# pierrebarbera/epa-ng

Hardware: AMD Instinct MI355X
Metric: query placements/sec (whole node), 512-tip GTR+G4 DNA ref, preplace+thorough (higher is better)
Workload: dtype f64; 1 GPU; cfg2: 512-tip DNA GTR+G4 ref, W=1500, 150 bp reads, dyn-heur 0.99999, preplace+thorough; branches=1021, parallelism=query-shard x1 (weak)

## Files before the change

epa_ng_amd/build.py:

```python
import os
import subprocess
import sys

HERE = os.path.dirname(os.path.abspath(__file__))
ROOT = os.path.dirname(HERE)
CSRC = os.path.join(HERE, "csrc")
HIPCC = os.environ.get("HIPCC", "/opt/rocm/bin/hipcc")

DEV_SOURCES = ["epa_dev.hip", "preplace.hip", "thorough_dna.hip", "thorough_aa.hip", "thorough_aa_mfma.hip", "thorough_generic.hip", "score_at.hip", "marginal.hip", "rell.hip", "comm.hip"]
EXTRA_FLAGS = {"thorough_dna.hip": ["-mllvm", "-amdgpu-sched-strategy=iterative-ilp"],
               "thorough_aa_mfma.hip": ["-mllvm", "-amdgpu-sched-strategy=iterative-ilp"]}
DEV_FLAGS = ["--offload-arch=gfx950", "-O3", "-std=c++17", "-fPIC", "-I", os.path.join(ROOT, "include"),
             "-I", CSRC, "-Wall", "-Wno-unused-function", "-Wno-unused-result"]


def _newer(target, deps):
    if not os.path.exists(target):
        return True
    t = os.path.getmtime(target)
    return any(os.path.getmtime(d) > t for d in deps)


def build_dev(force=False, verbose=False):
    out = os.path.join(HERE, "libepa_dev.so")
    objdir = os.path.join(HERE, "build")
    os.makedirs(objdir, exist_ok=True)
    hdrs = [os.path.join(CSRC, "epa_dev_internal.hpp"), os.path.join(CSRC, "wave_util.hpp"), os.path.join(CSRC, "rccl_abi.hpp"),
            os.path.join(ROOT, "include", "epa_dev.h")]
    objs, procs = [], []
    for src in DEV_SOURCES:
        sp = os.path.join(CSRC, src)
        op = os.path.join(objdir, src.replace(".hip", ".o"))
        objs.append(op)
        if force or _newer(op, [sp] + hdrs):
            cmd = [HIPCC] + DEV_FLAGS + EXTRA_FLAGS.get(src, []) + ["-c", sp, "-o", op]
            if verbose:
                print(" ".join(cmd), file=sys.stderr)
            procs.append((src, subprocess.Popen(cmd), [HIPCC] + DEV_FLAGS + ["-c", sp, "-o", op]))
    for src, p, plain in procs:
        if p.wait() != 0:
            if not EXTRA_FLAGS.get(src) or subprocess.call(plain) != 0:
                raise RuntimeError("hipcc failed on " + src)
    if force or procs or _newer(out, objs):
        cmd = [HIPCC, "--offload-arch=gfx950", "-shared", "-fPIC", "-o", out + ".tmp"] + objs
        subprocess.check_call(cmd)
        os.replace(out + ".tmp", out)
    return out


HOST_SOURCES = ["model.cpp", "aa_models.cpp", "parse_model.cpp", "tree.cpp", "place.cpp", "place_ranks.cpp", "rescore.cpp", "io.cpp", "capi.cpp"]
HOST_FLAGS = ["-O2", "-std=c++17", "-fPIC", "-fopenmp", "-Wall", "-Wextra", "-Wno-unused-parameter",
              "-I", os.path.join(ROOT, "include")]


def build_host(force=False, verbose=False):
    hdir = os.path.join(CSRC, "host")
    out = os.path.join(HERE, "libepa_host.so")
    exe = os.path.join(HERE, "epa-ng-amd")
    srcs = [os.path.join(hdir, s) for s in HOST_SOURCES]
    deps = srcs + [os.path.join(hdir, "epa_host.hpp"), os.path.join(ROOT, "include", "epa_dev.h")]
    link = ["-L", HERE, "-lepa_dev", "-Wl,-rpath,$ORIGIN"]
    if force or _newer(out, deps):
        cmd = ["g++"] + HOST_FLAGS + ["-shared", "-o", out + ".tmp"] + srcs + link
        if verbose:
            print(" ".join(cmd), file=sys.stderr)
        subprocess.check_call(cmd)
        os.replace(out + ".tmp", out)
    main = os.path.join(hdir, "main.cpp")
    if force or _newer(exe, deps + [main, out]):
        cmd = ["g++"] + HOST_FLAGS + ["-o", exe + ".tmp", main, "-L", HERE, "-lepa_host", "-lepa_dev",
                                      "-Wl,-rpath,$ORIGIN"]
        subprocess.check_call(cmd)
        os.replace(exe + ".tmp", exe)
    return out


if __name__ == "__main__":
    print(build_dev(force="--force" in sys.argv, verbose=True))
    print(build_host(force="--force" in sys.argv, verbose=True))
```

epa_ng_amd/csrc/epa_dev.hip:

```cpp
#include "epa_dev_internal.hpp"

#include <math.h>
#include <string.h>

#include <algorithm>
#include <numeric>
#include <atomic>
#include <thread>

static thread_local std::string g_create_err;

int epa_fail(epa_ctx* ctx, int code, const std::string& msg) {
  if (ctx) ctx->err = msg; else g_create_err = msg;
  return code;
}

namespace {
__global__ void __launch_bounds__(256) k_zero(uint4* __restrict__ a, size_t na, uint4* __restrict__ b, size_t nb) {
  const size_t stride = (size_t)gridDim.x * 256, i0 = (size_t)blockIdx.x * 256 + threadIdx.x;
  const uint4 z = make_uint4(0u, 0u, 0u, 0u);
  for (size_t i = i0; i < na; i += stride) a[i] = z;
  for (size_t i = i0; i < nb; i += stride) b[i] = z;
}
}
// ... 473 lines not shown
double log_sum_exp(const double* v, uint32_t K) {
  double mx = v[0], sum = 0.0;
  for (uint32_t j = 1; j < K; ++j) mx = std::max(mx, v[j]);
  for (uint32_t j = 0; j < K; ++j) sum += std::exp(v[j] - mx);
  return mx + std::log(sum);
}
}

extern "C" int epa_quadrature_legendre01(uint32_t K, double* nodes, double* log_weights) {
  if (K < 1 || K > 64 || !nodes || !log_weights) return EPA_ERR_INVALID_ARG;
  std::vector<double> d(K, 0.0), o(K > 1 ? K - 1 : 0), x;
  for (uint32_t i = 1; i < K; ++i) o[i - 1] = (double)i / std::sqrt(4.0 * i * i - 1.0);
  tridiag_eigenvalues(d, o, x);
  for (uint32_t j = 0; j < K; ++j) {
    double t = x[j], dp = 1.0;
    for (int it = 0; it < 3; ++it) {
      double p0 = 1.0, p1 = t;
      for (uint32_t n = 1; n < K; ++n) { const double p2 = ((2.0 * n + 1.0) * t * p1 - n * p0) / (n + 1.0); p0 = p1; p1 = p2; }
      dp = K * (t * p1 - p0) / (t * t - 1.0);
      if (it < 2) t -= p1 / dp;
    }
    nodes[j] = 0.5 * (1.0 + t);
    log_weights[j] = -std::log((1.0 - t) * (1.0 + t)) - 2.0 * std::log(std::fabs(dp));
  }
  const double norm = log_sum_exp(log_weights, K);
  for (uint32_t j = 0; j < K; ++j) log_weights[j] -= norm;
  return EPA_OK;
}

extern "C" int epa_quadrature_laguerre(uint32_t K, double* nodes, double* log_weights) {
  if (K < 1 || K > 64 || !nodes || !log_weights) return EPA_ERR_INVALID_ARG;
  std::vector<double> d(K), o(K > 1 ? K - 1 : 0), x;
  for (uint32_t i = 0; i < K; ++i) d[i] = 2.0 * i + 1.0;
  for (uint32_t i = 1; i < K; ++i) o[i - 1] = (double)i;
  tridiag_eigenvalues(d, o, x);
  for (uint32_t j = 0; j < K; ++j) {
    double t = x[j], lm = 1.0;
    for (int it = 0; it < 3; ++it) {
      double l0 = 1.0, l1 = 1.0 - t;
      for (uint32_t n = 1; n < K; ++n) { const double l2 = ((2.0 * n + 1.0 - t) * l1 - n * l0) / (n + 1.0); l0 = l1; l1 = l2; }
      lm = l0;
      if (it < 2) t -= l1 * t / (K * (l1 - l0));
    }
    nodes[j] = t;
    log_weights[j] = std::log(t) - 2.0 * std::log((double)K) - 2.0 * std::log(std::fabs(lm));
  }
  const double norm = log_sum_exp(log_weights, K);
  for (uint32_t j = 0; j < K; ++j) log_weights[j] -= norm;
  return EPA_OK;
}

extern "C" int epa_dev_device_count(void) {
  int n = 0;
  if (hipGetDeviceCount(&n) != hipSuccess) { (void)hipGetLastError(); return 0; }
  return n;
}

extern "C" const char* epa_dev_last_error(const epa_ctx* ctx) {
  return ctx ? ctx->err.c_str() : g_create_err.c_str();
}

extern "C" int epa_dev_set_query_layout(epa_ctx* ctx, uint32_t code_stride) {
  if (!ctx) return EPA_ERR_INVALID_ARG;
  ctx->code_stride = code_stride;
  return EPA_OK;
}

extern "C" int epa_dev_set_option(epa_ctx* ctx, const char* key, int value) {
  if (!ctx || !key) return EPA_ERR_INVALID_ARG;
  if (strcmp(key, "lookup_block") == 0) {
    if (!ctx->lookup_blocks) return epa_fail(ctx, EPA_ERR_INVALID_ARG, "set_option: lookup_block needs a context in the blocked lookup layout");
    if (value <= 0 || (value & 63)) return epa_fail(ctx, EPA_ERR_INVALID_ARG, "set_option: lookup_block must be a positive multiple of 64");
    for (void* p : ctx->blk_buf)
      if (p) return epa_fail(ctx, EPA_ERR_INVALID_ARG, "set_option: lookup_block must be set before the first preplacement");
    ctx->lookup_block = (uint32_t)value;
    return EPA_OK;
  }
  struct Entry { const char* name; int EpaOptions::*field; };
  static const Entry table[] = {
      {"thorough_generic", &EpaOptions::thorough_generic}, {"preplace_generic", &EpaOptions::preplace_generic},
      {"select_full_rows", &EpaOptions::select_full_rows}, {"select_sort", &EpaOptions::select_sort},
      {"queued_thorough", &EpaOptions::queued_thorough},   {"xcd_balance", &EpaOptions::xcd_balance},
      {"aa_valu", &EpaOptions::aa_valu},                   {"timers", &EpaOptions::timers},
      {"newton_lds", &EpaOptions::newton_lds}};
  for (const Entry& e : table)
    if (strcmp(key, e.name) == 0) {
      ctx->opt.*e.field = value;
      ctx->generic_thorough = ctx->generic_native || ctx->opt.thorough_generic != 0;
      return EPA_OK;
    }
  return epa_fail(ctx, EPA_ERR_INVALID_ARG, std::string("set_option: unknown key '") + key + "'");
}

extern "C" int epa_dev_set_heuristic(epa_ctx* ctx, int mode, double param) {
  if (!ctx) return EPA_ERR_INVALID_ARG;
  if (mode < EPA_HEUR_DYNAMIC || mode > EPA_HEUR_BASEBALL)
    return epa_fail(ctx, EPA_ERR_INVALID_ARG, "set_heuristic: unknown mode");
  if (mode == EPA_HEUR_FIXED && !(param >= 0.0 && param <= 1.0))
    return epa_fail(ctx, EPA_ERR_INVALID_ARG, "set_heuristic: the fraction must lie in [0, 1]");
  ctx->heur_mode = mode;
  ctx->heur_param = param;
  return EPA_OK;
}

extern "C" int epa_dev_set_query_packing(epa_ctx* ctx, int bits) {
  if (!ctx) return EPA_ERR_INVALID_ARG;
  if (bits != 8 && bits != 4) return epa_fail(ctx, EPA_ERR_INVALID_ARG, "set_query_packing: 8 or 4 bits per code");
  if (bits == 4 && ctx->s != 4)
    return epa_fail(ctx, EPA_ERR_UNSUPPORTED, "set_query_packing: the 4-bit format holds nucleotide codes only");
  ctx->code_packed4 = bits == 4;
  return EPA_OK;
}

extern "C" int epa_pack_codes_4bit(const uint8_t* codes, uint32_t Q, uint32_t stride, uint8_t* packed) {
  if (!codes || !packed) return EPA_ERR_INVALID_ARG;
  const size_t ps = ((size_t)stride + 1) / 2;
  const unsigned cap = g_encode_threads.load(std::memory_order_relaxed);
  const unsigned hw = cap ? cap : std::max(1u, std::thread::hardware_concurrency());
  const unsigned nt = (unsigned)std::min<uint64_t>(std::min(hw, 32u), std::max<uint64_t>(1, (uint64_t)Q * stride >> 20));
  std::vector<int> bad(nt, 0);
  auto work = [&](unsigned t) {
    const uint32_t q0 = (uint32_t)((uint64_t)Q * t / nt), q1 = (uint32_t)((uint64_t)Q * (t + 1) / nt);
    unsigned over = 0;
    for (uint32_t q = q0; q < q1; ++q) {
      const uint8_t* r = codes + (size_t)q * stride;
      uint8_t* o = packed + (size_t)q * ps;
      for (uint32_t p = 0; p < stride / 2; ++p) {
        const uint8_t hi = r[2 * p], lo = r[2 * p + 1];
        over |= hi | lo;
        o[p] = (uint8_t)((hi << 4) | lo);
      }
      if (stride & 1) { const uint8_t hi = r[stride - 1]; over |= hi; o[ps - 1] = (uint8_t)(hi << 4); }
    }
    bad[t] = over > 15;
  };
  if (nt == 1) work(0);
  else {
    std::vector<std::thread> th;
    for (unsigned t = 0; t < nt; ++t) th.emplace_back(work, t);
    for (auto& x : th) x.join();
  }
  for (unsigned t = 0; t < nt; ++t) if (bad[t]) return EPA_ERR_INVALID_ARG;
  return EPA_OK;
}

extern "C" int epa_unpack_codes_4bit(const uint8_t* packed, uint32_t Q, uint32_t stride, uint8_t* codes) {
  if (!codes || !packed) return EPA_ERR_INVALID_ARG;
  const size_t ps = ((size_t)stride + 1) / 2;
  for (uint32_t q = 0; q < Q; ++q)
    for (uint32_t i = 0; i < stride; ++i) {
      const uint8_t b = packed[(size_t)q * ps + i / 2];
      codes[(size_t)q * stride + i] = (i & 1) ? (b & 15u) : (b >> 4);
    }
  return EPA_OK;
}

extern "C" int epa_dev_set_stream(epa_ctx* ctx, void* s) {
  if (!ctx) return EPA_ERR_INVALID_ARG;
  ctx->stream = (hipStream_t)s;
  return EPA_OK;
}

extern "C" void epa_dev_destroy(epa_ctx* ctx) {
  if (!ctx) return;
  (void)hipSetDevice(ctx->device);
  (void)hipDeviceSynchronize();
  for (int i = 0; i < epa_ctx::N_BANKS * epa_ctx::N_SCRATCH; ++i) if (ctx->scratch[i]) (void)hipFree(ctx->scratch[i]);
  if (ctx->refT) (void)hipFree(ctx->refT);
  if (ctx->scSum) (void)hipFree(ctx->scSum);
  if (ctx->blen) (void)hipFree(ctx->blen);
  if (ctx->lookup) (void)hipFree(ctx->lookup);
  if (ctx->lookup2) (void)hipFree(ctx->lookup2);
  for (void* p : ctx->blk_buf) if (p) (void)hipFree(p);
  for (auto& v : ctx->blk_ev) for (hipEvent_t e : v) if (e) (void)hipEventDestroy(e);
  if (ctx->th_ctr) (void)hipFree(ctx->th_ctr);
  for (hipEvent_t e : ctx->ev_rb) if (e) (void)hipEventDestroy(e);
  if (ctx->refI) (void)hipFree(ctx->refI);
  if (ctx->cinv) (void)hipFree(ctx->cinv);
  if (ctx->resc0) (void)hipFree(ctx->resc0);
  if (ctx->dmodel) (void)hipFree(ctx->dmodel);
  for (ChunkSlot& sl : ctx->slots) {
    if (sl.h_in) (void)hipHostFree(sl.h_in);
    if (sl.h_out) (void)hipHostFree(sl.h_out);
    if (sl.h_stats) (void)hipHostFree(sl.h_stats);
    if (sl.h_sel) (void)hipHostFree(sl.h_sel);
    if (sl.d_in) (void)hipFree(sl.d_in);
    if (sl.d_unpacked) (void)hipFree(sl.d_unpacked);
    if (sl.d_pairs) (void)hipFree(sl.d_pairs);
    if (sl.d_res) (void)hipFree(sl.d_res);
    if (sl.d_stats) (void)hipFree(sl.d_stats);
    if (sl.d_merge) (void)hipFree(sl.d_merge);
    if (sl.d_gpairs) (void)hipFree(sl.d_gpairs);
    if (sl.d_gres) (void)hipFree(sl.d_gres);
    if (sl.d_goff) (void)hipFree(sl.d_goff);
    if (sl.h_goff) (void)hipHostFree(sl.h_goff);
    for (hipEvent_t e : {sl.ev_up, sl.ev_done, sl.ev_down, sl.ev_base}) if (e) (void)hipEventDestroy(e);
    if (sl.stream) (void)hipStreamDestroy(sl.stream);
  }
  if (ctx->copy_stream) (void)hipStreamDestroy(ctx->copy_stream);
  if (ctx->down_stream) (void)hipStreamDestroy(ctx->down_stream);
  std::vector<EvTimer*> ts = {&ctx->t_lookup};
  for (auto& bk : ctx->t_bank) for (auto& t : bk) ts.push_back(&t);
  for (auto* t : ts) { if (t->a) (void)hipEventDestroy(t->a); if (t->b) (void)hipEventDestroy(t->b); }
  delete ctx;
}

static int precompute_from_tree(epa_ctx* ctx, const epa_tree_desc* t, const uint32_t* d_tipmap);

static int padded_cats(int s, int c_in, uint32_t flags, bool from_tree) {
  int c = (c_in == 1 || c_in == 2) ? 4 : c_in;
  if (s == 4 && c_in >= 3 && (c_in & 3)) c = (c_in + 3) & ~3;
  if (s == 20 && (c_in == 3 || (c_in >= 5 && c_in <= 7))) c = (c_in + 3) & ~3;
  if (c_in >= 3 && c != c_in && (flags & EPA_FLAG_RATE_SCALERS) && !from_tree) c = c_in;
  return c;
}

static bool tuned_thorough_shape(int s, int c, uint32_t flags, bool zero0) {
  const bool sliding = !(flags & EPA_FLAG_RAXML_BLO);
  const bool dna_groups = s == 4 && (c & 3) == 0 && c <= 16;
  const bool tuned_local = (s == 4 && zero0) || s == 20;
  const bool tuned_cats = c == 4 || (dna_groups && sliding && zero0) || (s == 20 && c == 8);
  return tuned_cats && (sliding || tuned_local) &&
         !(flags & (EPA_FLAG_NEWTON_SLOW_BISECT | EPA_FLAG_NEWTON_STRICT_DF | EPA_FLAG_KEEP_EIGENVALUES));
}

static std::atomic<uint64_t> g_mem_cap{0};
extern "C" void epa_dev_set_mem_cap(uint64_t bytes) { g_mem_cap.store(bytes, std::memory_order_relaxed); }

constexpr uint32_t EPA_BLOCK_DEFAULT = 1024;
constexpr int EPA_PLAN_BANKS = 4;

extern "C" int epa_dev_footprint(uint32_t states, uint32_t rate_cats, uint64_t sites, uint64_t branches, int flags,
                                 int from_tree, uint32_t block_branches, int banks, epa_footprint* out) {
  if (!out || !(states == 4 || states == 20) || rate_cats < 1 || rate_cats > EPA_MAX_CATS || !sites || !branches ||
      sites > 0xffffffffull || branches > 0xffffffffull || banks < 0 || (block_branches & 63u))
    return epa_fail(nullptr, EPA_ERR_INVALID_ARG, "footprint: bad shape");
  const uint64_t s = states, W = sites, B = branches;
  const uint64_t c = (uint64_t)padded_cats((int)states, (int)rate_cats, (uint32_t)flags, from_tree != 0);
  const bool blocks = (flags & EPA_FLAG_LOOKUP_BLOCKS) != 0;
  const bool tuned = tuned_thorough_shape((int)s, (int)c, (uint32_t)flags, !(flags & EPA_FLAG_KEEP_EIGENVALUES));
  epa_footprint f;
  memset(&f, 0, sizeof(f));
  f.reft = 8 * 2 * B * c * s * W;
  f.scsum = 4 * B * W;
  if (!blocks) {
    f.lookup = 8 * B * W * (s == 4 ? 16 : 24);
    f.lookup2 = s == 4 ? 8 * B * 2 * ((W + 1) / 2) * 36 : 0;
    f.refi = tuned ? 8 * B * c * s * W + B * W : 0;
  } else {
    const uint64_t blk = std::min<uint64_t>(block_branches ? block_branches : EPA_BLOCK_DEFAULT, (B + 63) & ~(uint64_t)63);
    f.bank = 8 * blk * W * (s == 4 ? 16 : 24) + (s == 4 ? 8 * blk * 2 * ((W + 1) / 2) * 36 : 0);
  }
  f.misc = 8 * B + sizeof(ModelDev) + 256 * (uint64_t)epa_ctx::N_BANKS;
  if (from_tree) {
    const uint64_t n = (B + 3) / 2, cdim = (flags & EPA_FLAG_RATE_SCALERS) ? c : 1;
    f.create_temp = n * W + 32 * 3 * (n - 2) + 4 * 2 * B * cdim * W + 4 * B;
  }
  f.reference = f.reft + f.scsum + f.lookup + f.lookup2 + f.refi + f.misc;
  f.steady = f.reference + (uint64_t)banks * f.bank;
  f.peak = std::max(f.steady, f.reference + f.create_temp);
  *out = f;
  return EPA_OK;
// ... 308 lines not shown
      for (int i = 0; i < S; ++i) if ((mask >> i) & 1u) acc += Ui[x * S + i];
      ta[x] = acc;
    }
  }
  if (tip_b) {
    const uint32_t mask = tipmap[tipchars[(size_t)(r.cb & ~EPA_TIP) * W + site]];
    for (int x = 0; x < S; ++x) {
      double acc = 0.0;
      for (int i = 0; i < S; ++i) if ((mask >> i) & 1u) acc += Ui[x * S + i];
      tb[x] = acc;
    }
  }
  double I[EPA_MAX_CATS][S];
  bool ksmall[EPA_MAX_CATS];
  double mx = 0.0;
  for (int k = 0; k < c; ++k) {
    double av[S], bv[S];
#pragma unroll
    for (int x = 0; x < S; ++x) {
      av[x] = (tip_a ? ta[x] : A[(size_t)(k * S + x) * W]) * Ea[k * S + x];
      bv[x] = (tip_b ? tb[x] : Bv[(size_t)(k * S + x) * W]) * Eb[k * S + x];
    }
    double mxk = 0.0;
#pragma unroll
    for (int i = 0; i < S; ++i) {
      double a = 0.0, b = 0.0;
#pragma unroll
      for (int x = 0; x < S; ++x) {
        a = fma(U[i * S + x], av[x], a);
        b = fma(U[i * S + x], bv[x], b);
      }
      const double v = a * b;
      I[k][i] = v;
      mxk = fmax(mxk, v);
    }
    ksmall[k] = mxk < 0x1p-256;
    mx = fmax(mx, mxk);
  }
  const bool resc = mx < 0x1p-256;
  double* out = refT + (size_t)r.side * cs * W + site;
  for (int k = 0; k < c; ++k) {
    const double mult = (rate_scalers ? ksmall[k] : resc) ? 0x1p+256 : 1.0;
#pragma unroll
    for (int x = 0; x < S; ++x) {
      double acc = 0.0;
#pragma unroll
      for (int i = 0; i < S; ++i) acc = fma(Ui[x * S + i], I[k][i] * mult, acc);
      out[(size_t)(k * S + x) * W] = acc;
    }
  }
  if (rate_scalers) {
    for (int k = 0; k < c; ++k) {
      const uint32_t sa = tip_a ? 0u : sc_side[((size_t)r.ca * c + k) * W + site];
      const uint32_t sb = tip_b ? 0u : sc_side[((size_t)r.cb * c + k) * W + site];
      sc_side[((size_t)r.side * c + k) * W + site] = sa + sb + (ksmall[k] ? 1u : 0u);
    }
    return;
  }
  const uint32_t sa = tip_a ? 0u : sc_side[(size_t)r.ca * W + site];
  const uint32_t sb = tip_b ? 0u : sc_side[(size_t)r.cb * W + site];
  sc_side[(size_t)r.side * W + site] = sa + sb + (resc ? 1u : 0u);
}

__global__ void __launch_bounds__(256) k_tip_sides(const ModelDev* __restrict__ m,
                                                   const uint32_t* __restrict__ tip_of_branch,
                                                   const uint8_t* __restrict__ tipchars,
                                                   const uint32_t* __restrict__ tipmap, uint32_t W,
                                                   double* __restrict__ refT, uint32_t b0) {
  const uint32_t b = b0 + blockIdx.y;
  const uint32_t t = tip_of_branch[b];
  if (t == 0xffffffffu) return;
  const uint32_t site = blockIdx.x * blockDim.x + threadIdx.x;
  if (site >= W) return;
  const int s = m->s, c = m->c;
  const uint32_t mask = tipmap[tipchars[(size_t)t * W + site]];
  double* out = refT + (size_t)(2 * b + 1) * c * s * W + site;
  for (int x = 0; x < s; ++x) {
    double acc = 0.0;
    for (int i = 0; i < s; ++i) if ((mask >> i) & 1u) acc += m->Ui[x * s + i];
    for (int k = 0; k < c; ++k) out[(size_t)(k * s + x) * W] = acc;
  }
}

__global__ void k_scaler_sum(const uint32_t* __restrict__ sc_side, uint32_t* __restrict__ scSum, size_t n,
                             uint32_t W) {
  const size_t i = (size_t)blockIdx.x * blockDim.x + threadIdx.x;
  if (i >= n) return;
  const size_t b = i / W, w = i % W;
  scSum[i] = sc_side[(2 * b) * W + w] + sc_side[(2 * b + 1) * W + w];
}

__global__ void __launch_bounds__(256) k_align_rates(const ModelDev* __restrict__ m, double* __restrict__ refT,
                                                     const uint32_t* __restrict__ sc_side,
                                                     uint32_t* __restrict__ scSum, uint32_t W, uint32_t b0) {
  const uint32_t b = b0 + blockIdx.y;
  const uint32_t site = blockIdx.x * blockDim.x + threadIdx.x;
  if (site >= W) return;
  const int c = m->c, s = m->s;
  const uint32_t* sp = sc_side + (size_t)(2 * b) * c * W + site;
  const uint32_t* sd = sc_side + (size_t)(2 * b + 1) * c * W + site;
  uint32_t mn = 0xffffffffu;
  for (int k = 0; k < c; ++k) mn = min(mn, sp[(size_t)k * W] + sd[(size_t)k * W]);
  double* X = refT + (size_t)(2 * b) * c * s * W + site;
  for (int k = 0; k < c; ++k) {
    const uint32_t d = min(sp[(size_t)k * W] + sd[(size_t)k * W] - mn, 4u);
    if (!d) continue;
    const double f = d == 1 ? 0x1p-256 : d == 2 ? 0x1p-512 : d == 3 ? 0x1p-768 : 0x1p-1024;
    for (int x = 0; x < s; ++x) X[(size_t)(k * s + x) * W] *= f;
  }
  scSum[(size_t)b * W + site] = mn;
}

static int precompute_from_tree(epa_ctx* ctx, const epa_tree_desc* t, const uint32_t* d_tipmap) {
  const uint32_t n = t->tips, R = t->inner_records, B = ctx->B, W = ctx->W;
  if (!t->tipchars || !t->rec_child_a || !t->rec_child_b || !t->rec_length_a || !t->rec_length_b ||
      !t->branch_prox || !t->branch_dist || !d_tipmap)
    return epa_fail(ctx, EPA_ERR_INVALID_ARG, "null pointer in tree descriptor");
  if (n < 3 || R != 3 * (n - 2) || B != 2 * n - 3)
    return epa_fail(ctx, EPA_ERR_INVALID_ARG, "tree descriptor: sizes are not those of an unrooted binary tree");
  std::vector<uint32_t> side_of(R, 0xffffffffu), tip_of_branch(B, 0xffffffffu);
  for (uint32_t b = 0; b < B; ++b) {
    const uint32_t p = t->branch_prox[b], d = t->branch_dist[b];
    if ((p & EPA_TIP) || p >= R || side_of[p] != 0xffffffffu)
      return epa_fail(ctx, EPA_ERR_INVALID_ARG, "tree descriptor: bad proximal record");
    side_of[p] = 2 * b;
    if (d & EPA_TIP) {
      if ((d & ~EPA_TIP) >= n) return epa_fail(ctx, EPA_ERR_INVALID_ARG, "tree descriptor: bad tip id");
      tip_of_branch[b] = d & ~EPA_TIP;
    } else {
      if (d >= R || side_of[d] != 0xffffffffu)
        return epa_fail(ctx, EPA_ERR_INVALID_ARG, "tree descriptor: bad distal record");
      side_of[d] = 2 * b + 1;
    }
  }
  for (uint32_t r = 0; r < R; ++r)
    if (side_of[r] == 0xffffffffu)
      return epa_fail(ctx, EPA_ERR_INVALID_ARG, "tree descriptor: a record is not a side of any branch");
  std::vector<int> level(R, -1);
  auto child_level = [&](uint32_t op) { return (op & EPA_TIP) ? 0 : level[op]; };
  for (uint32_t root = 0; root < R; ++root) {
    if (level[root] >= 0) continue;
    std::vector<uint32_t> st{root};
    while (!st.empty()) {
      const uint32_t r = st.back();
      if (level[r] >= 0) { st.pop_back(); continue; }
      const uint32_t a = t->rec_child_a[r], b = t->rec_child_b[r];
      if ((!(a & EPA_TIP) && a >= R) || (!(b & EPA_TIP) && b >= R) || ((a & EPA_TIP) && (a & ~EPA_TIP) >= n) ||
          ((b & EPA_TIP) && (b & ~EPA_TIP) >= n))
        return epa_fail(ctx, EPA_ERR_INVALID_ARG, "tree descriptor: bad child operand");
      if (st.size() > (size_t)R + 1) return epa_fail(ctx, EPA_ERR_INVALID_ARG, "tree descriptor: cyclic records");
      const bool na = !(a & EPA_TIP) && level[a] < 0, nb = !(b & EPA_TIP) && level[b] < 0;
      if (na) st.push_back(a);
      if (nb) st.push_back(b);
      if (na || nb) continue;
      level[r] = 1 + std::max(child_level(a), child_level(b));
      st.pop_back();
    }
  }
  int nlev = 0;
  for (uint32_t r = 0; r < R; ++r) nlev = std::max(nlev, level[r]);
  std::vector<std::vector<uint32_t>> by_level(nlev + 1);
  for (uint32_t r = 0; r < R; ++r) by_level[level[r]].push_back(r);
  std::vector<RecDev> recs;
  recs.reserve(R);
  std::vector<uint32_t> lev_begin;
  auto opnd = [&](uint32_t op) { return (op & EPA_TIP) ? op : side_of[op]; };
  for (int l = 1; l <= nlev; ++l) {
    lev_begin.push_back((uint32_t)recs.size());
    for (uint32_t r : by_level[l])
      recs.push_back(RecDev{side_of[r], opnd(t->rec_child_a[r]), opnd(t->rec_child_b[r]), 0, t->rec_length_a[r],
                            t->rec_length_b[r]});
  }
  lev_begin.push_back((uint32_t)recs.size());
  uint8_t* d_tips = nullptr;
  RecDev* d_recs = nullptr;
  uint32_t *d_sc = nullptr, *d_tob = nullptr;
  std::string tree_oom;
  {
    epa_footprint f;
    size_t fr = 0, tot = 0;
    if (epa_dev_footprint((uint32_t)ctx->s, (uint32_t)ctx->c_in, W, B, (ctx->rate_scalers ? (int)EPA_FLAG_RATE_SCALERS : 0) |
                          (ctx->lookup_blocks ? (int)EPA_FLAG_LOOKUP_BLOCKS : 0), 1, ctx->lookup_blocks ? ctx->lookup_block : 0,
                          EPA_PLAN_BANKS, &f) == EPA_OK && hipMemGetInfo(&fr, &tot) == hipSuccess)
      tree_oom = " (reference precompute: " + std::to_string(f.peak) + " bytes needed, " + std::to_string(fr) + " bytes free now)";
  }
  auto cleanup = [&]() {
    if (d_tips) (void)hipFree(d_tips);
    if (d_recs) (void)hipFree(d_recs);
    if (d_sc) (void)hipFree(d_sc);
    if (d_tob) (void)hipFree(d_tob);
  };
#define TREE_HIP(call) do { hipError_t e__ = (call); if (e__ != hipSuccess) { cleanup(); (void)hipGetLastError(); return epa_fail(ctx, e__ == hipErrorOutOfMemory ? EPA_ERR_NO_MEMORY : EPA_ERR_HIP, std::string(#call) + ": " + hipGetErrorString(e__) + (e__ == hipErrorOutOfMemory ? tree_oom : std::string())); } } while (0)
  TREE_HIP(hipMalloc(&d_tips, (size_t)n * W));
  TREE_HIP(hipMemcpy(d_tips, t->tipchars, (size_t)n * W, hipMemcpyHostToDevice));
  TREE_HIP(hipMalloc(&d_recs, sizeof(RecDev) * recs.size()));
  TREE_HIP(hipMemcpy(d_recs, recs.data(), sizeof(RecDev) * recs.size(), hipMemcpyHostToDevice));
  const size_t cdim = ctx->rate_scalers ? (size_t)ctx->c : 1;
  TREE_HIP(hipMalloc(&d_sc, sizeof(uint32_t) * 2 * (size_t)B * cdim * W));
  TREE_HIP(hipMemset(d_sc, 0, sizeof(uint32_t) * 2 * (size_t)B * cdim * W));
  TREE_HIP(hipMalloc(&d_tob, sizeof(uint32_t) * B));
  TREE_HIP(hipMemcpy(d_tob, tip_of_branch.data(), sizeof(uint32_t) * B, hipMemcpyHostToDevice));
  const dim3 blk(256);
  for (uint32_t b0 = 0; b0 < B; b0 += EPA_GRID_Y)
    hipLaunchKernelGGL(k_tip_sides, dim3((W + 255) / 256, std::min<uint32_t>(EPA_GRID_Y, B - b0)), blk, 0, ctx->stream,
                       ctx->dmodel, d_tob, d_tips, d_tipmap, W, ctx->refT, b0);
  for (size_t l = 0; l + 1 < lev_begin.size(); ++l) {
    const uint32_t cnt = lev_begin[l + 1] - lev_begin[l];
    if (!cnt) continue;
    for (uint32_t off = 0; off < cnt; off += EPA_GRID_Y) {
      const dim3 grid((W + 255) / 256, std::min<uint32_t>(EPA_GRID_Y, cnt - off));
      if (ctx->s == 4)
        hipLaunchKernelGGL(k_clv_level<4>, grid, blk, 0, ctx->stream, ctx->dmodel, d_recs + lev_begin[l] + off,
                           d_tips, d_tipmap, W, ctx->refT, d_sc, ctx->rate_scalers ? 1 : 0);
      else
        hipLaunchKernelGGL(k_clv_level<20>, grid, blk, 0, ctx->stream, ctx->dmodel, d_recs + lev_begin[l] + off,
                           d_tips, d_tipmap, W, ctx->refT, d_sc, ctx->rate_scalers ? 1 : 0);
    }
  }
  if (ctx->rate_scalers) {
    for (uint32_t b0 = 0; b0 < B; b0 += EPA_GRID_Y)
      hipLaunchKernelGGL(k_align_rates, dim3((W + 255) / 256, std::min<uint32_t>(EPA_GRID_Y, B - b0)), blk, 0, ctx->stream,
                         ctx->dmodel, ctx->refT, d_sc, ctx->scSum, W, b0);
  } else {
    const size_t nbw = (size_t)B * W;
    hipLaunchKernelGGL(k_scaler_sum, dim3((uint32_t)((nbw + 255) / 256)), blk, 0, ctx->stream, d_sc, ctx->scSum, nbw, W);
  }
  TREE_HIP(hipStreamSynchronize(ctx->stream));
  TREE_HIP(hipGetLastError());
#undef TREE_HIP
  cleanup();
  return EPA_OK;
}

template <int S>
__global__ void __launch_bounds__(256) k_tree_logl(const ModelDev* __restrict__ m,
                                                  const double* __restrict__ refT,
                                                  const uint32_t* __restrict__ scSum, uint32_t b, double len,
                                                  uint32_t W, const double* __restrict__ cinv,
                                                  double* __restrict__ partial) {
  __shared__ double U[S * S];
  __shared__ double E[EPA_MAX_CATS * S];
  __shared__ double red[256];
  const int c = m->c;
  for (int i = threadIdx.x; i < S * S; i += blockDim.x) U[i] = m->U[i];
  for (int i = threadIdx.x; i < c * S; i += blockDim.x) E[i] = exp(m->lam[i % S] * m->rate[i / S] * len);
  __syncthreads();
  const uint32_t site = blockIdx.x * blockDim.x + threadIdx.x;
  double v = 0.0;
  if (site < W) {
    const size_t cs = (size_t)c * S;
    const double* X = refT + (size_t)(2 * b) * cs * W + site;
    const double* D = refT + (size_t)(2 * b + 1) * cs * W + site;
    double L = 0.0;
    for (int k = 0; k < c; ++k) {
      double xv[S], dv[S];
#pragma unroll
      for (int x = 0; x < S; ++x) { xv[x] = X[(size_t)(k * S + x) * W]; dv[x] = D[(size_t)(k * S + x) * W] * E[k * S + x]; }
      double t = 0.0;
#pragma unroll
      for (int i = 0; i < S; ++i) {
        double a = 0.0, d = 0.0;
#pragma unroll
        for (int x = 0; x < S; ++x) { a = fma(U[i * S + x], xv[x], a); d = fma(U[i * S + x], dv[x], d); }
        t = fma(m->pi[i] * a, d, t);
      }
      L = fma(m->w[k], t, L);
    }
    if (cinv) L += cinv[site];
    v = log(L) + (double)scSum[(size_t)b * W + site] * (-256.0 * 0.6931471805599453094);
  }
  red[threadIdx.x] = v;
  __syncthreads();
  for (int o = 128; o; o >>= 1) {
    if ((int)threadIdx.x < o) red[threadIdx.x] += red[threadIdx.x + o];
    __syncthreads();
  }
  if (threadIdx.x == 0) partial[blockIdx.x] = red[0];
}

extern "C" int epa_dev_tree_logl(epa_ctx* ctx, uint32_t branch, double* lnl) {
  if (!ctx || !lnl || branch >= ctx->B) return epa_fail(ctx, EPA_ERR_INVALID_ARG, "bad argument");
  EPA_HIP(ctx, hipSetDevice(ctx->device));
  const uint32_t nblk = (ctx->W + 255) / 256;
  double* d_part = (double*)epa_scratch(ctx, 9, sizeof(double) * nblk);
  if (!d_part) return epa_fail(ctx, EPA_ERR_HIP, "hipMalloc(tree lnL partials)");
  const double len = ctx->h_blen[branch];
  if (ctx->s == 4)
    hipLaunchKernelGGL(k_tree_logl<4>, dim3(nblk), dim3(256), 0, ctx->stream, ctx->dmodel, ctx->refT, ctx->scSum,
                       branch, len, ctx->W, ctx->cinv, d_part);
  else
    hipLaunchKernelGGL(k_tree_logl<20>, dim3(nblk), dim3(256), 0, ctx->stream, ctx->dmodel, ctx->refT, ctx->scSum,
                       branch, len, ctx->W, ctx->cinv, d_part);
  std::vector<double> part(nblk);
  EPA_HIP(ctx, hipMemcpyAsync(part.data(), d_part, sizeof(double) * nblk, hipMemcpyDeviceToHost, ctx->stream));
  EPA_HIP(ctx, hipStreamSynchronize(ctx->stream));
  double s = 0.0;
  for (double p : part) s += p;
  *lnl = s;
  return EPA_OK;
}

extern "C" int epa_dev_create_from_tree(const epa_tree_desc* tree, int device, epa_ctx** out) {
  if (!tree || !out) return epa_fail(nullptr, EPA_ERR_INVALID_ARG, "null argument");
  *out = nullptr;
  if (epa_dev_device_count() <= 0)
    return epa_fail(nullptr, EPA_ERR_NO_DEVICE,
                    "no HIP device visible: libepa_dev has no CPU fallback by design");
  epa_ctx* ctx = new epa_ctx();
  int rc = create_impl(&tree->ref, device, ctx, tree);
  if (rc != EPA_OK) {
    g_create_err = ctx->err;
    epa_dev_destroy(ctx);
// ... 339 lines not shown
extern "C" int epa_dev_select_candidates(epa_ctx* ctx, const double* lnl, uint32_t Q,
                                         double threshold, epa_pair* pairs, uint64_t max_pairs,
                                         uint64_t* n_pairs) {
  if (!ctx || !lnl || !pairs || !n_pairs) return epa_fail(ctx, EPA_ERR_INVALID_ARG, "null argument");
  *n_pairs = 0;
  if (Q == 0) return EPA_OK;
  EPA_HIP(ctx, hipSetDevice(ctx->device));
  const double* d_lnl = (const double*)epa_to_device(ctx, 3, lnl, sizeof(double) * (size_t)Q * ctx->B);
  if (!d_lnl) return epa_fail(ctx, EPA_ERR_HIP, "lnl upload failed");
  const bool out_dev = epa_is_device_ptr(pairs);
  epa_pair* d_pairs = out_dev ? pairs : (epa_pair*)epa_scratch(ctx, 4, sizeof(epa_pair) * max_pairs);
  if (!d_pairs) return epa_fail(ctx, EPA_ERR_HIP, "hipMalloc(pairs)");
  int rc = launch_select(ctx, d_lnl, Q, threshold, d_pairs, max_pairs, n_pairs);
  if (rc) return rc;
  if (!out_dev && *n_pairs) {
    EPA_HIP(ctx, hipMemcpy(pairs, d_pairs, sizeof(epa_pair) * (*n_pairs), hipMemcpyDeviceToHost));
  }
  return EPA_OK;
}

static int chunk_body_begin(epa_ctx* ctx, const uint8_t* d_codes, const uint32_t* d_begin, const uint32_t* d_span,
                            uint32_t Q, uint32_t max_span, double threshold, epa_pair* d_pairs,
                            uint64_t max_pairs, uint32_t* rb, SelectPending* sp, epa_result* d_res = nullptr,
                            unsigned long long* d_stats = nullptr) {
  const uint32_t pitch = (ctx->B + 7u) & ~7u;
  double* d_lnl = (double*)epa_scratch(ctx, 3, sizeof(double) * (size_t)Q * pitch);
  if (!d_lnl) return epa_fail(ctx, EPA_ERR_HIP, "hipMalloc(chunk table)");
  ctx->lnl_pitch = pitch;
  const uint32_t nseg = (ctx->B + 63) / 64;
  ctx->segmax = nullptr;
  if (nseg <= 64 && ctx->heur_mode == 0) {
    ctx->segp = (nseg + 7u) & ~7u;
    ctx->segmax = (unsigned long long*)epa_scratch(ctx, 10, sizeof(unsigned long long) * (size_t)Q * ctx->segp);
    if (!ctx->segmax) return epa_fail(ctx, EPA_ERR_HIP, "hipMalloc(segment maxima)");
    ctx->segmax_zero_bytes = sizeof(unsigned long long) * (size_t)Q * ctx->segp;
  }
  int rc = launch_preplace(ctx, d_codes, d_begin, d_span, Q, d_lnl, max_span);
  if (ctx->segmax_zero_bytes) {
    ctx->segmax_zero_bytes = 0;
    if (!rc) rc = epa_fail(ctx, EPA_ERR_HIP, "segment maxima not cleared");
  }
  if (!rc) rc = launch_select_begin(ctx, d_lnl, Q, threshold, d_pairs, max_pairs, d_span, rb, sp);
  ctx->lnl_pitch = 0;
  ctx->segmax = nullptr;
  if (!rc && d_stats && sp->d_rb && sp->bitmap && max_pairs <= 0xffffffffull) {
    rc = launch_select_emit(ctx, sp);
    if (!rc) rc = epa_zero_async(ctx, d_stats, 128, epa_th_ctr(ctx), epa_th_ctr(ctx) ? 64 : 0);
    if (!rc) {
      ctx->clean_stats[ctx->bank] = d_stats;
      ctx->clean_ctr[ctx->bank] = epa_th_ctr(ctx) != nullptr;
    }
  }
  if (!rc && d_res && d_stats && sp->d_rb && sp->bitmap && max_pairs <= 0xffffffffull) {
    const bool off = !ctx->opt.queued_thorough;
    const int cls = epa_span_class(ctx->s, max_span);
    const bool eligible = !off && ctx->s == 4 && !ctx->generic_thorough && ctx->dna.ng == 1 && epa_th_ctr(ctx) &&
                          (cls <= 2 || cls == 10 || cls == 11);
    if (eligible) {
      rc = launch_select_emit(ctx, sp);
      if (!rc && ctx->clean_stats[ctx->bank] == d_stats) ctx->clean_stats[ctx->bank] = nullptr;
      else if (!rc) rc = epa_zero_async(ctx, d_stats, 128);
      if (!rc) {
        const int q = launch_thorough_queued(ctx, d_pairs, sp->d_rb, max_pairs, d_codes, d_begin, d_span, max_span, d_res, d_stats);
        if (q == -2) return EPA_ERR_HIP;
        sp->queued_cls = q;
      }
    }
  }
  return rc;
}

static int chunk_body_end(epa_ctx* ctx, SelectPending* sp, const uint8_t* d_codes, const uint32_t* d_begin,
                          const uint32_t* d_span, uint32_t max_span, epa_pair* d_pairs, epa_result* d_res,
                          unsigned long long* d_stats, uint64_t* n_out) {
  const uint32_t pitch = (ctx->B + 7u) & ~7u;
  ctx->lnl_pitch = pitch;
  uint64_t n = 0;
  int rc = launch_select_end(ctx, sp, &n);
  ctx->lnl_pitch = 0;
  if (rc) return rc;
  rc = select_check_status(ctx, sp);
  if (rc) return rc;
  *n_out = n;
  if (sp->queued_cls >= 0 && sp->rb[9 + sp->queued_cls] == (uint32_t)n) return EPA_OK;
  if (ctx->clean_stats[ctx->bank] == d_stats && sp->queued_cls < 0) ctx->clean_stats[ctx->bank] = nullptr;
  else {
    ctx->clean_stats[ctx->bank] = nullptr;
    rc = epa_zero_async(ctx, d_stats, 128);
    if (rc) return rc;
  }
  if (n == 0) return EPA_OK;
  return launch_thorough(ctx, d_pairs, n, d_codes, d_begin, d_span, max_span, d_res, d_stats,
                         sp->have_hist ? sp->cls_hist : nullptr);
}

static int chunk_body(epa_ctx* ctx, const uint8_t* d_codes, const uint32_t* d_begin, const uint32_t* d_span,
                      uint32_t Q, uint32_t max_span, double threshold, epa_pair* d_pairs, epa_result* d_res,
                      uint64_t max_pairs, unsigned long long* d_stats, uint64_t* n_out) {
  uint32_t rb[64] = {};
  SelectPending sp;
  int rc = chunk_body_begin(ctx, d_codes, d_begin, d_span, Q, max_span, threshold, d_pairs, max_pairs, rb, &sp, d_res, d_stats);
  if (rc) return rc;
  return chunk_body_end(ctx, &sp, d_codes, d_begin, d_span, max_span, d_pairs, d_res, d_stats, n_out);
}

static int chunk_stats(epa_ctx* ctx, uint64_t n, const unsigned long long* hst, epa_thorough_stats* stats) {
  epa_xcd_feedback(ctx, n, hst);
  ctx->last_stats.pairs = n;
  ctx->last_stats.rounds = hst[0];
  ctx->last_stats.newton_evals = hst[1];
  ctx->last_stats.reverts = hst[2];
  if (stats) *stats = ctx->last_stats;
  if (hst[3])
    return epa_fail(ctx, EPA_ERR_NEG_INF,
                    "-INF logl at branch " + std::to_string((uint32_t)(hst[4] >> 32)) +
                        " with sequence " + std::to_string((uint32_t)(hst[4] & 0xffffffffu)));
  return EPA_OK;
}

static int thorough_supported(epa_ctx*) { return EPA_OK; }

extern "C" int epa_dev_place_chunk(epa_ctx* ctx, const uint8_t* q_codes, const uint32_t* win_begin,
                                   const uint32_t* win_span, uint32_t Q, uint32_t max_span,
                                   double threshold, epa_pair* pairs, epa_result* results,
                                   uint64_t max_pairs, uint64_t* n_pairs, epa_thorough_stats* stats) {
  if (!ctx || !q_codes || !win_begin || !win_span || !pairs || !results || !n_pairs)
    return epa_fail(ctx, EPA_ERR_INVALID_ARG, "null argument");
  *n_pairs = 0;
  if (stats) memset(stats, 0, sizeof(*stats));
  if (Q == 0) return EPA_OK;
  EPA_HIP(ctx, hipSetDevice(ctx->device));
  int rc = thorough_supported(ctx);
  if (rc) return rc;
  rc = epa_dev_build_lookup(ctx);
  if (rc) return rc;
  if (max_span == 0) {
    std::vector<uint32_t> buf;
    const uint32_t* hs = host_view(win_span, Q, buf, ctx->stream);
    if (!hs) return epa_fail(ctx, EPA_ERR_HIP, "cannot read window spans");
    for (uint32_t q = 0; q < Q; ++q) max_span = std::max(max_span, hs[q]);
  }
  if (max_span > ctx->W) max_span = ctx->W;
  const uint8_t* d_codes = epa_codes_to_device(ctx, q_codes, Q);
  const uint32_t* d_begin = (const uint32_t*)epa_to_device(ctx, 1, win_begin, sizeof(uint32_t) * Q);
  const uint32_t* d_span = (const uint32_t*)epa_to_device(ctx, 2, win_span, sizeof(uint32_t) * Q);
  if (!d_codes || !d_begin || !d_span) return epa_fail(ctx, EPA_ERR_HIP, "query upload failed");
  const bool pairs_dev = epa_is_device_ptr(pairs), res_dev = epa_is_device_ptr(results);
  epa_pair* d_pairs = pairs_dev ? pairs : (epa_pair*)epa_scratch(ctx, 4, sizeof(epa_pair) * max_pairs);
  epa_result* d_res = res_dev ? results : (epa_result*)epa_scratch(ctx, 5, sizeof(epa_result) * max_pairs);
  if (!d_pairs || !d_res) return epa_fail(ctx, EPA_ERR_HIP, "hipMalloc(chunk buffers)");
  unsigned long long* d_stats = reinterpret_cast<unsigned long long*>(reinterpret_cast<char*>(epa_th_ctr(ctx)) + 128);
  uint64_t n = 0;
  rc = chunk_body(ctx, d_codes, d_begin, d_span, Q, max_span, threshold, d_pairs, d_res, max_pairs, d_stats, &n);
  if (rc) return rc;
  *n_pairs = n;
  if (n == 0) return EPA_OK;
  unsigned long long hst[16];
  if (!pairs_dev)
    EPA_HIP(ctx, hipMemcpyAsync(pairs, d_pairs, sizeof(epa_pair) * n, hipMemcpyDeviceToHost, ctx->stream));
  if (!res_dev)
    EPA_HIP(ctx, hipMemcpyAsync(results, d_res, sizeof(epa_result) * n, hipMemcpyDeviceToHost, ctx->stream));
  EPA_HIP(ctx, hipMemcpyAsync(hst, d_stats, 128, hipMemcpyDeviceToHost, ctx->stream));
  EPA_HIP(ctx, hipStreamSynchronize(ctx->stream));
  return chunk_stats(ctx, n, hst, stats);
}

static int slot_of(epa_ctx* ctx, int slot, ChunkSlot** out) {
  if (!ctx) return EPA_ERR_INVALID_ARG;
  if (slot < 0 || slot >= epa_ctx::N_SLOTS) return epa_fail(ctx, EPA_ERR_INVALID_ARG, "chunk pipeline: slot must be 0 .. 23");
  ChunkSlot& s = ctx->slots[slot];
  if (!ctx->copy_stream) EPA_HIP(ctx, hipStreamCreateWithFlags(&ctx->copy_stream, hipStreamNonBlocking));
  if (!ctx->down_stream) EPA_HIP(ctx, hipStreamCreateWithFlags(&ctx->down_stream, hipStreamNonBlocking));
  if (!s.ev_up) {
    EPA_HIP(ctx, hipEventCreateWithFlags(&s.ev_up, hipEventDisableTiming));
    EPA_HIP(ctx, hipEventCreateWithFlags(&s.ev_done, hipEventDisableTiming));
    EPA_HIP(ctx, hipEventCreateWithFlags(&s.ev_down, hipEventDisableTiming));
// ... 745 lines not shown
```

epa_ng_amd/csrc/epa_dev_internal.hpp:

```cpp
#pragma once

#include <hip/hip_runtime.h>
#include <stdint.h>

#include <string>
#include <vector>

#include "epa_dev.h"

#define EPA_MAX_STATES 20
#define EPA_MAX_CATS 16
#define EPA_MAX_COLS 24
#define EPA_GRID_Y 65535u

struct ModelDNA {
  double U[16];
  double Ui[16];
  double lam[4];
  double rate[16];
  double w[16];
  double pi[4];
  int ng;
};

struct BloConsts {
  double min_branch, max_branch, default_branch, epsilon, pendant_default;
  uint32_t max_rounds, max_newton;
  uint32_t sliding;
  uint32_t newton_variant;
};

struct ModelDev {
  int s, c, ncols;
  double U[EPA_MAX_STATES * EPA_MAX_STATES];
  double Ui[EPA_MAX_STATES * EPA_MAX_STATES];
  double lam[EPA_MAX_STATES];
  double pi[EPA_MAX_STATES];
  double rate[EPA_MAX_CATS];
  double w[EPA_MAX_CATS];
  uint32_t colmask[EPA_MAX_COLS];
  double qt[EPA_MAX_COLS * EPA_MAX_STATES];
};

struct EvTimer {
  hipEvent_t a = nullptr, b = nullptr;
  bool valid = false;
};

struct SelectPending {
  const double* d_lnl = nullptr;
  uint32_t Q = 0, cap = 0;
  double threshold = 0.0;
  epa_pair* d_pairs = nullptr;
  uint64_t max_pairs = 0;
  const uint32_t* d_span = nullptr;
  unsigned long long *stage = nullptr, *keys_a = nullptr, *keys_b = nullptr;
  uint32_t *counts = nullptr, *offsets = nullptr;
  uint32_t *bitmap = nullptr, *boffs = nullptr;
  uint32_t wpr = 0;
  void* temp = nullptr;
  size_t sort_bytes = 0;
  uint32_t* rb = nullptr;
  bool have_status = false;
  bool rerun = false;
  hipEvent_t ev_rb = nullptr;
  const uint32_t* d_rb = nullptr;
  bool emitted = false;
  int queued_cls = -1;
  uint32_t cls_hist[16] = {};
  bool have_hist = false;
  const uint32_t* pre_status = nullptr;
};

struct ChunkSlot {
  void* h_in = nullptr;
  size_t h_in_sz = 0;
  void* d_in = nullptr;
  const uint8_t* x_codes = nullptr;
  const uint32_t* x_begin = nullptr;
  const uint32_t* x_span = nullptr;
  size_t d_in_sz = 0;
  uint8_t* d_unpacked = nullptr;
  size_t d_unpacked_sz = 0;
  size_t codes_bytes = 0;
  uint32_t Q = 0, stride = 0;
  bool packed4 = false;
  epa_pair* d_pairs = nullptr;
  epa_result* d_res = nullptr;
  size_t cap = 0;
  void* h_out = nullptr;
  size_t h_out_sz = 0;
  unsigned long long* h_stats = nullptr;
  unsigned long long* d_stats = nullptr;
  hipEvent_t ev_up = nullptr, ev_done = nullptr, ev_down = nullptr, ev_base = nullptr;
  hipStream_t stream = nullptr;
  const epa_pair* out_pairs = nullptr;
  const epa_result* out_res = nullptr;
  uint64_t n = 0;
  int state = 0;
  SelectPending sel;
  uint32_t* h_sel = nullptr;
  const uint8_t* l_codes = nullptr;
  const uint32_t *l_begin = nullptr, *l_span = nullptr;
  epa_pair* l_pairs = nullptr;
  epa_result* l_res = nullptr;
  uint32_t l_max_span = 0, l_flags = 0;
  int leader = -1;
  int g_index = 0;
  int g_n = 0;
  int g_left = 0;
  int g_slots[8] = {};
  uint32_t g_qoff[9] = {};
  uint32_t own_Q = 0;
  const uint8_t* own_x_codes = nullptr;
  const uint32_t *own_x_begin = nullptr, *own_x_span = nullptr;
  void* d_merge = nullptr;
  size_t d_merge_sz = 0;
  epa_pair* d_gpairs = nullptr;
  epa_result* d_gres = nullptr;
  size_t g_cap = 0;
  uint32_t* d_goff = nullptr;
  uint32_t* h_goff = nullptr;
};
constexpr int EPA_MAX_GROUP = 8;

struct EpaOptions {
  int thorough_generic = 0;
  int preplace_generic = 0;
  int select_full_rows = 0;
  int select_sort = 0;
  int queued_thorough = 0;
  int xcd_balance = 1;
  int aa_valu = 0;
  int timers = 1;
  int newton_lds = 0;
};

struct epa_ctx {
  int device = 0;
  EpaOptions opt;
  int n_cu = 256;
  hipStream_t stream = nullptr;
  std::string err;

  int s = 0, c = 0, ncols = 0;
  int c_in = 0;
  uint32_t W = 0, B = 0;
  ModelDev hmodel;
  ModelDev* dmodel = nullptr;
  ModelDNA dna;
  bool dna_zero0 = false;
  bool rate_scalers = false;
  bool generic_thorough = false;
  bool generic_native = false;
  BloConsts blo;
  int aa_x_as_n = 0;
  uint32_t code_stride = 0;

  double* refT = nullptr;
  uint32_t* scSum = nullptr;
  double* blen = nullptr;
  double* lookup = nullptr;
  double* refI = nullptr;
  uint8_t* resc0 = nullptr;
  double* cinv = nullptr;
  double inv_w0 = 0.0;
  double* lookup2 = nullptr;
  bool lookup_built = false;
  bool lookup_blocks = false;
  uint32_t lookup_block = 1024;
  std::vector<double> h_blen;

  static constexpr int N_SCRATCH = 18;
  static constexpr int N_SLOTS = 24;
  static constexpr int N_BANKS = 1 + N_SLOTS;
  int bank = 0;
  void* scratch[N_BANKS * N_SCRATCH] = {};
  size_t scratch_sz[N_BANKS * N_SCRATCH] = {};

  uint32_t* d_status = nullptr;
  uint32_t select_cap = 64;
  uint32_t* th_ctr = nullptr;
  uint32_t lnl_pitch = 0;
  unsigned long long* segmax = nullptr;
  uint32_t segp = 0;
  size_t segmax_zero_bytes = 0;
  bool code_packed4 = false;
  int heur_mode = 0;
  double heur_param = 0.0;

  hipStream_t copy_stream = nullptr, down_stream = nullptr;
  ChunkSlot slots[N_SLOTS];

  enum { T_PREPLACE = 0, T_THOROUGH = 1, T_SELECT = 2, T_SCORE = 3, T_SITES = 4, T_RELL = 5, T_MARGINAL = 6, N_TIMERS = 7 };
  EvTimer t_lookup;
  std::vector<hipEvent_t> blk_ev[N_BANKS];
  uint32_t blk_ev_n[N_BANKS] = {};
  void* blk_buf[N_BANKS] = {};
  size_t blk_sz[N_BANKS] = {};
  EvTimer t_bank[N_BANKS][N_TIMERS];
  uint32_t xcd_cum[9] = {0u, 1u << 17, 2u << 17, 3u << 17, 4u << 17, 5u << 17, 6u << 17, 7u << 17, 1u << 20};
  double xcd_w[8] = {0.125, 0.125, 0.125, 0.125, 0.125, 0.125, 0.125, 0.125};
  double last_sclk_mhz = 0.0;
  bool xstamp_ok = false;
  hipEvent_t ev_rb[N_BANKS] = {};
  const void* clean_stats[N_BANKS] = {};
  bool clean_ctr[N_BANKS] = {};
  int t_last[N_TIMERS] = {};
  epa_thorough_stats last_stats{};
};

int epa_fail(epa_ctx* ctx, int code, const std::string& msg);
void* epa_scratch(epa_ctx* ctx, int slot, size_t bytes);
inline uint32_t* epa_th_ctr(epa_ctx* ctx) { return ctx->th_ctr ? ctx->th_ctr + 64 * ctx->bank : nullptr; }
int epa_zero_async(epa_ctx* ctx, void* p, size_t bytes, void* p2 = nullptr, size_t bytes2 = 0);
inline int epa_th_ctr_reset(epa_ctx* ctx) {
  if (ctx->clean_ctr[ctx->bank]) { ctx->clean_ctr[ctx->bank] = false; return 0; }
  return epa_zero_async(ctx, epa_th_ctr(ctx), 64);
}
bool epa_is_device_ptr(const void* p);
const void* epa_to_device(epa_ctx* ctx, int slot, const void* p, size_t bytes);
const uint8_t* epa_codes_to_device(epa_ctx* ctx, const uint8_t* q_codes, uint32_t Q);
const uint8_t* epa_codes_to_device(epa_ctx* ctx, const uint8_t* q_codes, uint32_t Q);
void epa_xcd_feedback(epa_ctx* ctx, uint64_t n_pairs, const unsigned long long* hst);
#define EPA_XSTAMP_MASK 0x7ffffffffffull
void epa_timer_start(epa_ctx* ctx, EvTimer& t);
void epa_timer_stop(epa_ctx* ctx, EvTimer& t);
inline EvTimer& epa_t(epa_ctx* ctx, int which) { ctx->t_last[which] = ctx->bank; return ctx->t_bank[ctx->bank][which]; }

#define EPA_HIP(ctx, call)                                                               \
  do {                                                                                    \
    hipError_t e__ = (call);                                                              \
    if (e__ != hipSuccess)                                                                \
      return epa_fail(ctx, EPA_ERR_HIP, std::string(#call) + ": " + hipGetErrorString(e__)); \
  } while (0)

constexpr int EPA_N_CLS = 12;
constexpr uint32_t EPA_AA_LDS_MAX_SPAN = 102;
__host__ __device__ inline int epa_span_class(int states, uint32_t span) {
  if (states != 4) return span <= 64 ? 0 : span <= 128 ? 1 : span <= 192 ? 2 : 3;
  if (span > 64 && span <= 96) return 10;
  if (span > 128 && span <= 160) return 11;
  const uint32_t nch = (span + 63) / 64;
  return nch <= 4 ? (nch ? (int)nch - 1 : 0) : nch <= 6 ? 4 : nch <= 8 ? 5 : nch <= 12 ? 6 : nch <= 16 ? 7 : nch <= 24 ? 8 : 9;
}

int launch_transform(epa_ctx* ctx, const double* d_clv_or_null, const uint8_t* d_tip_or_null,
                     const uint32_t* d_tipmap, uint32_t tipmap_size, double* dst);
int launch_build_lookup(epa_ctx* ctx);
int launch_build_lookup2(epa_ctx* ctx);
uint32_t epa_block_branches(const epa_ctx* ctx);
size_t epa_block_bytes(int s, uint32_t W, uint32_t blk, size_t* off2);
void* epa_block_buffer(epa_ctx* ctx);
int launch_build_lookup_block(epa_ctx* ctx, uint32_t b0, uint32_t nb, double* blk_lookup);
int launch_build_lookup2_block(epa_ctx* ctx, uint32_t nb, const double* blk_lookup, double* blk_lookup2);
int launch_preplace(epa_ctx* ctx, const uint8_t* d_codes, const uint32_t* d_begin,
                    const uint32_t* d_span, uint32_t Q, double* d_lnl, uint32_t max_span);
int preplace_check_status(epa_ctx* ctx);
int launch_thorough(epa_ctx* ctx, const epa_pair* d_pairs, uint64_t n_pairs, const uint8_t* d_codes,
                    const uint32_t* d_begin, const uint32_t* d_span, uint32_t max_span,
                    epa_result* d_out, unsigned long long* d_stats,
                    const uint32_t* cls_hist = nullptr);
int launch_thorough_queued(epa_ctx* ctx, const epa_pair* d_pairs, const uint32_t* d_spec, uint64_t max_pairs,
                           const uint8_t* d_codes, const uint32_t* d_begin, const uint32_t* d_span, uint32_t max_span,
                           epa_result* d_out, unsigned long long* d_stats);
int launch_select_emit(epa_ctx* ctx, SelectPending* sp);
int launch_thorough_aa(epa_ctx* ctx, const epa_pair* d_pairs, const uint32_t* d_order, uint64_t n_pairs,
                       const uint8_t* d_codes, const uint32_t* d_begin, const uint32_t* d_span,
                       uint32_t max_span, bool want_lds, epa_result* d_out, unsigned long long* d_stats);
int launch_thorough_generic(epa_ctx* ctx, const epa_pair* d_pairs, uint64_t n_pairs, const uint8_t* d_codes,
                            const uint32_t* d_begin, const uint32_t* d_span, uint32_t max_span,
                            epa_result* d_out, unsigned long long* d_stats,
                            const uint32_t* d_order = nullptr, bool caller_times = false);
int launch_thorough_aa_mfma(epa_ctx* ctx, const epa_pair* d_pairs, const uint32_t* d_order, uint64_t n_pairs,
                            const uint8_t* d_codes, const uint32_t* d_begin, const uint32_t* d_span,
                            uint32_t max_span, epa_result* d_out, unsigned long long* d_stats);
int launch_score_at(epa_ctx* ctx, const epa_pair* d_pairs, const double* d_pendant, const double* d_distal,
                    const double* d_proximal, uint64_t n, const uint8_t* d_codes, const uint32_t* d_begin,
                    const uint32_t* d_span, double* d_lnl);
int launch_site_lnl(epa_ctx* ctx, const epa_pair* d_pairs, const double* d_pendant, const double* d_distal,
                    const double* d_proximal, const uint32_t* d_order, uint64_t n_rows, const uint8_t* d_codes,
                    const uint32_t* d_begin, const uint32_t* d_span, uint32_t pitch, bool pad, double* d_rows,
                    bool timed);
int launch_rell(epa_ctx* ctx, const epa_pair* d_pairs, const double* d_pendant, const double* d_distal,
                const double* d_proximal, uint64_t n, const uint8_t* d_codes, const uint32_t* d_begin,
                const uint32_t* d_span, const uint32_t* h_span, uint32_t Q, const uint64_t* d_stream_id,
                uint32_t replicates, uint64_t seed, double* d_support);
int launch_marginal(epa_ctx* ctx, const epa_pair* d_pairs, uint64_t n, const double* d_rule, uint32_t Kx, uint32_t Kp,
                    const uint8_t* d_codes, const uint32_t* d_begin, const uint32_t* d_span, double* d_marginal,
                    double* d_grid);
int launch_select(epa_ctx* ctx, const double* d_lnl, uint32_t Q, double threshold,
                  epa_pair* d_pairs, uint64_t max_pairs, uint64_t* n_pairs,
                  const uint32_t* d_span = nullptr);
int launch_select_begin(epa_ctx* ctx, const double* d_lnl, uint32_t Q, double threshold, epa_pair* d_pairs,
                        uint64_t max_pairs, const uint32_t* d_span, uint32_t* rb, SelectPending* sp);
int launch_select_end(epa_ctx* ctx, SelectPending* sp, uint64_t* n_pairs);
int select_check_status(epa_ctx* ctx, const SelectPending* sp);
```

epa_ng_amd/csrc/preplace.hip:

```cpp
#include "epa_dev_internal.hpp"
#include "wave_util.hpp"

#include <cstdlib>
#include <cstring>
#include <rocprim/device/device_radix_sort.hpp>

using epa_radix_cfg = rocprim::radix_sort_config<rocprim::default_config, rocprim::default_config,
                                                 rocprim::default_config, 0>;
#include <rocprim/device/device_scan.hpp>

#include <algorithm>

namespace {

constexpr int GQ = 256;
constexpr int CH = 160;
constexpr int SPREAD = 96;
constexpr int TROWS = CH + SPREAD;
constexpr int NB = 16;
constexpr int CW = CH / 4;

struct Group {
  uint32_t start;
  uint32_t count;
  uint32_t min_begin;
  uint32_t cls;
};

__device__ __forceinline__ void validate_window(uint32_t i, uint32_t begin, uint32_t span, uint32_t W,
                                                uint32_t cmax, uint32_t* status) {
  if (span == 0) atomicMax(&status[0], 0x80000000u | i);
  else if ((uint64_t)begin + span > W || span > cmax) atomicMax(&status[1], 0x80000000u | i);
}
__global__ void k_validate(const uint32_t* __restrict__ win_begin, const uint32_t* __restrict__ win_span,
                           uint32_t Q, uint32_t W, uint32_t cmax, uint32_t* __restrict__ status) {
  const uint32_t i = blockIdx.x * blockDim.x + threadIdx.x;
  if (i < Q) validate_window(i, win_begin[i], win_span[i], W, cmax, status);
}

__global__ void k_iota(uint32_t* v, uint32_t n) {
  const uint32_t i = blockIdx.x * blockDim.x + threadIdx.x;
  if (i < n) v[i] = i;
}

__global__ void __launch_bounds__(256) k_count_keys(const uint32_t* __restrict__ keys, uint32_t Q,
                                                    uint32_t* __restrict__ cnt, uint32_t* __restrict__ rank) {
  const uint32_t q = blockIdx.x * 256 + threadIdx.x;
  if (q < Q) rank[q] = atomicAdd(&cnt[keys[q]], 1u);
}
__global__ void __launch_bounds__(1024) k_scan_counts(uint32_t* __restrict__ cnt, uint32_t K) {
  __shared__ uint32_t wsum[16];
  __shared__ uint32_t carry_s;
  const uint32_t t = threadIdx.x, lane = t & 63u, wv = t >> 6;
  if (t == 0) carry_s = 0;
  __syncthreads();
  constexpr uint32_t PER = 8;
  for (uint32_t base = 0; base < K; base += 1024 * PER) {
    uint32_t v[PER], tot = 0;
#pragma unroll
    for (uint32_t i = 0; i < PER; ++i) {
      const uint32_t k = base + t * PER + i;
      v[i] = k < K ? cnt[k] : 0u;
      tot += v[i];
    }
    uint32_t inc = tot;
#pragma unroll
    for (int o = 1; o < 64; o <<= 1) {
      const uint32_t u = __shfl_up(inc, o);
      if ((int)lane >= o) inc += u;
    }
    if (lane == 63) wsum[wv] = inc;
    __syncthreads();
    uint32_t before = carry_s;
    for (uint32_t w = 0; w < wv; ++w) before += wsum[w];
    uint32_t run = before + inc - tot;
#pragma unroll
    for (uint32_t i = 0; i < PER; ++i) {
      const uint32_t k = base + t * PER + i;
      if (k < K) cnt[k] = run;
      run += v[i];
    }
    __syncthreads();
    if (t == 1023) carry_s = run;
    __syncthreads();
  }
}
__global__ void __launch_bounds__(256) k_scatter_sorted(const uint32_t* __restrict__ keys,
                                                        const uint32_t* __restrict__ rank,
                                                        const uint32_t* __restrict__ offs, uint32_t Q,
                                                        uint32_t* __restrict__ sorted_keys,
                                                        uint32_t* __restrict__ perm) {
  const uint32_t q = blockIdx.x * 256 + threadIdx.x;
  if (q >= Q) return;
  const uint32_t k = keys[q], pos = offs[k] + rank[q];
  sorted_keys[pos] = k;
  perm[pos] = q;
}

__global__ void __launch_bounds__(256) k_make_groups(const uint32_t* __restrict__ sorted_keys, uint32_t Q,
                                                     uint32_t Wp, uint32_t n_blocks,
                                                     uint32_t class_blocks, uint32_t gq0, uint32_t gq1,
                                                     uint32_t spr0, uint32_t max_runs, Group* __restrict__ groups,
                                                     uint32_t max_groups, uint32_t* __restrict__ status) {
  extern __shared__ uint32_t sh[];
  uint32_t* lo = sh;
  uint32_t* runbase = lo + n_blocks + 1;
  uint32_t* run_start = runbase + n_blocks + 1;
  uint32_t* run_end = run_start + max_runs;
  uint32_t* run_off = run_end + max_runs;
  auto lower_bound = [&](uint32_t a, uint32_t b, uint64_t key) {
    while (a < b) {
      const uint32_t m = (a + b) >> 1;
      if ((uint64_t)sorted_keys[m] < key) a = m + 1; else b = m;
    }
    return a;
  };
  for (uint32_t k = threadIdx.x; k <= n_blocks; k += blockDim.x)
    lo[k] = k == n_blocks ? Q : lower_bound(0, Q, (uint64_t)k * Wp);
  for (uint32_t i = threadIdx.x; i < max_groups; i += blockDim.x) groups[i] = Group{0, 0, 0, 0};
  __syncthreads();
  if (threadIdx.x == 0) {
    uint32_t r = 0;
    for (uint32_t b = 0; b < n_blocks; ++b) {
      const uint32_t gq = b >= class_blocks ? gq1 : gq0;
      runbase[b] = r;
      r += (lo[b + 1] - lo[b] + gq - 1) / gq;
    }
    runbase[n_blocks] = r;
  }
  __syncthreads();
  const uint32_t nruns = min(runbase[n_blocks], max_runs);
  for (uint32_t r = threadIdx.x; r < nruns; r += blockDim.x) {
    uint32_t b = 0;
    while (b + 1 < n_blocks && r >= runbase[b + 1]) ++b;
    const uint32_t gq = b >= class_blocks ? gq1 : gq0;
    const uint32_t start = lo[b] + (r - runbase[b]) * gq, end = min(lo[b + 1], start + gq);
    const uint32_t k0 = sorted_keys[start], k1 = sorted_keys[end - 1];
    const uint32_t spr = b >= class_blocks ? (uint32_t)SPREAD : spr0;
    run_start[r] = start;
    run_end[r] = end;
    run_off[r] = (k1 - k0 < spr) ? 1u : (k1 / spr - k0 / spr + 1);
  }
  __syncthreads();
  uint32_t* cnt = run_off + max_runs + 1;
  for (uint32_t r = threadIdx.x; r < nruns; r += blockDim.x) cnt[r] = run_off[r];
  __syncthreads();
  for (uint32_t r = threadIdx.x; r <= nruns; r += blockDim.x) {
    uint32_t g = 0;
    for (uint32_t i = 0; i < r; ++i) g += cnt[i];
    run_off[r] = g;
  }
  __syncthreads();
  if (threadIdx.x == 0) {
    const uint32_t r1 = class_blocks < n_blocks ? min(runbase[class_blocks], nruns) : nruns;
    status[4] = min(run_off[nruns], max_groups);
    status[5] = min(run_off[r1], max_groups);
  }
  for (uint32_t r = threadIdx.x; r < nruns; r += blockDim.x) {
    uint32_t b = 0;
    while (b + 1 < n_blocks && r >= runbase[b + 1]) ++b;
    const uint32_t cls = b >= class_blocks ? 1u : 0u;
    const uint32_t start = run_start[r], end = run_end[r], g0 = run_off[r], n = run_off[r + 1] - g0;
    if (n == 1) {
      if (g0 < max_groups) groups[g0] = Group{start, end - start, 0, cls};
    } else {
      const uint32_t spr = cls ? (uint32_t)SPREAD : spr0;
      const uint32_t kb = sorted_keys[start] / spr;
// ... 1264 lines not shown
        if (weighted ? (sabove + iw >= threshold) : (ic >= rem)) atomicMin(&s_first, t);
        atomicMax(&s_last, t);
      }
      __syncthreads();
      uint32_t ts = s_first;
      if (ts == 256u) {
        if (p == 7) { all = true; n = B; break; }
        ts = s_last;
      }
      const uint32_t ec = ts ? s_hc[ts - 1u] : 0u;
      const double ew = ts ? s_hw[ts - 1u] : 0.0;
      m = s_hc[ts] - ec;
      cabove += ec;
      rem -= weighted ? 0u : ec;
      sabove += ew;
      prefix = (prefix << 8) | (unsigned long long)(255u - ts);
      __syncthreads();
    }
    if (!all) {
      K = prefix;
      if (weighted) {
        const double w = exp(seg_val(K) - mx) / tot;
        double sum = sabove;
        while (r < m && sum < threshold) { sum += w; ++r; }
        n = cabove + r;
      } else {
        r = rem;
      }
    }
  }
  if (n > 0) {
    const bool ordered = !all && r < m;
    uint32_t tie_base = 0;
    if (t == 0) s_cnt = 0u;
    __syncthreads();
    for (uint32_t base = 0; base < B; base += 256) {
      const uint32_t i = base + t;
      const unsigned long long k = i < B ? seg_key(src[i]) : 0ull;
      bool sel = i < B && (all || k > K);
      bool eq = i < B && !all && k == K;
      if (ordered) {
        const unsigned long long bal = __ballot(eq);
        if (lane == 0) s_wu[wv] = (uint32_t)__popcll(bal);
        __syncthreads();
        uint32_t before = tie_base + (uint32_t)__popcll(bal & ((1ull << lane) - 1ull));
        for (uint32_t w = 0; w < wv; ++w) before += s_wu[w];
        tie_base += s_wu[0] + s_wu[1] + s_wu[2] + s_wu[3];
        eq = eq && before < r;
        __syncthreads();
      }
      sel = sel || eq;
      uint32_t slot = 0;
      if (!so.bitmap) {
        const unsigned long long bal = __ballot(sel);
        uint32_t wbase = 0;
        if (lane == 0 && bal) wbase = atomicAdd(&s_cnt, (uint32_t)__popcll(bal));
        wbase = (uint32_t)__builtin_amdgcn_readfirstlane((int)wbase);
        slot = wbase + (uint32_t)__popcll(bal & ((1ull << lane) - 1ull));
      }
      if (sel) so.put(q, i, slot, status);
    }
  }
  if (t == 0) counts[q] = so.count(n);
}

__global__ void __launch_bounds__(256) k_class_hist(const uint32_t* __restrict__ counts,
                                                   const uint32_t* __restrict__ win_span, uint32_t Q,
                                                   int states, uint32_t* __restrict__ hist) {
  const uint32_t q = blockIdx.x * 256 + threadIdx.x;
  const int cls = q < Q ? epa_span_class(states, win_span[q]) : -1;
  const uint32_t n = q < Q ? counts[q] : 0;
  for (int c = 0; c < EPA_N_CLS; ++c) {
    if (__ballot(cls == c) == 0ull) continue;
    uint32_t v = cls == c ? n : 0;
#pragma unroll
    for (int o = 32; o; o >>= 1) v += __shfl_xor(v, o);
    if ((threadIdx.x & 63) == 0 && v) atomicAdd(&hist[c], v);
  }
}

__global__ void __launch_bounds__(64) k_pack_readback(const uint32_t* __restrict__ status,
                                                     const uint32_t* __restrict__ total,
                                                     const uint32_t* __restrict__ pre_status,
                                                     uint32_t* __restrict__ out) {
  const uint32_t t = threadIdx.x;
  if (t == 0) out[0] = *total;
  if (t < 8 + EPA_N_CLS) out[1 + t] = status[t];
  if (t < 4) out[32 + t] = pre_status ? pre_status[t] : 0u;
}

__global__ void __launch_bounds__(256) k_compact(const unsigned long long* __restrict__ stage,
                                                 const uint32_t* __restrict__ counts,
                                                 const uint32_t* __restrict__ offsets, uint32_t Q,
                                                 uint32_t cap, unsigned long long* __restrict__ keys) {
  const uint32_t q = blockIdx.x * 4 + (threadIdx.x >> 6);
  const int lane = threadIdx.x & 63;
  if (q >= Q) return;
  const uint32_t n = counts[q], o = offsets[q];
  for (uint32_t i = lane; i < n; i += 64) keys[o + i] = stage[(size_t)q * cap + i];
}

__global__ void __launch_bounds__(256) k_emit_pairs(const uint32_t* __restrict__ bitmap, uint32_t wpr,
                                                    const uint32_t* __restrict__ boffs,
                                                    epa_pair* __restrict__ pairs, uint32_t nb, uint32_t max_pairs) {
  __shared__ uint32_t wsum[4];
  const uint32_t b = blockIdx.x, t = threadIdx.x, lane = t & 63u, wv = t >> 6;
  if (boffs[nb] > max_pairs) return;
  uint32_t base = boffs[b];
  const uint32_t end = boffs[b + 1];
  if (base == end) return;
  const uint32_t* row = bitmap + (size_t)b * wpr;
  for (uint32_t w0 = 0; w0 < wpr && base < end; w0 += 256) {
    const uint32_t wi = w0 + t;
    uint32_t bits = wi < wpr ? row[wi] : 0u;
    const uint32_t c = (uint32_t)__popc(bits);
    uint32_t inc = c;
#pragma unroll
    for (int o = 1; o < 64; o <<= 1) {
      const uint32_t u = __shfl_up(inc, o);
      if ((int)lane >= o) inc += u;
    }
    if (lane == 63) wsum[wv] = inc;
    __syncthreads();
    uint32_t before = 0, total = 0;
#pragma unroll
    for (uint32_t w = 0; w < 4; ++w) {
      if (w < wv) before += wsum[w];
      total += wsum[w];
    }
    uint32_t o = base + before + inc - c;
    while (bits) {
      const uint32_t k = (uint32_t)__ffs((int)bits) - 1u;
      bits &= bits - 1u;
      pairs[o].branch_id = b;
      pairs[o].seq_id = wi * 32u + k;
      ++o;
    }
    base += total;
    __syncthreads();
  }
}

__global__ void k_keys_to_pairs(const unsigned long long* __restrict__ keys, uint64_t n,
                                epa_pair* __restrict__ pairs) {
  const uint64_t i = (uint64_t)blockIdx.x * blockDim.x + threadIdx.x;
  if (i < n) {
    pairs[i].branch_id = (uint32_t)(keys[i] >> 32);
    pairs[i].seq_id = (uint32_t)(keys[i] & 0xffffffffu);
  }
}

size_t align256(size_t x) { return (x + 255) & ~(size_t)255; }

}

int launch_build_lookup2(epa_ctx* ctx) {
  if (!ctx->lookup2)
    EPA_HIP(ctx, hipMalloc(&ctx->lookup2, sizeof(double) * (size_t)ctx->B * 2 * ((ctx->W + 1) / 2) * PE));
  for (uint32_t b0 = 0; b0 < ctx->B; b0 += EPA_GRID_Y)
    hipLaunchKernelGGL(k_build_lookup2, dim3((ctx->W * PE + 255) / 256, std::min<uint32_t>(EPA_GRID_Y, ctx->B - b0)), dim3(256), 0,
                       ctx->stream, ctx->lookup, ctx->W, ctx->lookup2, b0);
  EPA_HIP(ctx, hipGetLastError());
  return EPA_OK;
}

int launch_build_lookup2_block(epa_ctx* ctx, uint32_t nb, const double* blk_lookup, double* blk_lookup2) {
  for (uint32_t r0 = 0; r0 < nb; r0 += EPA_GRID_Y)
    hipLaunchKernelGGL(k_build_lookup2, dim3((ctx->W * PE + 255) / 256, std::min<uint32_t>(EPA_GRID_Y, nb - r0)), dim3(256), 0,
                       ctx->stream, blk_lookup, ctx->W, blk_lookup2, r0);
  EPA_HIP(ctx, hipGetLastError());
  return EPA_OK;
// ... 163 lines not shown
  }
  { const int rc = mark(2 * nblocks); if (rc) return rc; }
  if (timed) ctx->blk_ev_n[ctx->bank] = 2 * nblocks + 1;
  EPA_HIP(ctx, hipGetLastError());
  return EPA_OK;
}

int preplace_check_status(epa_ctx* ctx) {
  if (!ctx->d_status) return EPA_OK;
  uint32_t st[4];
  EPA_HIP(ctx, hipMemcpy(st, ctx->d_status, sizeof(st), hipMemcpyDeviceToHost));
  if (st[0])
    return epa_fail(ctx, EPA_ERR_QUERY_ALL_GAP, "Sequence " + std::to_string(st[0] & 0x7fffffffu) +
                                                    " does not appear to have any non-gap sites!");
  if (st[1])
    return epa_fail(ctx, EPA_ERR_QUERY_WIDTH, "Query sequence length not same as reference alignment!");
  return EPA_OK;
}

int launch_select_begin(epa_ctx* ctx, const double* d_lnl, uint32_t Q, double threshold, epa_pair* d_pairs,
                        uint64_t max_pairs, const uint32_t* d_span, uint32_t* rb, SelectPending* sp) {
  sp->have_hist = false;
  const uint32_t B = ctx->B;
  const uint32_t pitch = ctx->lnl_pitch ? ctx->lnl_pitch : B;
  if (!sp->rerun) sp->pre_status = (const uint32_t*)ctx->d_status;
  const double stream_band = (ctx->heur_mode == 0 && threshold > 0.0 && threshold < 1.0) ? 1.0 - std::log((1.0 - threshold) / (double)B) : 0.0;
  const int mode = ctx->heur_mode;
  uint32_t limit = 0;
  if (mode == 1) {
    limit = (uint32_t)std::min<double>((double)B, std::ceil(ctx->heur_param * (double)B));
    ctx->select_cap = std::max(ctx->select_cap, std::max(limit, 1u));
  } else if (mode == 2) {
    ctx->select_cap = std::max(ctx->select_cap, std::min(B, 48u));
  }
  const uint32_t cap = ctx->select_cap;
  size_t scan_bytes = 0, sort_bytes = 0;
  (void)rocprim::exclusive_scan(nullptr, scan_bytes, (uint32_t*)nullptr, (uint32_t*)nullptr, 0u, Q,
                                rocprim::plus<uint32_t>(), ctx->stream);
  const size_t worst = std::min<uint64_t>(max_pairs, (uint64_t)Q * cap);
  (void)rocprim::radix_sort_keys<epa_radix_cfg>(nullptr, sort_bytes, (unsigned long long*)nullptr,
                                 (unsigned long long*)nullptr, worst, 0, 64, ctx->stream);
  const uint32_t wpr = (Q + 31) / 32;
  const bool force_sort = ctx->opt.select_sort != 0;
  const bool bm = !force_sort && (size_t)B * wpr * sizeof(uint32_t) <= ((size_t)64 << 20);
  sp->bitmap = nullptr;
  if (bm) {
    const size_t cb = align256(sizeof(uint32_t) * ((size_t)B + 1));
    const size_t mb = align256(sizeof(uint32_t) * (size_t)B * wpr);
    const size_t qb2 = align256(sizeof(uint32_t) * (Q + 1));
    char* base = (char*)epa_scratch(ctx, 7, 512 + cb + mb + qb2);
    if (!base) return epa_fail(ctx, EPA_ERR_HIP, "hipMalloc(select scratch)");
    uint32_t* status = reinterpret_cast<uint32_t*>(base);
    uint32_t* bcount = reinterpret_cast<uint32_t*>(base + 512);
    uint32_t* bitmap = reinterpret_cast<uint32_t*>(base + 512 + cb);
    uint32_t* counts = reinterpret_cast<uint32_t*>(base + 512 + cb + mb);
    sp->bitmap = bitmap; sp->boffs = bcount; sp->wpr = wpr;
    sp->counts = counts; sp->offsets = nullptr;
    sp->d_lnl = d_lnl; sp->Q = Q; sp->threshold = threshold; sp->d_pairs = d_pairs; sp->max_pairs = max_pairs;
    sp->d_span = d_span; sp->cap = cap; sp->rb = rb;
    { const int zr = epa_zero_async(ctx, base, 512 + cb + mb); if (zr) return zr; }
    epa_timer_start(ctx, epa_t(ctx, epa_ctx::T_SELECT));
    const SelOut so{nullptr, 0u, bitmap, bcount, wpr};
    const dim3 grid((Q + 3) / 4);
    const int nr = (int)((B + 63) / 64);
#define SEL(N) hipLaunchKernelGGL(k_select<N>, grid, dim3(256), 0, ctx->stream, d_lnl, Q, B, pitch, threshold, mode, limit, so, counts, status)
    const bool seg_off = ctx->opt.select_full_rows != 0;
    bool seg_hist = false;
    if (ctx->segmax && !seg_off && mode == 0 && threshold < 1.0 && nr <= 64)
    {
      const double band_x = 1.0 - std::log((1.0 - threshold) / (double)B);
      const double band_t = std::max(band_x, std::log((double)B) + 38.0);
      constexpr uint32_t sel_grid = 16;
      const dim3 grid_seg(std::min<uint32_t>((Q + 3) / 4, (uint32_t)ctx->n_cu * sel_grid));
      hipLaunchKernelGGL(k_select_seg<8>, grid_seg, dim3(256), 0, ctx->stream, d_lnl, ctx->segmax, ctx->segp, Q, B, pitch, threshold,
                         band_x, band_t, so, counts, status, d_span, ctx->s, d_span ? status + 8 : nullptr);
      seg_hist = d_span != nullptr;
    }
    else if (nr <= 2) SEL(2); else if (nr <= 4) SEL(4); else if (nr <= 8) SEL(8); else if (nr <= 16) SEL(16);
    else if (nr <= 32) SEL(32); else if (nr <= 64) SEL(64);
    else if (nr <= 128) hipLaunchKernelGGL(k_select_wg<32>, dim3(Q), dim3(256), 0, ctx->stream, d_lnl, Q, B, pitch, threshold, mode, limit, so, counts, status);
    else if (nr <= 256) hipLaunchKernelGGL(k_select_wg<64>, dim3(Q), dim3(256), 0, ctx->stream, d_lnl, Q, B, pitch, threshold, mode, limit, so, counts, status);
    else hipLaunchKernelGGL(k_select_stream, dim3(Q), dim3(256), 0, ctx->stream, d_lnl, Q, B, pitch, threshold, stream_band, mode, limit, so, counts, status);
#undef SEL
    hipLaunchKernelGGL(k_scan_counts, dim3(1), dim3(1024), 0, ctx->stream, bcount, B + 1);
    if (d_span && !seg_hist)
      hipLaunchKernelGGL(k_class_hist, dim3((Q + 255) / 256), dim3(256), 0, ctx->stream, counts, d_span, Q,
                         ctx->s, status + 8);
    hipLaunchKernelGGL(k_pack_readback, dim3(1), dim3(64), 0, ctx->stream, status, bcount + B,
                       sp->pre_status, status + 64);
    EPA_HIP(ctx, hipMemcpyAsync(rb, status + 64, sizeof(uint32_t) * 36, hipMemcpyDeviceToHost, ctx->stream));
    sp->have_status = sp->pre_status != nullptr;
    if (!ctx->ev_rb[ctx->bank]) EPA_HIP(ctx, hipEventCreateWithFlags(&ctx->ev_rb[ctx->bank], hipEventDisableTiming));
    EPA_HIP(ctx, hipEventRecord(ctx->ev_rb[ctx->bank], ctx->stream));
    sp->ev_rb = ctx->ev_rb[ctx->bank];
    sp->d_rb = status + 64;
    sp->emitted = false;
    sp->queued_cls = -1;
    return EPA_OK;
  }
  sp->ev_rb = nullptr; sp->d_rb = nullptr; sp->emitted = false; sp->queued_cls = -1;
  const size_t qb = align256(sizeof(uint32_t) * (Q + 1));
  const size_t sb = align256(sizeof(unsigned long long) * (size_t)Q * cap);
  const size_t kb = align256(sizeof(unsigned long long) * worst);
  const size_t tb = std::max(scan_bytes, sort_bytes);
  char* base = (char*)epa_scratch(ctx, 7, 512 + 2 * qb + sb + 2 * kb + tb);
  if (!base) return epa_fail(ctx, EPA_ERR_HIP, "hipMalloc(select scratch)");
  uint32_t* status = reinterpret_cast<uint32_t*>(base);
  uint32_t* counts = reinterpret_cast<uint32_t*>(base + 512);
  uint32_t* offsets = reinterpret_cast<uint32_t*>(base + 512 + qb);
  sp->stage = reinterpret_cast<unsigned long long*>(base + 512 + 2 * qb);
  sp->keys_a = reinterpret_cast<unsigned long long*>(base + 512 + 2 * qb + sb);
  sp->keys_b = reinterpret_cast<unsigned long long*>(base + 512 + 2 * qb + sb + kb);
  sp->temp = base + 512 + 2 * qb + sb + 2 * kb;
  sp->sort_bytes = sort_bytes;
  sp->counts = counts; sp->offsets = offsets;
  sp->d_lnl = d_lnl; sp->Q = Q; sp->threshold = threshold; sp->d_pairs = d_pairs; sp->max_pairs = max_pairs;
  sp->d_span = d_span; sp->cap = cap; sp->rb = rb;
  EPA_HIP(ctx, hipMemsetAsync(status, 0, 512, ctx->stream));
  EPA_HIP(ctx, hipMemsetAsync(counts + Q, 0, sizeof(uint32_t), ctx->stream));
  epa_timer_start(ctx, epa_t(ctx, epa_ctx::T_SELECT));
  const dim3 grid((Q + 3) / 4);
  const int nr = (int)((B + 63) / 64);
  const SelOut so{sp->stage, cap, nullptr, nullptr, 0u};
#define SEL(N) hipLaunchKernelGGL(k_select<N>, grid, dim3(256), 0, ctx->stream, d_lnl, Q, B, pitch, threshold, mode, limit, so, counts, status)
  if (nr <= 2) SEL(2); else if (nr <= 4) SEL(4); else if (nr <= 8) SEL(8); else if (nr <= 16) SEL(16);
  else if (nr <= 32) SEL(32); else if (nr <= 64) SEL(64);
  else if (nr <= 128) hipLaunchKernelGGL(k_select_wg<32>, dim3(Q), dim3(256), 0, ctx->stream, d_lnl, Q, B, pitch, threshold, mode, limit, so, counts, status);
  else if (nr <= 256) hipLaunchKernelGGL(k_select_wg<64>, dim3(Q), dim3(256), 0, ctx->stream, d_lnl, Q, B, pitch, threshold, mode, limit, so, counts, status);
  else hipLaunchKernelGGL(k_select_stream, dim3(Q), dim3(256), 0, ctx->stream, d_lnl, Q, B, pitch, threshold, stream_band, mode, limit, so, counts, status);
#undef SEL
  EPA_HIP(ctx, rocprim::exclusive_scan(sp->temp, scan_bytes, counts, offsets, 0u, Q + 1,
                                       rocprim::plus<uint32_t>(), ctx->stream));
  if (d_span)
    hipLaunchKernelGGL(k_class_hist, dim3((Q + 255) / 256), dim3(256), 0, ctx->stream, counts, d_span, Q,
                       ctx->s, status + 8);
  hipLaunchKernelGGL(k_pack_readback, dim3(1), dim3(64), 0, ctx->stream, status, offsets + Q,
                     sp->pre_status, status + 64);
  EPA_HIP(ctx, hipMemcpyAsync(rb, status + 64, sizeof(uint32_t) * 36, hipMemcpyDeviceToHost, ctx->stream));
  sp->have_status = sp->pre_status != nullptr;
  return EPA_OK;
}

int launch_select_emit(epa_ctx* ctx, SelectPending* sp) {
  if (!sp->bitmap || !sp->d_rb || sp->emitted) return EPA_OK;
  hipLaunchKernelGGL(k_emit_pairs, dim3(ctx->B), dim3(256), 0, ctx->stream, sp->bitmap, sp->wpr, sp->boffs, sp->d_pairs, ctx->B, (uint32_t)std::min<uint64_t>(sp->max_pairs, 0xffffffffu));
  epa_timer_stop(ctx, epa_t(ctx, epa_ctx::T_SELECT));
  EPA_HIP(ctx, hipGetLastError());
  sp->emitted = true;
  return EPA_OK;
}

int launch_select_end(epa_ctx* ctx, SelectPending* sp, uint64_t* n_pairs) {
  const uint32_t B = ctx->B, Q = sp->Q;
  for (;;) {
    if (sp->ev_rb) EPA_HIP(ctx, hipEventSynchronize(sp->ev_rb));
    else EPA_HIP(ctx, hipStreamSynchronize(ctx->stream));
    const uint32_t total = sp->rb[0];
    const uint32_t* hst = sp->rb + 1;
    if (hst[2] && !sp->bitmap) {
      if (sp->cap >= B) return epa_fail(ctx, EPA_ERR_HIP, "select_candidates: staging overflow");
      ctx->select_cap = std::min<uint32_t>(B, std::max(sp->cap * 4, hst[2]));
      uint32_t* rb = sp->rb;
      sp->rerun = true;
      int rc = launch_select_begin(ctx, sp->d_lnl, Q, sp->threshold, sp->d_pairs, sp->max_pairs, sp->d_span, rb, sp);
      sp->rerun = false;
      if (rc) return rc;
      continue;
    }
    if (total > sp->max_pairs)
      return epa_fail(ctx, EPA_ERR_PAIR_OVERFLOW,
                      "select_candidates: " + std::to_string(total) + " candidates exceed max_pairs");
    if (total && sp->bitmap) {
      if (!sp->emitted)
        hipLaunchKernelGGL(k_emit_pairs, dim3(B), dim3(256), 0, ctx->stream, sp->bitmap, sp->wpr, sp->boffs, sp->d_pairs, B, (uint32_t)std::min<uint64_t>(sp->max_pairs, 0xffffffffu));
    } else if (total) {
      const dim3 grid((Q + 3) / 4);
      hipLaunchKernelGGL(k_compact, grid, dim3(256), 0, ctx->stream, sp->stage, sp->counts, sp->offsets, Q, sp->cap,
                         sp->keys_a);
      int bits = 33;
      while ((1ull << (bits - 32)) <= B && bits < 64) ++bits;
      size_t sort_bytes = sp->sort_bytes;
      EPA_HIP(ctx, rocprim::radix_sort_keys<epa_radix_cfg>(sp->temp, sort_bytes, sp->keys_a, sp->keys_b, (size_t)total,
                                                           32, bits, ctx->stream));
      hipLaunchKernelGGL(k_keys_to_pairs, dim3((total + 255) / 256), dim3(256), 0, ctx->stream, sp->keys_b,
                         (uint64_t)total, sp->d_pairs);
    }
    if (!sp->emitted) epa_timer_stop(ctx, epa_t(ctx, epa_ctx::T_SELECT));
    EPA_HIP(ctx, hipGetLastError());
    *n_pairs = total;
    if (sp->d_span) {
      for (int c = 0; c < EPA_N_CLS; ++c) sp->cls_hist[c] = hst[8 + c];
      sp->have_hist = true;
    }
    return EPA_OK;
  }
}

int select_check_status(epa_ctx* ctx, const SelectPending* sp) {
  if (!sp->have_status) return EPA_OK;
  const uint32_t* st = sp->rb + 32;
  if (st[0])
    return epa_fail(ctx, EPA_ERR_QUERY_ALL_GAP, "Sequence " + std::to_string(st[0] & 0x7fffffffu) +
                                                    " does not appear to have any non-gap sites!");
  if (st[1])
    return epa_fail(ctx, EPA_ERR_QUERY_WIDTH, "Query sequence length not same as reference alignment!");
  return EPA_OK;
}

int launch_select(epa_ctx* ctx, const double* d_lnl, uint32_t Q, double threshold,
                  epa_pair* d_pairs, uint64_t max_pairs, uint64_t* n_pairs, const uint32_t* d_span) {
  uint32_t rb[64] = {};
  SelectPending sp;
  int rc = launch_select_begin(ctx, d_lnl, Q, threshold, d_pairs, max_pairs, d_span, rb, &sp);
  if (rc) return rc;
  return launch_select_end(ctx, &sp, n_pairs);
}
```

epa_ng_amd/csrc/thorough_dna.hip:

```cpp
#include "epa_dev_internal.hpp"
#include "wave_util.hpp"

#include <cstring>
#include <rocprim/device/device_radix_sort.hpp>

using epa_radix_cfg = rocprim::radix_sort_config<rocprim::default_config, rocprim::default_config,
                                                 rocprim::default_config, 0>;

#include <algorithm>
#include <vector>
#include <cstdio>
#include <type_traits>
#include <cstdlib>

namespace {


struct ThArgs {
  ModelDNA m;
  BloConsts blo;
  const double* refT;
  const double* refI;
  const uint8_t* resc0;
  const double* cinv;
  double inv_w0;
  const uint32_t* scSum;
  const double* blen;
  const double* qt;
  const epa_pair* pairs;
  const uint32_t* order;
  const uint8_t* codes;
  uint32_t cstride, crel;
  const uint32_t* win_begin;
  const uint32_t* win_span;
  epa_result* out;
  unsigned long long* stats;
  uint32_t* qctr;
  double* sscratch;
  uint64_t n_pairs;
  uint32_t W;
  uint32_t Wpad;
  const uint32_t* spec;
  uint32_t spec_cls, spec_max;
  uint32_t xcum[9];
  uint32_t xstamp;
};

using namespace epa_wave;

__device__ __forceinline__ uint32_t zero_after(double v) {
  uint32_t z;
  asm volatile("v_mov_b32 %0, 0" : "=v"(z) : "v"(__double2loint(v)));
  return z;
}

using KArgs = const __attribute__((address_space(4))) ThArgs*;
__device__ __forceinline__ KArgs kargs_fresh() {
  KArgs p = (KArgs)__builtin_amdgcn_kernarg_segment_ptr();
  asm volatile("" : "+s"(p));
  return p;
}
struct PhaseModel {
  double U[16], Ui[16], w[4];
  __device__ __forceinline__ void load(uint32_t grp) {
    KArgs p = kargs_fresh();
#pragma unroll
    for (int i = 0; i < 16; ++i) { U[i] = p->m.U[i]; Ui[i] = p->m.Ui[i]; }
#pragma unroll
    for (int i = 0; i < 4; ++i) w[i] = p->m.w[grp * 4 + i];
  }
};

struct LaneConst {
  double lr;
  double cN;
  double w;
  int slot;
  int npos;
  const double* e2t;
  double lrn;
  double cn[3];
};

template <int N, class F>
__device__ __forceinline__ void static_for(F&& f) {
  if constexpr (N > 0) {
    static_for<N - 1>(f);
    f(std::integral_constant<int, N - 1>{});
  }
}
constexpr int dpp_pos(int k, int x) { return (k >> 1) * 8 + (k & 1) * 3 + x - 1; }
template <int N>
__device__ __forceinline__ void fmac_bcast(double& acc, double t, double s) {
  asm("v_fmac_f64_dpp %0, %1, %2 row_newbcast:%3 row_mask:0xf bank_mask:0xf" : "+v"(acc) : "v"(t), "v"(s), "i"(N));
}
__device__ __forceinline__ void dpp_ready(double& a, double& b, double& c) {
  asm("s_nop 1" : "+v"(a), "+v"(b), "+v"(c));
}
__device__ __forceinline__ void dpp_rows23_upper(double& a, double& b, double& c) {
  int al = __double2loint(a), ah = __double2hiint(a), bl = __double2loint(b), bh = __double2hiint(b);
  int cl = __double2loint(c), ch = __double2hiint(c);
  asm("s_nop 1\n\t"
      "v_mov_b32_dpp %0, %0 row_ror:8 row_mask:0xc bank_mask:0xf\n\t"
      "v_mov_b32_dpp %1, %1 row_ror:8 row_mask:0xc bank_mask:0xf\n\t"
      "v_mov_b32_dpp %2, %2 row_ror:8 row_mask:0xc bank_mask:0xf\n\t"
      "v_mov_b32_dpp %3, %3 row_ror:8 row_mask:0xc bank_mask:0xf\n\t"
      "v_mov_b32_dpp %4, %4 row_ror:8 row_mask:0xc bank_mask:0xf\n\t"
      "v_mov_b32_dpp %5, %5 row_ror:8 row_mask:0xc bank_mask:0xf"
      : "+v"(al), "+v"(ah), "+v"(bl), "+v"(bh), "+v"(cl), "+v"(ch));
  a = __hiloint2double(ah, al);
  b = __hiloint2double(bh, bl);
  c = __hiloint2double(ch, cl);
  dpp_ready(a, b, c);
}

__device__ __forceinline__ void lds_pair(const double* p, double& a, double& b) {
  const double2 v = *reinterpret_cast<const double2*>(__builtin_assume_aligned(p, 16));
  a = v.x;
  b = v.y;
}

__device__ __forceinline__ void table_publish(double* tab, int lane, double v) {
  tab[lane] = v;
  __builtin_amdgcn_fence(__ATOMIC_RELEASE, "wavefront");
  __builtin_amdgcn_wave_barrier();
  __builtin_amdgcn_fence(__ATOMIC_ACQUIRE, "wavefront");
}

// ... 382 lines not shown
  wave_sum2(fl, dfl, f, df);
  cb.sum2(f, df, lane);
}

template <int NCH, bool ZERO0, int NW, bool TAILH = false, int NG = 1>
__device__ __forceinline__ double window_lnl(const SiteState<NCH>& st, const double (&ew)[16], Comb<NW, NG>& cb,
                                             int lane, const double* tab = nullptr) {
  double mant = 1.0;
  int ex = 0;
  double lsite[NCH];
#pragma unroll
  for (int ch = 0; ch < NCH; ++ch) {
    double l0 = ZERO0 ? st.S[ch][0] : 0.0;
    if (TAILH && ch == NCH - 1) {
      const double* ewh = tab + 32 + ((lane >> 5) << 3);
      double eh[8];
#pragma unroll
      for (int i = 0; i < 4; ++i) lds_pair(ewh + 2 * i, eh[2 * i], eh[2 * i + 1]);
#pragma unroll
      for (int i = 0; i < 8; ++i)
        if (!(ZERO0 && (i & 3) == 0)) l0 = fma(st.S[ch][i], eh[i], l0);
      l0 = xhalf_add(l0);
    } else {
#pragma unroll
      for (int i = 0; i < 16; ++i)
        if (!(ZERO0 && (i & 3) == 0)) l0 = fma(st.S[ch][i], ew[i], l0);
    }
    lsite[ch] = l0;
  }
  cb.template groups<NCH>(lsite, lane);
#pragma unroll
  for (int ch = 0; ch < NCH; ++ch) {
    double l0 = lsite[ch];
    bool mine = st.valid[ch];
    if (TAILH && ch == NCH - 1) mine = mine && lane < 32;
    if (!mine) l0 = 1.0;
    const int sc = mine ? (int)(st.sc[ch] + st.resc[ch]) : 0;
    mant *= __builtin_amdgcn_frexp_mant(l0);
    ex += __builtin_amdgcn_frexp_exp(l0) - 256 * sc;
    if ((ch & 7) == 7) {
      ex += __builtin_amdgcn_frexp_exp(mant);
      mant = __builtin_amdgcn_frexp_mant(mant);
    }
  }
  double v = wave_sum(log(mant) + (double)ex * 0.6931471805599453094), z = 0.0;
  cb.sum2(v, z, lane);
  return v;
}

template <int NCH, bool ZERO0, int NW, bool TAILH = false, int NG = 1, bool TDPP = false>
__device__ __forceinline__ double newton(const SiteState<NCH>& st, double* tab, int lane,
                                         const LaneConst& lc, Comb<NW, NG>& cb, double x1, double xguess,
                                         double x2, double tol, int max_iters, uint32_t& evals) {
  double rts = xguess, f, df, xl, xh, dx;
  if (rts < x1) rts = x1;
  if (rts > x2) rts = x2;
  derivatives<NCH, ZERO0, NW, TAILH, NG, TDPP>(st, tab, lane, lc, cb, rts, f, df);
  ++evals;
  if (!isfinite(f) || !isfinite(df)) return NAN;
  if (df >= 0.0 && fabs(f) < tol) return rts;
  if (f < 0.0) { xl = rts; xh = x2; } else { xh = rts; xl = x1; }
  for (int i = 1; i <= max_iters; ++i) {
    if (df <= 0.0 || (((rts - xh) * df - f) * ((rts - xl) * df - f) >= 0.0)) {
      dx = 0.5 * (xh - xl);
      rts = xl + dx;
      if (xl == rts) return rts;
    } else {
      dx = f / df;
      const double temp = rts;
      rts -= dx;
      if (temp == rts) return rts;
    }
    if (fabs(dx) < tol || i == max_iters) return rts;
    if (rts < x1) rts = x1;
    derivatives<NCH, ZERO0, NW, TAILH, NG, TDPP>(st, tab, lane, lc, cb, rts, f, df);
    ++evals;
    if (!isfinite(f) || !isfinite(df)) return NAN;
    if (df > 0.0 && fabs(f) < tol) return rts;
    if (f < 0.0) xl = rts; else xh = rts;
  }
  return NAN;
}

template <int NCH, bool ZERO0, bool INV, int NW, bool LOCAL, bool TAILH = false, int NG = 1, bool TDPP = false>
__device__ __forceinline__ void process_pair(const ThArgs& a, const uint64_t pidx, const int lane,
                                             double* tab, const double* qts, double* qa, const LaneConst& lc,
                                             Comb<NW, NG>& cb, uint32_t (&wstat)[3]) {
  static_assert(NG == 1 || NW == 1, "category groups and site blocks do not combine");
  const uint32_t site0 = NW > 1 ? (uint32_t)cb.wv * NCH * 64 : 0u;
  const uint32_t grp = NG > 1 ? (uint32_t)cb.wv : 0u;
  const uint64_t pid = a.order ? a.order[pidx] : pidx;
  const epa_pair pr = a.pairs[pid];
  const uint32_t b = (uint32_t)__builtin_amdgcn_readfirstlane((int)pr.branch_id);
  const uint32_t q = (uint32_t)__builtin_amdgcn_readfirstlane((int)pr.seq_id);
  const uint32_t begin = (uint32_t)__builtin_amdgcn_readfirstlane((int)a.win_begin[q]);
  const uint32_t n = (uint32_t)__builtin_amdgcn_readfirstlane((int)a.win_span[q]);
  const size_t cW = a.W;
  const char* ref = reinterpret_cast<const char*>(a.refT + ((size_t)(2 * b) * NG + grp) * 16 * cW + begin);
  const uint32_t W8 = a.W * 8u;
  const uint32_t* scp = a.scSum + (size_t)b * cW + begin;
  const uint8_t* qc = a.codes + (size_t)q * a.cstride + (a.crel ? 0u : begin);
  const double orig = a.blen[b];

  SiteState<NCH> st;
  const uint32_t half = TAILH ? (uint32_t)lane >> 5 : 0u;
  const uint32_t hoff = half * 8u * W8;
  double* const tabh = tab + (half << 3);
  auto lane_site = [&](int ch) -> uint32_t {
    return site0 + ch * 64 + ((TAILH && ch == NCH - 1) ? (uint32_t)lane & 31u : (uint32_t)lane);
  };
#pragma unroll
  for (int ch = 0; ch < NCH; ++ch) {
    const uint32_t s = lane_site(ch);
    st.valid[ch] = (NW == 1 && ch < NCH - 1) ? true : s < n;
    const uint32_t sc = st.valid[ch] ? s : 0;
    st.sc[ch] = scp[sc];
    st.code[ch] = qc[sc];
    st.resc[ch] = 0;
  }

  double tp = a.blo.pendant_default, td = orig * 0.5, tx = orig * 0.5;
  uint32_t evals = 0, rounds = 0, reverted = 0;
  uint32_t chain = 0;

  auto cinv_of = [&](int ch) -> double {
    const uint32_t s = st.valid[ch] ? lane_site(ch) : 0;
    const double v = a.cinv[begin + s] * a.inv_w0;
    if (NG > 1 && grp != 0) return 0.0;
    return (TAILH && ch == NCH - 1 && half) ? 0.0 : v;
  };
  const char* refi_s = reinterpret_cast<const char*>(a.refI + ((size_t)b * NG + grp) * 16 * cW + begin);
  auto stream_phase = [&](auto mode_c) {
    constexpr int MODE = decltype(mode_c)::value;
    constexpr int DEPTH = TH_STREAM_DEPTH;
    constexpr int NKL = TAILH ? 2 : 4;
    constexpr int NS = 4 * (NCH - 1) + NKL;
    constexpr int R = DEPTH + 1;
    PhaseModel pm;
    pm.load(grp);
    uint32_t W8p = W8;
    asm volatile("" : "+s"(W8p));
    double An[R][4], Bn[R][4];
    uint32_t soff[NCH], sidx[NCH];
#pragma unroll
    for (int ch = 0; ch < NCH; ++ch) {
      sidx[ch] = st.valid[ch] ? lane_site(ch) : 0;
      soff[ch] = sidx[ch] * 8u + ((TAILH && ch == NCH - 1) ? hoff : 0u);
    }
    uint32_t tok = chain;
    if constexpr (MODE == 1 || MODE == 3) {
      const int kq = lane & 3;
      const double* qv = qts + (lane >> 2) * 4;
      const double* e0 = tab + kq * 4;
      double av[4];
#pragma unroll
      for (int x = 0; x < 4; ++x) av[x] = qv[x] * e0[x];
      double* dst = qa + (lane >> 2) * QA_STRIDE + kq * 4;
#pragma unroll
      for (int i = 0; i < 4; ++i) {
        double v = pm.U[i * 4] * av[0];
#pragma unroll
        for (int x = 1; x < 4; ++x) v = fma(pm.U[i * 4 + x], av[x], v);
        dst[i] = v;
      }
      __builtin_amdgcn_fence(__ATOMIC_RELEASE, "wavefront");
      __builtin_amdgcn_wave_barrier();
      __builtin_amdgcn_fence(__ATOMIC_ACQUIRE, "wavefront");
    }
    auto issue = [&](int stp, uint32_t tk) {
      const int ch = stp >> 2, k = stp & 3, sl = stp % R;
      const uint32_t s0 = soff[ch] + tk;
#pragma unroll
      for (int x = 0; x < 4; ++x) {
        if (MODE == 2) An[sl][x] = *reinterpret_cast<const double*>(refi_s + (s0 + (uint32_t)(k * 4 + x) * W8p));
        else {
          An[sl][x] = *reinterpret_cast<const double*>(ref + (s0 + (uint32_t)(16 * NG + k * 4 + x) * W8p));
          Bn[sl][x] = *reinterpret_cast<const double*>(ref + (s0 + (uint32_t)(k * 4 + x) * W8p));
        }
      }
    };
#pragma unroll
    for (int p = 0; p < DEPTH; ++p)
      if (p < NS) issue(p, tok);
    int mx = 0;
    double qf[4];
#pragma unroll
    for (int stp = 0; stp < NS; ++stp) {
      const int ch = stp >> 2, k = stp & 3, sl = stp % R;
      const bool halfc = TAILH && ch == NCH - 1;
      const int NK = halfc ? 2 : 4;
      const double* tb = halfc ? tabh : tab;
      if (k == 0) {
        const double* qv = qts + st.code[ch] * 4;
        qf[0] = qv[0]; qf[1] = qv[1]; qf[2] = qv[2]; qf[3] = qv[3];
      }
      if (stp + DEPTH < NS) issue(stp + DEPTH, tok);
      asm volatile("" ::: "memory");
      double It[4];
      if (MODE == 2) {
#pragma unroll
        for (int x = 0; x < 4; ++x) It[x] = An[sl][x];
      } else if (MODE == 0) {
        cat_inner(pm, An[sl], tb + k * 4 + 2 * tok, Bn[sl], tb + 16 + k * 4 + 2 * tok, It, mx);
      } else {
        const double* ap = qa + st.code[ch] * QA_STRIDE + ((halfc ? (int)half * 2 : 0) + k) * 4 + 2 * tok;
        double Ap[4];
        lds_pair(ap, Ap[0], Ap[1]); lds_pair(ap + 2, Ap[2], Ap[3]);
        cat_inner_pre(pm, Ap, MODE == 1 ? Bn[sl] : An[sl], tb + 16 + k * 4 + 2 * tok, It, mx);
      }
#pragma unroll
      for (int x = 0; x < 4; ++x)
        st.S[ch][k * 4 + x] = It[x] * ((MODE == 0 || MODE == 2) ? qf[x] : (MODE == 1 ? An[sl][x] : Bn[sl][x]));
      tok = zero_after(st.S[ch][k * 4 + 3]);
      if (k == NK - 1) {
        if (MODE == 2) {
          st.resc[ch] = (a.resc0 + (size_t)b * cW + begin)[sidx[ch]];
        } else {
          int mxs = mx;
          if (halfc) {
            const auto sw = __builtin_amdgcn_permlane32_swap(mx, mx, false, false);
            mxs = max((int)sw[0], (int)sw[1]);
          }
          if constexpr (NG > 1) {
            double mv[1] = {(double)mxs};
            cb.template groups<1, true>(mv, lane);
            mxs = (int)mv[0];
          }
          const uint32_t resc = (mxs < 0x2ff00000) ? 1u : 0u;
          if (__builtin_amdgcn_ballot_w64(resc != 0) != 0) {
            const double mult = resc ? 0x1p+256 : 1.0;
#pragma unroll
            for (int i = 0; i < 16; ++i)
              if (i < NK * 4) st.S[ch][i] *= mult;
          }
          if (MODE == 0) st.resc[ch] = resc;
          mx = 0;
        }
        if constexpr (INV) st.S[ch][0] += cinv_of(ch);
        if constexpr (ZERO0) {
          if (halfc) st.S[ch][0] = fma(half ? pm.w[3] : pm.w[1], st.S[ch][4], (half ? pm.w[2] : pm.w[0]) * st.S[ch][0]);
          else st.S[ch][0] = fma(pm.w[3], st.S[ch][12], fma(pm.w[2], st.S[ch][8], fma(pm.w[1], st.S[ch][4], pm.w[0] * st.S[ch][0])));
        }
        tok = zero_after(st.S[ch][halfc ? 7 : 15]);
      }
    }
    chain = tok;
  };
  auto product_phase = [&](auto mode_c) { stream_phase(mode_c); };
  auto window_score = [&]() -> double {
    double ew[16];
#pragma unroll
    for (int i = 0; i < 8; ++i) lds_pair(tab + 32 + 2 * i, ew[2 * i], ew[2 * i + 1]);
    return window_lnl<NCH, ZERO0, NW, TAILH, NG>(st, ew, cb, lane, tab);
  };
  auto score = [&](double td_, double tx_, double tp_) -> double {
    const double tl = lc.slot == 0 ? td_ : (lc.slot == 1 ? tx_ : tp_);
    table_publish(tab, lane, TH_EXP(lc.lr * tl) * (lc.slot == 2 ? lc.w : 1.0));
    product_phase(std::integral_constant<int, 0>{});
    return window_score();
  };
  auto side_sumtable = [&](double tp_, double tother_, auto toward_prox) {
    constexpr bool TOWARD_PROX = decltype(toward_prox)::value;
    table_publish(tab, lane, TH_EXP(lc.lr * (lc.slot == 0 ? tp_ : tother_)));
    product_phase(std::integral_constant<int, TOWARD_PROX ? 3 : 1>{});
  };
  auto distal_sumtable = [&](double tp_, double tx_) { side_sumtable(tp_, tx_, std::false_type{}); };

  auto score_first = [&](double tp_) -> double {
    table_publish(tab, lane, TH_EXP(lc.lr * tp_) * (lc.slot == 2 ? lc.w : 1.0));
    stream_phase(std::integral_constant<int, 2>{});
    return window_score();
  };

  double loglikelihood = a.refI ? -score_first(tp) : -score(td, tx, tp);

  uint32_t smoothings = a.blo.max_rounds;
  if constexpr (LOCAL) {
    const double xmin = a.blo.min_branch, xmax = a.blo.max_branch, xtol = xmin / 10.0;
    auto solve = [&](double cur) -> double {
      double g = cur;
      if (g < xmin || g > xmax) g = a.blo.default_branch;
      const double r = newton<NCH, ZERO0, NW, TAILH, NG, TDPP>(st, tab, lane, lc, cb, xmin, g, xmax, xtol, (int)a.blo.max_newton, evals);
      chain = zero_after(r);
      return (isfinite(r) && fabs(cur - r) > 1e-10) ? r : cur;
    };
    while (smoothings) {
      tp = solve(tp);
      side_sumtable(tp, tx, std::false_type{});
      td = solve(td);
      side_sumtable(tp, td, std::true_type{});
      tx = solve(tx);
      (void)score(td, tx, tp);
      tp = solve(tp);
      table_publish(tab, lane, TH_EXP(lc.lr * tp) * (lc.slot == 2 ? lc.w : 1.0));
      double ew[16];
#pragma unroll
      for (int i = 0; i < 8; ++i) lds_pair(tab + 32 + 2 * i, ew[2 * i], ew[2 * i + 1]);
      const double new_ll = -window_lnl<NCH, ZERO0, NW, TAILH, NG>(st, ew, cb, lane, tab);
      ++rounds;
      --smoothings;
      if (fabs(new_ll - loglikelihood) < a.blo.epsilon) smoothings = 0;
      loglikelihood = new_ll;
    }
  }
  while (!LOCAL && smoothings) {
    const double old_td = td, old_tp = tp;
    double xmin = a.blo.min_branch, xmax = a.blo.max_branch, xtol = xmin / 10.0;
    double xguess = tp;
    if (xguess < xmin || xguess > xmax) xguess = a.blo.default_branch;
    double xres = newton<NCH, ZERO0, NW, TAILH, NG, TDPP>(st, tab, lane, lc, cb, xmin, xguess, xmax, xtol, (int)a.blo.max_newton, evals);
    if (xres > 0.0) tp = xres;
    chain = zero_after(tp);
    distal_sumtable(tp, tx);
    xguess = td;
    xmin = fmin(a.blo.min_branch / 2.0, orig / 2.0);
    xtol = xmin / 10.0;
    xmax = orig - xtol;
    if (xguess < xmin || xguess > xmax) xguess = orig / 2.0;
    xres = newton<NCH, ZERO0, NW, TAILH, NG, TDPP>(st, tab, lane, lc, cb, xmin, xguess, xmax, xtol, (int)a.blo.max_newton, evals);
    if (xres > 0.0) { td = xres; tx = orig - xres; }
    chain = zero_after(td);
    const double new_ll = -score(td, tx, tp);
    ++rounds;
    if (new_ll - loglikelihood > new_ll * 1e-14) {
      tp = old_tp; td = old_td; tx = orig - old_td;
      reverted = 1;
      break;
    }
    --smoothings;
    if (fabs(new_ll - loglikelihood) < a.blo.epsilon) smoothings = 0;
    loglikelihood = new_ll;
  }

  if (lane == 0 && ((NW == 1 && NG == 1) || cb.wv == 0)) {
    const double lnl = -loglikelihood;
    epa_result r;
    r.lnl = lnl;
    r.pendant_length = tp;
    r.distal_length = (orig / (td + tx)) * td;
    a.out[pid] = r;
    if (!isfinite(lnl)) {
      if (atomicAdd(&a.stats[3], 1ull) == 0) a.stats[4] = ((unsigned long long)b << 32) | q;
    }
  }
  wstat[0] += rounds;
  wstat[1] += evals;
  wstat[2] += reverted;
}

template <int NCH, bool ZERO0, bool INV, int NW, bool LOCAL = false, bool TAILH = false, int NG = 1, bool TDPP = false>
__global__ void __launch_bounds__(64 * NW * NG, TH_WAVES) k_thorough_dna(const ThArgs a) {
  constexpr int NWV = NW * NG;
  __shared__ __attribute__((aligned(16))) double tab[64 * NWV];
  __shared__ __attribute__((aligned(16))) double qts[64];
  __shared__ double red[2 * NW * 2];
  __shared__ double e2t[64];
  __shared__ __attribute__((aligned(16))) double qa[(16 * QA_STRIDE) * NWV];
  __shared__ double xch[NG > 1 ? 2 * NG * Comb<NW, NG>::XCH_MAX * 64 : 1];
  const int lane = threadIdx.x & 63;
  Comb<NW, NG> cb{red, (int)(threadIdx.x >> 6), 0, xch, 0};
  if (threadIdx.x < 64) {
    qts[lane] = a.qt[lane];
    e2t[lane] = exp2((double)lane * 0.015625);
  }
  LaneConst lc;
  lc.e2t = e2t;
  {
    const int lk = (lane >> 2) & 3, lx = lane & 3;
    const int kg = (NG > 1 ? cb.wv * 4 : 0) + lk;
    lc.slot = lane >> 4;
    lc.lr = a.m.lam[lx] * a.m.rate[kg];
    lc.w = a.m.w[kg];
    lc.cN = lc.slot == 0 ? lc.w : (lc.slot == 1 ? lc.w * lc.lr : (lc.slot == 2 ? lc.w * lc.lr * lc.lr : 0.0));
    const int dump = lc.slot == 3 ? 36 + (lane & 15) : 52 + lc.slot * 4 + lk;
    lc.npos = (lc.slot < 3 && lx != 0) ? lc.slot * 12 + lk * 3 + lx - 1 : dump;
  }
  if constexpr (TDPP) {
    const int p = lane & 15, q = p & 7;
    const int kn = q < 6 ? 2 * (p >> 3) + q / 3 : 0, xn = q % 3 + 1;
    const double wn = q < 6 ? a.m.w[kn] : 0.0;
    lc.lrn = q < 6 ? a.m.lam[xn] * a.m.rate[kn] : 0.0;
    lc.cn[0] = wn;
    lc.cn[1] = wn * lc.lrn;
    lc.cn[2] = wn * lc.lrn * lc.lrn;
  }
  __syncthreads();
  const uint32_t x = blockIdx.x & 7;
  const uint32_t w = blockIdx.x >> 3, stride = gridDim.x >> 3;
  uint64_t n_pairs = a.n_pairs;
  if constexpr (NW == 1 && NG == 1) {
    if (a.spec) {
      const uint32_t n = a.spec[0];
      if (n > a.spec_max || a.spec[9 + a.spec_cls] != n || a.spec[32] || a.spec[33]) return;
      n_pairs = n;
    }
  }
  const uint64_t per = (n_pairs + 7) / 8;
  uint64_t lo = (uint64_t)x * per;
  uint64_t hi = lo + per < n_pairs ? lo + per : n_pairs;
  if constexpr (NW == 1 && NG == 1) {
    lo = (n_pairs * a.xcum[x]) >> 20;
    hi = (n_pairs * a.xcum[x + 1]) >> 20;
    if (a.xstamp && blockIdx.x == 0 && threadIdx.x == 0) a.stats[7] = __builtin_amdgcn_s_memrealtime() & EPA_XSTAMP_MASK;
  }
  const unsigned long long clk0 = __builtin_amdgcn_s_memtime(), rt0 = __builtin_amdgcn_s_memrealtime();
  uint32_t wstat[3] = {0, 0, 0};
  if constexpr (NW == 1 && NG == 1) {
    uint32_t* ctr = a.qctr + x;
    const uint32_t cnt = (uint32_t)(hi > lo ? hi - lo : 0);
    uint32_t nxt = 0;
#ifdef TH_TIMING
    unsigned long long* tlog = reinterpret_cast<unsigned long long*>(a.sscratch) + (size_t)blockIdx.x * 8;
    unsigned long long t_first = 0, t_second = 0;
    uint32_t npr = 0;
    if (lane == 0) tlog[0] = __builtin_amdgcn_s_memrealtime();
#endif
    if (lane == 0) nxt = atomicAdd(ctr, 1u);
    nxt = (uint32_t)__builtin_amdgcn_readfirstlane((int)nxt);
    while (nxt < cnt) {
      const uint32_t cur = nxt;
      uint32_t f = 0;
      if (lane == 0) f = atomicAdd(ctr, 1u);
      process_pair<NCH, ZERO0, INV, NW, LOCAL, TAILH, NG, TDPP>(a, lo + cur, lane, tab + cb.wv * 64, qts, qa + cb.wv * (16 * QA_STRIDE), lc, cb, wstat);
      nxt = (uint32_t)__builtin_amdgcn_readfirstlane((int)f);
#ifdef TH_TIMING
      ++npr;
      if (npr == 1) t_first = __builtin_amdgcn_s_memrealtime();
      if (npr == 2) t_second = __builtin_amdgcn_s_memrealtime();
#endif
    }
#ifdef TH_TIMING
    if (lane == 0) { tlog[1] = t_first; tlog[2] = t_second; tlog[3] = __builtin_amdgcn_s_memrealtime(); tlog[4] = npr; }
#endif
  } else {
    for (uint64_t p = lo + w; p < hi; p += stride)
      process_pair<NCH, ZERO0, INV, NW, LOCAL, TAILH, NG, TDPP>(a, p, lane, tab + cb.wv * 64, qts, qa + cb.wv * (16 * QA_STRIDE), lc, cb, wstat);
  }
  if (threadIdx.x == 0) {
    atomicAdd(&a.stats[0], (unsigned long long)wstat[0]);
    atomicAdd(&a.stats[1], (unsigned long long)wstat[1]);
    atomicAdd(&a.stats[2], (unsigned long long)wstat[2]);
    if constexpr (NW == 1 && NG == 1) {
      if (a.xstamp) atomicMax(&a.stats[8 + x], ((unsigned long long)(__builtin_amdgcn_s_memrealtime() & EPA_XSTAMP_MASK) << 21) |
                                                   (unsigned long long)(a.xcum[x + 1] - a.xcum[x]));
    }
    if (a.xstamp && blockIdx.x == 0) {
      a.stats[5] = __builtin_amdgcn_s_memtime() - clk0;
      a.stats[6] = __builtin_amdgcn_s_memrealtime() - rt0;
    }
  }
}

#ifdef TH_ONLY_MAIN
template __global__ void k_thorough_dna<3, true, false, 1, false, true, 1>(const ThArgs a);
template __global__ void k_thorough_dna<3, true, false, 1, false, true, 1, true>(const ThArgs a);
}
#else
template <class Deriv>
__device__ __forceinline__ double newton_fn(Deriv&& deriv, double x1, double xguess, double x2, double tol,
                                            int max_iters, uint32_t& evals) {
  double rts = xguess, f, df, xl, xh, dx;
  if (rts < x1) rts = x1;
  if (rts > x2) rts = x2;
  deriv(rts, f, df);
  ++evals;
  if (!isfinite(f) || !isfinite(df)) return NAN;
  if (df >= 0.0 && fabs(f) < tol) return rts;
  if (f < 0.0) { xl = rts; xh = x2; } else { xh = rts; xl = x1; }
  for (int i = 1; i <= max_iters; ++i) {
    if (df <= 0.0 || (((rts - xh) * df - f) * ((rts - xl) * df - f) >= 0.0)) {
      dx = 0.5 * (xh - xl);
      rts = xl + dx;
      if (xl == rts) return rts;
    } else {
      dx = f / df;
      const double temp = rts;
      rts -= dx;
      if (temp == rts) return rts;
    }
    if (fabs(dx) < tol || i == max_iters) return rts;
    if (rts < x1) rts = x1;
    deriv(rts, f, df);
    ++evals;
    if (!isfinite(f) || !isfinite(df)) return NAN;
    if (df > 0.0 && fabs(f) < tol) return rts;
    if (f < 0.0) xl = rts; else xh = rts;
  }
  return NAN;
}

template <bool ZERO0>
__global__ void __launch_bounds__(64, 2) k_thorough_dna_long(const ThArgs a) {
  __shared__ double tab[64];
  __shared__ double qts[64];
  __shared__ double e2t[64];
  const int lane = threadIdx.x;
  qts[lane] = a.qt[lane];
  e2t[lane] = exp2((double)lane * 0.015625);
  LaneConst lc;
  lc.e2t = e2t;
  {
    const int lk = (lane >> 2) & 3, lx = lane & 3;
    lc.slot = lane >> 4;
    lc.lr = a.m.lam[lx] * a.m.rate[lk];
    lc.w = a.m.w[lk];
    lc.cN = lc.slot == 0 ? lc.w : (lc.slot == 1 ? lc.w * lc.lr : (lc.slot == 2 ? lc.w * lc.lr * lc.lr : 0.0));
  }
  __syncthreads();
  const ModelDNA& m = a.m;
  double* slab = a.sscratch + (size_t)blockIdx.x * 17 * a.Wpad;
  const size_t cW = a.W;
  uint32_t wrounds = 0, wevals = 0, wreverts = 0;
  for (uint64_t pidx = blockIdx.x; pidx < a.n_pairs; pidx += gridDim.x) {
    const uint64_t pid = a.order ? a.order[pidx] : pidx;
    const epa_pair pr = a.pairs[pid];
    const uint32_t b = pr.branch_id, q = pr.seq_id;
    const uint32_t begin = a.win_begin[q], n = a.win_span[q];
    const uint32_t nch = (n + 63) / 64;
    const double* Xt = a.refT + (size_t)(2 * b) * 16 * cW + begin;
    const double* Dt = a.refT + (size_t)(2 * b + 1) * 16 * cW + begin;
    const uint32_t* scp = a.scSum + (size_t)b * cW + begin;
    const uint8_t* qc = a.codes + (size_t)q * a.cstride + (a.crel ? 0u : begin);
    const double orig = a.blen[b];

    auto score = [&](double td_, double tx_, double tp_, bool first) -> double {
      const double tl = lc.slot == 0 ? td_ : (lc.slot == 1 ? tx_ : tp_);
      table_publish(tab, lane, TH_EXP(lc.lr * tl) * (lc.slot == 2 ? lc.w : 1.0));
      double ew[16];
#pragma unroll
      for (int i = 0; i < 16; ++i) ew[i] = tab[32 + i];
      double mant = 1.0;
      int ex = 0;
      for (uint32_t ch = 0; ch < nch; ++ch) {
        const uint32_t site = ch * 64 + lane;
        const bool valid = site < n;
        const uint32_t s = valid ? site : 0;
        double It[16];
        uint32_t resc;
        if (first) {
// ... 52 lines not shown
            slab[(size_t)c * a.Wpad + site] = D[c] * It[c] + ((a.cinv && c == 0) ? a.cinv[begin + s] * a.inv_w0 : 0.0);
        }
      }
      __threadfence_block();
    };
    auto deriv = [&](double t, double& f, double& df) {
      table_publish(tab, lane, TH_EXP(lc.lr * t) * lc.cN);
      double e[16], e1[16], e2[16];
#pragma unroll
      for (int i = 0; i < 16; ++i) { e[i] = tab[i]; e1[i] = tab[16 + i]; e2[i] = tab[32 + i]; }
      double fl = 0.0, dfl = 0.0;
      for (uint32_t ch = 0; ch < nch; ++ch) {
        const uint32_t site = ch * 64 + lane;
        const bool valid = site < n;
        const uint32_t s = valid ? site : 0;
        double l0 = 0.0, l1 = 0.0, l2 = 0.0;
#pragma unroll
        for (int i = 0; i < 16; ++i) {
          const double sv = slab[(size_t)i * a.Wpad + s];
          l0 = fma(sv, e[i], l0);
          if (!(ZERO0 && (i & 3) == 0)) { l1 = fma(sv, e1[i], l1); l2 = fma(sv, e2[i], l2); }
        }
        const double inv = fast_rcp(l0);
        const double d1 = -l1 * inv;
        const double d2 = fma(d1, d1, -l2 * inv);
        if (valid) { fl += d1; dfl += d2; }
      }
      f = wave_sum(fl);
      df = wave_sum(dfl);
    };

    double tp = a.blo.pendant_default, td = orig * 0.5, tx = orig * 0.5;
    uint32_t evals = 0, rounds = 0, reverted = 0;
    double loglikelihood = -score(td, tx, tp, a.refI != nullptr);
    uint32_t smoothings = a.blo.max_rounds;
    while (smoothings) {
      const double old_td = td, old_tp = tp;
      double xmin = a.blo.min_branch, xmax = a.blo.max_branch, xtol = xmin / 10.0;
      double xguess = tp;
      if (xguess < xmin || xguess > xmax) xguess = a.blo.default_branch;
      double xres = newton_fn(deriv, xmin, xguess, xmax, xtol, (int)a.blo.max_newton, evals);
      if (xres > 0.0) tp = xres;
      distal_sumtable(tp, tx);
      xguess = td;
      xmin = fmin(a.blo.min_branch / 2.0, orig / 2.0);
      xtol = xmin / 10.0;
      xmax = orig - xtol;
      if (xguess < xmin || xguess > xmax) xguess = orig / 2.0;
      xres = newton_fn(deriv, xmin, xguess, xmax, xtol, (int)a.blo.max_newton, evals);
      if (xres > 0.0) { td = xres; tx = orig - xres; }
      const double new_ll = -score(td, tx, tp, false);
      ++rounds;
      if (new_ll - loglikelihood > new_ll * 1e-14) {
        tp = old_tp; td = old_td; tx = orig - old_td;
        reverted = 1;
        break;
      }
      --smoothings;
      if (fabs(new_ll - loglikelihood) < a.blo.epsilon) smoothings = 0;
      loglikelihood = new_ll;
    }
    if (lane == 0) {
      const double lnl = -loglikelihood;
      epa_result r;
      r.lnl = lnl;
      r.pendant_length = tp;
      r.distal_length = (orig / (td + tx)) * td;
      a.out[pid] = r;
      if (!isfinite(lnl)) {
        if (atomicAdd(&a.stats[3], 1ull) == 0) a.stats[4] = ((unsigned long long)b << 32) | q;
      }
    }
    wrounds += rounds; wevals += evals; wreverts += reverted;
  }
  if (lane == 0) {
    atomicAdd(&a.stats[0], (unsigned long long)wrounds);
    atomicAdd(&a.stats[1], (unsigned long long)wevals);
    atomicAdd(&a.stats[2], (unsigned long long)wreverts);
  }
}

}

namespace {

__global__ void __launch_bounds__(256) k_pair_class(const epa_pair* __restrict__ pairs, uint64_t n,
                                                   const uint32_t* __restrict__ win_span, int states,
                                                   uint32_t* __restrict__ keys, uint32_t* __restrict__ idx,
                                                   uint32_t* __restrict__ hist) {
  const uint64_t i = (uint64_t)blockIdx.x * 256 + threadIdx.x;
  const int cls = i < n ? epa_span_class(states, win_span[pairs[i].seq_id]) : -1;
  if (i < n) {
    if (keys) { keys[i] = (uint32_t)cls; idx[i] = (uint32_t)i; }
  }
  if (hist) {
    for (int c = 0; c < EPA_N_CLS; ++c) {
      const unsigned long long bal = __ballot(cls == c);
      if (bal && (threadIdx.x & 63) == 0) atomicAdd(&hist[c], (uint32_t)__popcll(bal));
    }
  }
}

template <int NCH, bool ZERO0, bool INV, int NW, bool LOCAL = false, bool TAILH = false>
void launch_dna(const epa_ctx* ctx, uint32_t nwg, const ThArgs& a) {
  if constexpr (ZERO0 && NW == 1 && !LOCAL && TH_WAVES < 3) {
    if (!ctx->opt.newton_lds) {
      hipLaunchKernelGGL((k_thorough_dna<NCH, ZERO0, INV, NW, LOCAL, TAILH, 1, true>), dim3(nwg), dim3(64), 0, ctx->stream, a);
      return;
    }
  }
  hipLaunchKernelGGL((k_thorough_dna<NCH, ZERO0, INV, NW, LOCAL, TAILH>), dim3(nwg), dim3(64 * NW), 0, ctx->stream, a);
}

}

static int launch_thorough_dna_class(epa_ctx* ctx, ThArgs a, int cls, uint32_t max_span) {
  const uint64_t n_pairs = a.n_pairs;
  uint32_t per_slot = (uint32_t)std::min<uint64_t>(32, std::max<uint64_t>(8, n_pairs / (2048 * 4)));
  constexpr uint64_t th_grid_waves = 0;
#ifdef TH_TIMING
#define TH_TIMING_ALLOC a.sscratch = (double*)epa_scratch(ctx, 9, 2048 * 64); (void)hipMemsetAsync(a.sscratch, 0, 2048 * 64, ctx->stream);
#define TH_TIMING_DUMP th_timing_dump(ctx, a.sscratch);
#else
#define TH_TIMING_ALLOC
#define TH_TIMING_DUMP
#endif
#define LAUNCH(N, NW_)                                                                            \
  do {                                                                                            \
    uint64_t want = (uint64_t)256 * 8 * per_slot / (NW_);                                          \
    a.qctr = nullptr;                                                                              \
    if ((NW_) == 1) {                                                                              \
      TH_TIMING_ALLOC                                                                              \
      { const int zr_ = epa_th_ctr_reset(ctx); if (zr_) return zr_; }                                  \
      a.qctr = epa_th_ctr(ctx);                                                                        \
      want = th_grid_waves ? th_grid_waves : 1024 * TH_WAVES;                                                   \
    }                                                                                              \
    if (want > n_pairs) want = n_pairs;                                                            \
    const uint32_t nwg = (uint32_t)((want + 7) / 8 * 8);                                           \
    constexpr bool TH_ = (NW_) == 1 && ((N) == 2 || (N) == 3);     \
    if (tailh && TH_ && ctx->dna_zero0 && !ctx->blo.sliding && !a.cinv)                                            \
      launch_dna<N, true, false, 1, true, TH_>(ctx, nwg, a);                                                       \
    else if (tailh && TH_ && ctx->dna_zero0 && !ctx->blo.sliding)                         \
      launch_dna<N, true, true, 1, true, TH_>(ctx, nwg, a);                                                        \
    else if (tailh && TH_ && ctx->dna_zero0 && ctx->blo.sliding && a.cinv)                                        \
      launch_dna<N, true, true, 1, false, TH_>(ctx, nwg, a);                                                       \
    else if (tailh && TH_ && ctx->dna_zero0 && ctx->blo.sliding)                                                   \
      launch_dna<N, true, false, 1, false, TH_>(ctx, nwg, a);                                                      \
    else if (!ctx->blo.sliding && a.cinv) launch_dna<N, true, true, NW_, true>(ctx, nwg, a);                       \
    else if (!ctx->blo.sliding) launch_dna<N, true, false, NW_, true>(ctx, nwg, a);                                \
    else if (a.cinv) launch_dna<N, true, true, NW_>(ctx, nwg, a);                                                  \
    else if (ctx->dna_zero0) launch_dna<N, true, false, NW_>(ctx, nwg, a);                                         \
    else launch_dna<N, false, false, NW_>(ctx, nwg, a);                                                            \
  } while (0)
  if (ctx->dna.ng > 1) {
    const bool ok = ctx->blo.sliding && ctx->dna_zero0 && (cls <= 2 || cls == 10 || cls == 11);
    if (!ok) {
      a.Wpad = (std::max(max_span, 1u) + 63) / 64 * 64;
      return launch_thorough_generic(ctx, a.pairs, n_pairs, a.codes, a.win_begin, a.win_span, max_span, a.out,
                                     a.stats, a.order ? a.order : nullptr, true);
    }
    const int nch = cls == 0 ? 1 : (cls == 1 || cls == 10) ? 2 : 3;
    uint64_t want = (uint64_t)256 * 8 * per_slot / (uint64_t)ctx->dna.ng;
    if (want > n_pairs) want = n_pairs;
    const uint32_t nwg = (uint32_t)((want + 7) / 8 * 8);
    a.qctr = nullptr;
#define LAUNCH_G(N, G)                                                                                          \
    do {                                                                                                        \
      if (a.cinv) hipLaunchKernelGGL((k_thorough_dna<N, true, true, 1, false, false, G>), dim3(nwg), dim3(64 * (G)), 0, ctx->stream, a); \
      else hipLaunchKernelGGL((k_thorough_dna<N, true, false, 1, false, false, G>), dim3(nwg), dim3(64 * (G)), 0, ctx->stream, a);       \
    } while (0)
#define LAUNCH_GN(G) do { if (nch == 1) LAUNCH_G(1, G); else if (nch == 2) LAUNCH_G(2, G); else LAUNCH_G(3, G); } while (0)
    if (ctx->dna.ng == 2) LAUNCH_GN(2); else if (ctx->dna.ng == 3) LAUNCH_GN(3); else LAUNCH_GN(4);
#undef LAUNCH_GN
#undef LAUNCH_G
    return EPA_OK;
  }
  const bool tailh = cls == 10 || cls == 11;
  constexpr bool n4_off = false;
  switch (cls) {
    case 0: LAUNCH(1, 1); break;
    case 1: case 10: LAUNCH(2, 1); break;
    case 2: case 11: LAUNCH(3, 1); break;
    case 3: if (n4_off) LAUNCH(2, 2); else LAUNCH(4, 1); break;
    case 4: LAUNCH(3, 2); break;
    case 5: LAUNCH(2, 4); break;
    case 6: LAUNCH(3, 4); break;
    case 7: LAUNCH(2, 8); break;
    case 8: LAUNCH(3, 8); break;
    default: {
      const uint32_t nlong = (uint32_t)std::min<uint64_t>(n_pairs, 2048);
      a.Wpad = (max_span + 63) / 64 * 64;
      a.sscratch = (double*)epa_scratch(ctx, 7, sizeof(double) * (size_t)nlong * 17 * a.Wpad);
      if (!a.sscratch) return epa_fail(ctx, EPA_ERR_HIP, "hipMalloc(long-window sumtable scratch)");
      if (ctx->dna_zero0) hipLaunchKernelGGL((k_thorough_dna_long<true>), dim3(nlong), dim3(64), 0, ctx->stream, a);
      else hipLaunchKernelGGL((k_thorough_dna_long<false>), dim3(nlong), dim3(64), 0, ctx->stream, a);
    }
  }
#undef LAUNCH
#ifdef TH_TIMING
  if (a.sscratch && (cls <= 2 || cls == 10 || cls == 11)) {
    std::vector<unsigned long long> h(2048 * 8);
    (void)hipStreamSynchronize(ctx->stream);
    (void)hipMemcpy(h.data(), a.sscratch, 2048 * 64, hipMemcpyDeviceToHost);
    unsigned long long t0 = ~0ull, t1 = 0;
    for (int w = 0; w < 2048; ++w) if (h[w * 8]) { t0 = std::min(t0, h[w * 8]); t1 = std::max(t1, h[w * 8 + 3]); }
    std::vector<double> st, fp, sp, ex, np_;
    for (int w = 0; w < 2048; ++w) {
      if (!h[w * 8]) continue;
      st.push_back((h[w * 8] - t0) * 0.01);
      if (h[w * 8 + 1]) fp.push_back((h[w * 8 + 1] - h[w * 8]) * 0.01);
      if (h[w * 8 + 2]) sp.push_back((h[w * 8 + 2] - h[w * 8 + 1]) * 0.01);
      ex.push_back((h[w * 8 + 3] - t0) * 0.01);
      np_.push_back((double)h[w * 8 + 4]);
    }
    for (int x = 0; x < 8; ++x) {
      double e0 = 1e30, e1 = 0, fsum = 0; unsigned long long np2 = 0; int nw = 0;
      for (int w = x; w < 2048; w += 8) {
        if (!h[w * 8]) continue;
        const double e = (h[w * 8 + 3] - t0) * 0.01;
        e0 = std::min(e0, e); e1 = std::max(e1, e); np2 += h[w * 8 + 4]; ++nw;
        if (h[w * 8 + 1]) fsum += (h[w * 8 + 1] - h[w * 8]) * 0.01;
      }
      fprintf(stderr, "  x %d: waves %d pairs %llu exit %.1f .. %.1f us, mean first pair %.1f\n", x, nw, np2, e0, e1, nw ? fsum / nw : 0.0);
    }
    auto pct = [](std::vector<double>& v, double p) { if (v.empty()) return 0.0; std::sort(v.begin(), v.end()); return v[(size_t)(p * (v.size() - 1))]; };
    fprintf(stderr, "TH_TIMING n_pairs %llu: span %.1f us | wave start p50 %.1f p99 %.1f max %.1f | first pair p50 %.1f p90 %.1f max %.1f | second pair p50 %.1f p90 %.1f | exit p1 %.1f p10 %.1f p50 %.1f p90 %.1f max %.1f | pairs/wave p50 %.0f max %.0f\n",
            (unsigned long long)a.n_pairs, (t1 - t0) * 0.01, pct(st, 0.5), pct(st, 0.99), pct(st, 1.0), pct(fp, 0.5), pct(fp, 0.9), pct(fp, 1.0), pct(sp, 0.5), pct(sp, 0.9),
            pct(ex, 0.01), pct(ex, 0.1), pct(ex, 0.5), pct(ex, 0.9), pct(ex, 1.0), pct(np_, 0.5), pct(np_, 1.0));
  }
#endif
  return EPA_OK;
}

static ThArgs dna_args(epa_ctx* ctx, const epa_pair* d_pairs, const uint32_t* ord, const uint8_t* d_codes,
                       const uint32_t* d_begin, const uint32_t* d_span, epa_result* d_out, unsigned long long* d_stats) {
  ThArgs a;
  a.m = ctx->dna;
  a.blo = ctx->blo;
  a.refT = ctx->refT;
  a.refI = ctx->lookup_built ? ctx->refI : nullptr;
  a.resc0 = ctx->resc0;
  a.cinv = ctx->cinv;
  a.inv_w0 = ctx->inv_w0;
  a.scSum = ctx->scSum;
  a.blen = ctx->blen;
  a.qt = ctx->dmodel->qt;
  a.pairs = d_pairs;
  a.order = ord;
  a.codes = d_codes;
  a.crel = ctx->code_stride ? 1u : 0u;
  a.cstride = a.crel ? ctx->code_stride : ctx->W;
  a.win_begin = d_begin;
  a.win_span = d_span;
  a.out = d_out;
  a.stats = d_stats;
  a.sscratch = nullptr;
  a.qctr = nullptr;
  a.n_pairs = 0;
  a.W = ctx->W;
  a.Wpad = 0;
  a.spec = nullptr;
  a.spec_cls = 0;
  a.spec_max = 0;
  for (int i = 0; i < 9; ++i) a.xcum[i] = ctx->xcd_cum[i];
  a.xstamp = 0;
  return a;
}

int launch_thorough_queued(epa_ctx* ctx, const epa_pair* d_pairs, const uint32_t* d_spec, uint64_t max_pairs,
                           const uint8_t* d_codes, const uint32_t* d_begin, const uint32_t* d_span, uint32_t max_span,
                           epa_result* d_out, unsigned long long* d_stats) {
  if (ctx->s != 4 || ctx->generic_thorough || ctx->dna.ng != 1 || !epa_th_ctr(ctx) || !d_span || !d_spec) return -1;
  if (max_pairs > 0xffffffffull) return -1;
  const int cls = epa_span_class(4, max_span);
  if (!(cls <= 2 || cls == 10 || cls == 11)) return -1;
  static const uint32_t bound[12] = {64, 128, 192, 0, 0, 0, 0, 0, 0, 0, 96, 160};
  ThArgs a = dna_args(ctx, d_pairs, nullptr, d_codes, d_begin, d_span, d_out, d_stats);
  a.n_pairs = 0xffffffffull;
  a.spec = d_spec;
  a.spec_cls = (uint32_t)cls;
  a.spec_max = (uint32_t)max_pairs;
  a.xstamp = 1u;
  epa_timer_start(ctx, epa_t(ctx, epa_ctx::T_THOROUGH));
  const int rc = launch_thorough_dna_class(ctx, a, cls, std::min(max_span, bound[cls]));
  epa_timer_stop(ctx, epa_t(ctx, epa_ctx::T_THOROUGH));
  if (rc) return -2;
  if (hipGetLastError() != hipSuccess) { (void)epa_fail(ctx, EPA_ERR_HIP, "queued thorough launch"); return -2; }
  return cls;
}

int launch_thorough(epa_ctx* ctx, const epa_pair* d_pairs, uint64_t n_pairs, const uint8_t* d_codes,
                    const uint32_t* d_begin, const uint32_t* d_span, uint32_t max_span,
                    epa_result* d_out, unsigned long long* d_stats, const uint32_t* cls_hist) {
  if (n_pairs > 0xffffffffull) return epa_fail(ctx, EPA_ERR_INVALID_ARG, "thorough: more than 2^32 pairs per call");
  if (ctx->generic_thorough || (!ctx->blo.sliding && ctx->s == 4 && max_span > 1536u)) {
    return launch_thorough_generic(ctx, d_pairs, n_pairs, d_codes, d_begin, d_span, max_span, d_out, d_stats);
  }
  uint32_t hist[EPA_N_CLS] = {};
  const int cmax = epa_span_class(ctx->s, max_span);
  uint64_t given = 0;
  if (cls_hist) for (int c = 0; c < EPA_N_CLS; ++c) given += cls_hist[c];
  const bool cached = cls_hist && given == n_pairs && n_pairs != 0;
  if (cached) {
    for (int c = 0; c < EPA_N_CLS; ++c) hist[c] = cls_hist[c];
  } else if (cmax == 0) {
    hist[0] = (uint32_t)n_pairs;
  }
  size_t temp_bytes = 0;
  (void)rocprim::radix_sort_pairs<epa_radix_cfg>(nullptr, temp_bytes, (uint32_t*)nullptr, (uint32_t*)nullptr,
                                  (uint32_t*)nullptr, (uint32_t*)nullptr, (size_t)n_pairs, 0, 4, ctx->stream);
  const size_t nb = (sizeof(uint32_t) * n_pairs + 255) & ~(size_t)255;
  uint32_t* d_hist = nullptr;
  uint32_t *d_keys = nullptr, *d_idx = nullptr, *d_keys2 = nullptr, *d_order = nullptr;
  auto carve = [&]() -> int {
    char* base = (char*)epa_scratch(ctx, 8, 256 + 4 * nb + temp_bytes);
    if (!base) return epa_fail(ctx, EPA_ERR_HIP, "hipMalloc(span-class scratch)");
    d_hist = (uint32_t*)base;
    d_keys = (uint32_t*)(base + 256); d_idx = (uint32_t*)(base + 256 + nb);
    d_keys2 = (uint32_t*)(base + 256 + 2 * nb); d_order = (uint32_t*)(base + 256 + 3 * nb);
    return EPA_OK;
  };
  const dim3 cgrid((uint32_t)((n_pairs + 255) / 256));
  bool have_keys = false;
  if (!cached && cmax != 0) {
    int rc = carve();
    if (rc) return rc;
    EPA_HIP(ctx, hipMemsetAsync(d_hist, 0, 64, ctx->stream));
    hipLaunchKernelGGL(k_pair_class, cgrid, dim3(256), 0, ctx->stream, d_pairs, n_pairs, d_span, ctx->s, d_keys,
                       d_idx, d_hist);
    EPA_HIP(ctx, hipMemcpyAsync(hist, d_hist, sizeof(hist), hipMemcpyDeviceToHost, ctx->stream));
    EPA_HIP(ctx, hipStreamSynchronize(ctx->stream));
    have_keys = true;
  }
  int present = 0;
  for (int c = 0; c < EPA_N_CLS; ++c) present += hist[c] != 0;
  const uint32_t* order = nullptr;
  if (present > 1) {
    if (!have_keys) {
      int rc = carve();
      if (rc) return rc;
      hipLaunchKernelGGL(k_pair_class, cgrid, dim3(256), 0, ctx->stream, d_pairs, n_pairs, d_span, ctx->s,
                         d_keys, d_idx, (uint32_t*)nullptr);
    }
    void* temp = (char*)d_order + nb;
    EPA_HIP(ctx, rocprim::radix_sort_pairs<epa_radix_cfg>(temp, temp_bytes, d_keys, d_keys2, d_idx, d_order, (size_t)n_pairs, 0, 4,
                                           ctx->stream));
    order = d_order;
  }
  epa_timer_start(ctx, epa_t(ctx, epa_ctx::T_THOROUGH));
  int rc = EPA_OK;
  uint64_t off = 0;
  ctx->xstamp_ok = present == 1;
  static const uint32_t dna_bound[EPA_N_CLS] = {64, 128, 192, 256, 384, 512, 768, 1024, 1536, 0xffffffffu, 96, 160};
  for (int c = 0; c < EPA_N_CLS && rc == EPA_OK; ++c) {
    if (!hist[c]) continue;
    const uint32_t* ord = order ? order + off : nullptr;
    off += hist[c];
    if (ctx->s == 20) {
      static const uint32_t aa_bound[4] = {64, 128, 192, 0xffffffffu};
      const bool aa_valu = ctx->opt.aa_valu != 0;
      const uint32_t bound = std::min(max_span, aa_bound[c < 4 ? c : 3]);
      const uint32_t mfma_max = ctx->c == 4 ? 384u : 256u;
      if (bound <= mfma_max && (!aa_valu || !ctx->blo.sliding || ctx->c != 4))
        rc = launch_thorough_aa_mfma(ctx, d_pairs, ord, hist[c], d_codes, d_begin, d_span, bound, d_out, d_stats);
      else if (ctx->c == 4 && ctx->blo.sliding)
        rc = launch_thorough_aa(ctx, d_pairs, ord, hist[c], d_codes, d_begin, d_span, bound,
                                bound <= EPA_AA_LDS_MAX_SPAN, d_out, d_stats);
      else
        rc = launch_thorough_generic(ctx, d_pairs, hist[c], d_codes, d_begin, d_span, bound, d_out, d_stats, ord, true);
      continue;
    }
    ThArgs a = dna_args(ctx, d_pairs, ord, d_codes, d_begin, d_span, d_out, d_stats);
    a.n_pairs = hist[c];
    a.xstamp = (present == 1 && ctx->dna.ng == 1 && (c <= 2 || c == 10 || c == 11)) ? 1u : 0u;
    rc = launch_thorough_dna_class(ctx, a, c, std::min(max_span, dna_bound[c]));
  }
  epa_timer_stop(ctx, epa_t(ctx, epa_ctx::T_THOROUGH));
  if (rc) return rc;
  EPA_HIP(ctx, hipGetLastError());
  return EPA_OK;
}
#endif
```

profiles/dpp_hazard_check.py:

```python
#!/usr/bin/env python3
import os
import re
import subprocess
import sys
import tempfile

ROOT = os.path.dirname(os.path.dirname(os.path.abspath(__file__)))
LLVM = "/opt/rocm/lib/llvm/bin/"
obj = os.path.join(ROOT, "epa_ng_amd", "build", "thorough_dna.o")
with tempfile.TemporaryDirectory() as d:
    fat, co = os.path.join(d, "fat.bin"), os.path.join(d, "k.co")
    subprocess.check_call([LLVM + "llvm-objcopy", "--dump-section", ".hip_fatbin=" + fat, obj])
    subprocess.check_call([LLVM + "clang-offload-bundler", "--unbundle", "--type=o", "--input=" + fat,
                           "--targets=hipv4-amdgcn-amd-amdhsa--gfx950", "--output=" + co])
    asm = subprocess.check_output([LLVM + "llvm-objdump", "-d", co], text=True)


def vregs(op):
    m = re.match(r"v\[(\d+):(\d+)\]", op.strip())
    if m:
        return set(range(int(m.group(1)), int(m.group(2)) + 1))
    m = re.match(r"v(\d+)$", op.strip())
    return {int(m.group(1))} if m else set()


ins = []
for l in asm.split("\n"):
    if re.match(r"^[0-9a-f]+ <", l):
        ins.append(None)
        continue
    m = re.match(r"\s+(\S+)\s*(.*?)\s*//", l)
    if m:
        ins.append((m.group(1), m.group(2)))
ndpp = bad = 0
for i, x in enumerate(ins):
    if x is None or "row_newbcast" not in x[1] and "row_ror" not in x[1]:
        continue
    ndpp += 1
    src0 = vregs(x[1].split(",")[1])
    ws, j = 0, i - 1
    while ws < 5 and j >= 0 and ins[j] is not None:
        op, args = ins[j]
        if op == "s_nop":
            ws += int(args.split()[0], 0) + 1
        else:
            dst = args.split(",")[0] if args else ""
            if ws < 2 and op.startswith("v_") and vregs(dst) & src0:
                bad += 1
                print("VGPR write -> DPP read: %s %s  ->  %s %s" % (op, args, x[0], x[1]))
            if "exec" in dst:
                bad += 1
                print("EXEC write -> DPP: %s %s  ->  %s %s" % (op, args, x[0], x[1]))
            ws += 1
        j -= 1
print("row_newbcast / row_ror instructions: %d, unpadded hazards: %d" % (ndpp, bad))
sys.exit(1 if bad else 0)
```

Before: 17.07 million placements/s.

## Specialize thorough DNA kernels for tip-distal branches using precomputed tip tables

Keeps the reference tip characters as 4-bit masks and builds a 64-entry table of Ui-projected tip vectors. Pairs whose distal node is a tip are split into extra span classes and run with a TIPD kernel variant. That variant reads the per-site tip mask and skips loading the distal CLV from the reference array. Tip-class launches go to a side stream with fork/join events so they can overlap the regular classes. The change adds more kernel instantiations, a sort over five key bits, extra class bookkeeping in readback, and more stream-synchronisation complexity.

Measured after the change: 17.71 million placements/s, median of 6. 1.04x the previous value.

```diff
diff --git a/epa_ng_amd/build.py b/epa_ng_amd/build.py
--- a/epa_ng_amd/build.py
+++ b/epa_ng_amd/build.py
@@ -7,9 +7,11 @@
 CSRC = os.path.join(HERE, "csrc")
 HIPCC = os.environ.get("HIPCC", "/opt/rocm/bin/hipcc")
 
-DEV_SOURCES = ["epa_dev.hip", "preplace.hip", "thorough_dna.hip", "thorough_aa.hip", "thorough_aa_mfma.hip", "thorough_generic.hip", "score_at.hip", "marginal.hip", "rell.hip", "comm.hip"]
+DEV_SOURCES = ["epa_dev.hip", "preplace.hip", "thorough_dna.hip", "thorough_dna_tipd.hip", "thorough_dna_tipd2h.hip", "thorough_aa.hip", "thorough_aa_mfma.hip", "thorough_generic.hip", "score_at.hip", "marginal.hip", "rell.hip", "comm.hip"]
 EXTRA_FLAGS = {"thorough_dna.hip": ["-mllvm", "-amdgpu-sched-strategy=iterative-ilp"],
+               "thorough_dna_tipd.hip": ["-mllvm", "-amdgpu-sched-strategy=iterative-ilp"],
                "thorough_aa_mfma.hip": ["-mllvm", "-amdgpu-sched-strategy=iterative-ilp"]}
+EXTRA_DEPS = {"thorough_dna_tipd.hip": ["thorough_dna.hip"], "thorough_dna_tipd2h.hip": ["thorough_dna.hip"]}
 DEV_FLAGS = ["--offload-arch=gfx950", "-O3", "-std=c++17", "-fPIC", "-I", os.path.join(ROOT, "include"),
              "-I", CSRC, "-Wall", "-Wno-unused-function", "-Wno-unused-result"]
 
@@ -32,7 +34,7 @@
         sp = os.path.join(CSRC, src)
         op = os.path.join(objdir, src.replace(".hip", ".o"))
         objs.append(op)
-        if force or _newer(op, [sp] + hdrs):
+        if force or _newer(op, [sp] + hdrs + [os.path.join(CSRC, d) for d in EXTRA_DEPS.get(src, [])]):
             cmd = [HIPCC] + DEV_FLAGS + EXTRA_FLAGS.get(src, []) + ["-c", sp, "-o", op]
             if verbose:
                 print(" ".join(cmd), file=sys.stderr)
diff --git a/epa_ng_amd/csrc/epa_dev.hip b/epa_ng_amd/csrc/epa_dev.hip
--- a/epa_ng_amd/csrc/epa_dev.hip
+++ b/epa_ng_amd/csrc/epa_dev.hip
@@ -579,7 +579,7 @@
       {"select_full_rows", &EpaOptions::select_full_rows}, {"select_sort", &EpaOptions::select_sort},
       {"queued_thorough", &EpaOptions::queued_thorough},   {"xcd_balance", &EpaOptions::xcd_balance},
       {"aa_valu", &EpaOptions::aa_valu},                   {"timers", &EpaOptions::timers},
-      {"newton_lds", &EpaOptions::newton_lds}};
+      {"newton_lds", &EpaOptions::newton_lds},             {"tip_distal", &EpaOptions::tip_distal}};
   for (const Entry& e : table)
     if (strcmp(key, e.name) == 0) {
       ctx->opt.*e.field = value;
@@ -675,6 +675,12 @@
   if (ctx->refI) (void)hipFree(ctx->refI);
   if (ctx->cinv) (void)hipFree(ctx->cinv);
   if (ctx->resc0) (void)hipFree(ctx->resc0);
+  if (ctx->tip_row) (void)hipFree(ctx->tip_row);
+  if (ctx->tipmask) (void)hipFree(ctx->tipmask);
+  if (ctx->tipd) (void)hipFree(ctx->tipd);
+  for (hipStream_t st : ctx->side_stream) if (st) (void)hipStreamDestroy(st);
+  for (hipEvent_t e : ctx->ev_fork) if (e) (void)hipEventDestroy(e);
+  for (hipEvent_t e : ctx->ev_join) if (e) (void)hipEventDestroy(e);
   if (ctx->dmodel) (void)hipFree(ctx->dmodel);
   for (ChunkSlot& sl : ctx->slots) {
     if (sl.h_in) (void)hipHostFree(sl.h_in);
@@ -1149,6 +1155,19 @@
   }
 }
 
+__global__ void __launch_bounds__(256) k_tip_masks(uint8_t* __restrict__ tipchars, const uint32_t* __restrict__ tipmap, size_t n) {
+  const size_t i = (size_t)blockIdx.x * blockDim.x + threadIdx.x;
+  if (i < n) tipchars[i] = (uint8_t)(tipmap[tipchars[i]] & 15u);
+}
+__global__ void __launch_bounds__(64) k_tip_table(const ModelDev* __restrict__ m, double* __restrict__ tipd) {
+  const int s = m->s;
+  const uint32_t mask = threadIdx.x >> 2;
+  const int x = threadIdx.x & 3;
+  double acc = 0.0;
+  for (int i = 0; i < s; ++i) if ((mask >> i) & 1u) acc += m->Ui[x * s + i];
+  tipd[threadIdx.x] = acc;
+}
+
 __global__ void k_scaler_sum(const uint32_t* __restrict__ sc_side, uint32_t* __restrict__ scSum, size_t n,
                              uint32_t W) {
   const size_t i = (size_t)blockIdx.x * blockDim.x + threadIdx.x;
@@ -1292,9 +1311,20 @@
     const size_t nbw = (size_t)B * W;
     hipLaunchKernelGGL(k_scaler_sum, dim3((uint32_t)((nbw + 255) / 256)), blk, 0, ctx->stream, d_sc, ctx->scSum, nbw, W);
   }
+  const bool keep_tips = ctx->s == 4 && !ctx->generic_native;
+  if (keep_tips) {
+    TREE_HIP(hipMalloc(&ctx->tipd, sizeof(double) * 64));
+    hipLaunchKernelGGL(k_tip_table, dim3(1), dim3(64), 0, ctx->stream, ctx->dmodel, ctx->tipd);
+    const size_t nt = (size_t)n * W;
+    hipLaunchKernelGGL(k_tip_masks, dim3((uint32_t)((nt + 255) / 256)), blk, 0, ctx->stream, d_tips, d_tipmap, nt);
+  }
   TREE_HIP(hipStreamSynchronize(ctx->stream));
   TREE_HIP(hipGetLastError());
 #undef TREE_HIP
+  if (keep_tips) {
+    ctx->tipmask = d_tips; d_tips = nullptr;
+    ctx->tip_row = d_tob; d_tob = nullptr;
+  }
   cleanup();
   return EPA_OK;
 }
@@ -1800,7 +1830,7 @@
   rc = select_check_status(ctx, sp);
   if (rc) return rc;
   *n_out = n;
-  if (sp->queued_cls >= 0 && sp->rb[9 + sp->queued_cls] == (uint32_t)n) return EPA_OK;
+  if (sp->queued_cls >= 0 && sp->rb[9 + sp->queued_cls] + sp->rb[9 + epa_tip_class(sp->queued_cls)] == (uint32_t)n) return EPA_OK;
   if (ctx->clean_stats[ctx->bank] == d_stats && sp->queued_cls < 0) ctx->clean_stats[ctx->bank] = nullptr;
   else {
     ctx->clean_stats[ctx->bank] = nullptr;
@@ -1808,8 +1838,9 @@
     if (rc) return rc;
   }
   if (n == 0) return EPA_OK;
+  const bool hist_ok = sp->have_hist && (sp->tip_split || !epa_tipd_active(ctx));
   return launch_thorough(ctx, d_pairs, n, d_codes, d_begin, d_span, max_span, d_res, d_stats,
-                         sp->have_hist ? sp->cls_hist : nullptr);
+                         hist_ok ? sp->cls_hist : nullptr);
 }
 
 static int chunk_body(epa_ctx* ctx, const uint8_t* d_codes, const uint32_t* d_begin, const uint32_t* d_span,
diff --git a/epa_ng_amd/csrc/epa_dev_internal.hpp b/epa_ng_amd/csrc/epa_dev_internal.hpp
--- a/epa_ng_amd/csrc/epa_dev_internal.hpp
+++ b/epa_ng_amd/csrc/epa_dev_internal.hpp
@@ -67,8 +67,9 @@
   const uint32_t* d_rb = nullptr;
   bool emitted = false;
   int queued_cls = -1;
-  uint32_t cls_hist[16] = {};
+  uint32_t cls_hist[24] = {};
   bool have_hist = false;
+  bool tip_split = false;
   const uint32_t* pre_status = nullptr;
 };
 
@@ -134,6 +135,7 @@
   int aa_valu = 0;
   int timers = 1;
   int newton_lds = 0;
+  int tip_distal = 1;
 };
 
 struct epa_ctx {
@@ -166,6 +168,9 @@
   double* cinv = nullptr;
   double inv_w0 = 0.0;
   double* lookup2 = nullptr;
+  uint32_t* tip_row = nullptr;
+  uint8_t* tipmask = nullptr;
+  double* tipd = nullptr;
   bool lookup_built = false;
   bool lookup_blocks = false;
   uint32_t lookup_block = 1024;
@@ -204,6 +209,8 @@
   double last_sclk_mhz = 0.0;
   bool xstamp_ok = false;
   hipEvent_t ev_rb[N_BANKS] = {};
+  hipStream_t side_stream[N_BANKS] = {};
+  hipEvent_t ev_fork[N_BANKS] = {}, ev_join[N_BANKS] = {};
   const void* clean_stats[N_BANKS] = {};
   bool clean_ctr[N_BANKS] = {};
   int t_last[N_TIMERS] = {};
@@ -214,9 +221,9 @@
 void* epa_scratch(epa_ctx* ctx, int slot, size_t bytes);
 inline uint32_t* epa_th_ctr(epa_ctx* ctx) { return ctx->th_ctr ? ctx->th_ctr + 64 * ctx->bank : nullptr; }
 int epa_zero_async(epa_ctx* ctx, void* p, size_t bytes, void* p2 = nullptr, size_t bytes2 = 0);
-inline int epa_th_ctr_reset(epa_ctx* ctx) {
+inline int epa_th_ctr_reset(epa_ctx* ctx, size_t bytes = 64) {
   if (ctx->clean_ctr[ctx->bank]) { ctx->clean_ctr[ctx->bank] = false; return 0; }
-  return epa_zero_async(ctx, epa_th_ctr(ctx), 64);
+  return epa_zero_async(ctx, epa_th_ctr(ctx), bytes);
 }
 bool epa_is_device_ptr(const void* p);
 const void* epa_to_device(epa_ctx* ctx, int slot, const void* p, size_t bytes);
@@ -236,6 +243,14 @@
   } while (0)
 
 constexpr int EPA_N_CLS = 12;
+constexpr int EPA_N_CLSX = 17;
+__host__ __device__ inline bool epa_tip_class_ok(int cls) { return cls <= 2 || cls == 10 || cls == 11; }
+__host__ __device__ inline int epa_tip_class(int cls) { return cls <= 2 ? 12 + cls : cls == 10 ? 15 : cls == 11 ? 16 : cls; }
+__host__ __device__ inline int epa_base_class(int key) { return key < 12 ? key : key <= 14 ? key - 12 : key == 15 ? 10 : 11; }
+inline bool epa_tipd_active(const epa_ctx* ctx) {
+  return ctx->tip_row && ctx->opt.tip_distal && ctx->s == 4 && !ctx->generic_thorough && ctx->dna.ng == 1 &&
+         ctx->dna_zero0 && ctx->blo.sliding && !ctx->cinv;
+}
 constexpr uint32_t EPA_AA_LDS_MAX_SPAN = 102;
 __host__ __device__ inline int epa_span_class(int states, uint32_t span) {
   if (states != 4) return span <= 64 ? 0 : span <= 128 ? 1 : span <= 192 ? 2 : 3;
diff --git a/epa_ng_amd/csrc/preplace.hip b/epa_ng_amd/csrc/preplace.hip
--- a/epa_ng_amd/csrc/preplace.hip
+++ b/epa_ng_amd/csrc/preplace.hip
@@ -48,13 +48,17 @@
   const uint32_t q = blockIdx.x * 256 + threadIdx.x;
   if (q < Q) rank[q] = atomicAdd(&cnt[keys[q]], 1u);
 }
-__global__ void __launch_bounds__(1024) k_scan_counts(uint32_t* __restrict__ cnt, uint32_t K) {
+__global__ void __launch_bounds__(1024) k_scan_counts(uint32_t* __restrict__ cnt, uint32_t K,
+                                                      const uint32_t* __restrict__ tip_row = nullptr,
+                                                      uint32_t* __restrict__ tip_total = nullptr) {
   __shared__ uint32_t wsum[16];
   __shared__ uint32_t carry_s;
+  __shared__ uint32_t tips_s;
   const uint32_t t = threadIdx.x, lane = t & 63u, wv = t >> 6;
-  if (t == 0) carry_s = 0;
+  if (t == 0) { carry_s = 0; tips_s = 0; }
   __syncthreads();
   constexpr uint32_t PER = 8;
+  uint32_t tips = 0;
   for (uint32_t base = 0; base < K; base += 1024 * PER) {
     uint32_t v[PER], tot = 0;
 #pragma unroll
@@ -62,6 +66,7 @@
       const uint32_t k = base + t * PER + i;
       v[i] = k < K ? cnt[k] : 0u;
       tot += v[i];
+      if (tip_row && k + 1 < K && tip_row[k] != 0xffffffffu) tips += v[i];
     }
     uint32_t inc = tot;
 #pragma unroll
@@ -83,6 +88,11 @@
     __syncthreads();
     if (t == 1023) carry_s = run;
     __syncthreads();
+  }
+  if (tip_total) {
+    if (tips) atomicAdd(&tips_s, tips);
+    __syncthreads();
+    if (t == 0) *tip_total = tips_s;
   }
 }
 __global__ void __launch_bounds__(256) k_scatter_sorted(const uint32_t* __restrict__ keys,
@@ -1513,11 +1523,26 @@
 __global__ void __launch_bounds__(64) k_pack_readback(const uint32_t* __restrict__ status,
                                                      const uint32_t* __restrict__ total,
                                                      const uint32_t* __restrict__ pre_status,
-                                                     uint32_t* __restrict__ out) {
+                                                     uint32_t* __restrict__ out,
+                                                     const uint32_t* __restrict__ tip_total = nullptr) {
   const uint32_t t = threadIdx.x;
   if (t == 0) out[0] = *total;
   if (t < 8 + EPA_N_CLS) out[1 + t] = status[t];
+  else if (t < 8 + EPA_N_CLSX) out[1 + t] = 0u;
+  if (t == 30) out[30] = 0u;
   if (t < 4) out[32 + t] = pre_status ? pre_status[t] : 0u;
+  __syncthreads();
+  if (tip_total && t == 0) {
+    int one = -1, n = 0;
+    for (int c = 0; c < EPA_N_CLS; ++c)
+      if (status[8 + c]) { one = c; ++n; }
+    if (n == 1 && epa_tip_class_ok(one)) {
+      const uint32_t all = status[8 + one], tips = min(*tip_total, all);
+      out[9 + one] = all - tips;
+      out[9 + epa_tip_class(one)] = tips;
+      out[30] = 1u;
+    }
+  }
 }
 
 __global__ void __launch_bounds__(256) k_compact(const unsigned long long* __restrict__ stage,
@@ -1847,12 +1872,14 @@
     else if (nr <= 256) hipLaunchKernelGGL(k_select_wg<64>, dim3(Q), dim3(256), 0, ctx->stream, d_lnl, Q, B, pitch, threshold, mode, limit, so, counts, status);
     else hipLaunchKernelGGL(k_select_stream, dim3(Q), dim3(256), 0, ctx->stream, d_lnl, Q, B, pitch, threshold, stream_band, mode, limit, so, counts, status);
 #undef SEL
-    hipLaunchKernelGGL(k_scan_counts, dim3(1), dim3(1024), 0, ctx->stream, bcount, B + 1);
+    const bool tipd = epa_tipd_active(ctx) && d_span != nullptr;
+    hipLaunchKernelGGL(k_scan_counts, dim3(1), dim3(1024), 0, ctx->stream, bcount, B + 1,
+                       tipd ? (const uint32_t*)ctx->tip_row : (const uint32_t*)nullptr, tipd ? status + 40 : (uint32_t*)nullptr);
     if (d_span && !seg_hist)
       hipLaunchKernelGGL(k_class_hist, dim3((Q + 255) / 256), dim3(256), 0, ctx->stream, counts, d_span, Q,
                          ctx->s, status + 8);
     hipLaunchKernelGGL(k_pack_readback, dim3(1), dim3(64), 0, ctx->stream, status, bcount + B,
-                       sp->pre_status, status + 64);
+                       sp->pre_status, status + 64, tipd ? (const uint32_t*)(status + 40) : (const uint32_t*)nullptr);
     EPA_HIP(ctx, hipMemcpyAsync(rb, status + 64, sizeof(uint32_t) * 36, hipMemcpyDeviceToHost, ctx->stream));
     sp->have_status = sp->pre_status != nullptr;
     if (!ctx->ev_rb[ctx->bank]) EPA_HIP(ctx, hipEventCreateWithFlags(&ctx->ev_rb[ctx->bank], hipEventDisableTiming));
@@ -1954,8 +1981,9 @@
     EPA_HIP(ctx, hipGetLastError());
     *n_pairs = total;
     if (sp->d_span) {
-      for (int c = 0; c < EPA_N_CLS; ++c) sp->cls_hist[c] = hst[8 + c];
+      for (int c = 0; c < EPA_N_CLSX; ++c) sp->cls_hist[c] = hst[8 + c];
       sp->have_hist = true;
+      sp->tip_split = sp->rb[30] != 0;
     }
     return EPA_OK;
   }
diff --git a/epa_ng_amd/csrc/thorough_dna.hip b/epa_ng_amd/csrc/thorough_dna.hip
--- a/epa_ng_amd/csrc/thorough_dna.hip
+++ b/epa_ng_amd/csrc/thorough_dna.hip
@@ -44,6 +44,9 @@
   uint32_t spec_cls, spec_max;
   uint32_t xcum[9];
   uint32_t xstamp;
+  const uint32_t* tip_row;
+  const uint8_t* tipmask;
+  const double* tipd;
 };
 
 using namespace epa_wave;
@@ -592,11 +595,12 @@
   return NAN;
 }
 
-template <int NCH, bool ZERO0, bool INV, int NW, bool LOCAL, bool TAILH = false, int NG = 1, bool TDPP = false>
+template <int NCH, bool ZERO0, bool INV, int NW, bool LOCAL, bool TAILH = false, int NG = 1, bool TDPP = false, bool TIPD = false>
 __device__ __forceinline__ void process_pair(const ThArgs& a, const uint64_t pidx, const int lane,
                                              double* tab, const double* qts, double* qa, const LaneConst& lc,
-                                             Comb<NW, NG>& cb, uint32_t (&wstat)[3]) {
+                                             Comb<NW, NG>& cb, uint32_t (&wstat)[3], const double* dts = nullptr) {
   static_assert(NG == 1 || NW == 1, "category groups and site blocks do not combine");
+  static_assert(!TIPD || (ZERO0 && !INV && NW == 1 && !LOCAL && NG == 1), "TIPD exists for the single-wave sliding kernels");
   const uint32_t site0 = NW > 1 ? (uint32_t)cb.wv * NCH * 64 : 0u;
   const uint32_t grp = NG > 1 ? (uint32_t)cb.wv : 0u;
   const uint64_t pid = a.order ? a.order[pidx] : pidx;
@@ -613,6 +617,12 @@
   const double orig = a.blen[b];
 
   SiteState<NCH> st;
+  uint32_t tmk[TIPD ? NCH : 1];
+  const uint8_t* tmp = nullptr;
+  if constexpr (TIPD) {
+    const uint32_t trow = (uint32_t)__builtin_amdgcn_readfirstlane((int)a.tip_row[b]);
+    tmp = a.tipmask + (size_t)trow * cW + begin;
+  }
   const uint32_t half = TAILH ? (uint32_t)lane >> 5 : 0u;
   const uint32_t hoff = half * 8u * W8;
   double* const tabh = tab + (half << 3);
@@ -627,6 +637,7 @@
     st.sc[ch] = scp[sc];
     st.code[ch] = qc[sc];
     st.resc[ch] = 0;
+    if constexpr (TIPD) tmk[ch] = tmp[sc];
   }
 
   double tp = a.blo.pendant_default, td = orig * 0.5, tx = orig * 0.5;
@@ -658,9 +669,10 @@
       soff[ch] = sidx[ch] * 8u + ((TAILH && ch == NCH - 1) ? hoff : 0u);
     }
     uint32_t tok = chain;
-    if constexpr (MODE == 1 || MODE == 3) {
+    constexpr bool TIP0 = TIPD && MODE == 0, TIP1 = TIPD && MODE == 1;
+    if constexpr (MODE == 1 || MODE == 3 || TIP0) {
       const int kq = lane & 3;
-      const double* qv = qts + (lane >> 2) * 4;
+      const double* qv = (TIP0 ? dts : qts) + (lane >> 2) * 4;
       const double* e0 = tab + kq * 4;
       double av[4];
 #pragma unroll
@@ -684,7 +696,7 @@
       for (int x = 0; x < 4; ++x) {
         if (MODE == 2) An[sl][x] = *reinterpret_cast<const double*>(refi_s + (s0 + (uint32_t)(k * 4 + x) * W8p));
         else {
-          An[sl][x] = *reinterpret_cast<const double*>(ref + (s0 + (uint32_t)(16 * NG + k * 4 + x) * W8p));
+          if (!TIP0 && !TIP1) An[sl][x] = *reinterpret_cast<const double*>(ref + (s0 + (uint32_t)(16 * NG + k * 4 + x) * W8p));
           Bn[sl][x] = *reinterpret_cast<const double*>(ref + (s0 + (uint32_t)(k * 4 + x) * W8p));
         }
       }
@@ -694,6 +706,7 @@
       if (p < NS) issue(p, tok);
     int mx = 0;
     double qf[4];
+    double df[TIP1 ? 4 : 1];
 #pragma unroll
     for (int stp = 0; stp < NS; ++stp) {
       const int ch = stp >> 2, k = stp & 3, sl = stp % R;
@@ -703,6 +716,7 @@
       if (k == 0) {
         const double* qv = qts + st.code[ch] * 4;
         qf[0] = qv[0]; qf[1] = qv[1]; qf[2] = qv[2]; qf[3] = qv[3];
+        if constexpr (TIP1) { const double* dv = dts + tmk[ch] * 4; lds_pair(dv, df[0], df[1]); lds_pair(dv + 2, df[2], df[3]); }
       }
       if (stp + DEPTH < NS) issue(stp + DEPTH, tok);
       asm volatile("" ::: "memory");
@@ -710,17 +724,18 @@
       if (MODE == 2) {
 #pragma unroll
         for (int x = 0; x < 4; ++x) It[x] = An[sl][x];
-      } else if (MODE == 0) {
+      } else if (MODE == 0 && !TIP0) {
         cat_inner(pm, An[sl], tb + k * 4 + 2 * tok, Bn[sl], tb + 16 + k * 4 + 2 * tok, It, mx);
       } else {
-        const double* ap = qa + st.code[ch] * QA_STRIDE + ((halfc ? (int)half * 2 : 0) + k) * 4 + 2 * tok;
+        const uint32_t row = TIP0 ? tmk[ch] : st.code[ch];
+        const double* ap = qa + row * QA_STRIDE + ((halfc ? (int)half * 2 : 0) + k) * 4 + 2 * tok;
         double Ap[4];
         lds_pair(ap, Ap[0], Ap[1]); lds_pair(ap + 2, Ap[2], Ap[3]);
-        cat_inner_pre(pm, Ap, MODE == 1 ? Bn[sl] : An[sl], tb + 16 + k * 4 + 2 * tok, It, mx);
+        cat_inner_pre(pm, Ap, (MODE == 1 || TIP0) ? Bn[sl] : An[sl], tb + 16 + k * 4 + 2 * tok, It, mx);
       }
 #pragma unroll
       for (int x = 0; x < 4; ++x)
-        st.S[ch][k * 4 + x] = It[x] * ((MODE == 0 || MODE == 2) ? qf[x] : (MODE == 1 ? An[sl][x] : Bn[sl][x]));
+        st.S[ch][k * 4 + x] = It[x] * ((MODE == 0 || MODE == 2) ? qf[x] : (MODE == 1 ? (TIP1 ? df[x] : An[sl][x]) : Bn[sl][x]));
       tok = zero_after(st.S[ch][k * 4 + 3]);
       if (k == NK - 1) {
         if (MODE == 2) {
@@ -858,7 +873,7 @@
   wstat[2] += reverted;
 }
 
-template <int NCH, bool ZERO0, bool INV, int NW, bool LOCAL = false, bool TAILH = false, int NG = 1, bool TDPP = false>
+template <int NCH, bool ZERO0, bool INV, int NW, bool LOCAL = false, bool TAILH = false, int NG = 1, bool TDPP = false, bool TIPD = false>
 __global__ void __launch_bounds__(64 * NW * NG, TH_WAVES) k_thorough_dna(const ThArgs a) {
   constexpr int NWV = NW * NG;
   __shared__ __attribute__((aligned(16))) double tab[64 * NWV];
@@ -867,11 +882,13 @@
   __shared__ double e2t[64];
   __shared__ __attribute__((aligned(16))) double qa[(16 * QA_STRIDE) * NWV];
   __shared__ double xch[NG > 1 ? 2 * NG * Comb<NW, NG>::XCH_MAX * 64 : 1];
+  __shared__ __attribute__((aligned(16))) double dts[TIPD ? 64 : 2];
   const int lane = threadIdx.x & 63;
   Comb<NW, NG> cb{red, (int)(threadIdx.x >> 6), 0, xch, 0};
   if (threadIdx.x < 64) {
     qts[lane] = a.qt[lane];
     e2t[lane] = exp2((double)lane * 0.015625);
+    if constexpr (TIPD) dts[lane] = a.tipd[lane];
   }
   LaneConst lc;
   lc.e2t = e2t;
@@ -901,7 +918,7 @@
   if constexpr (NW == 1 && NG == 1) {
     if (a.spec) {
       const uint32_t n = a.spec[0];
-      if (n > a.spec_max || a.spec[9 + a.spec_cls] != n || a.spec[32] || a.spec[33]) return;
+      if (n > a.spec_max || a.spec[9 + a.spec_cls] + a.spec[9 + epa_tip_class((int)a.spec_cls)] != n || a.spec[32] || a.spec[33]) return;
       n_pairs = n;
     }
   }
@@ -911,7 +928,7 @@
   if constexpr (NW == 1 && NG == 1) {
     lo = (n_pairs * a.xcum[x]) >> 20;
     hi = (n_pairs * a.xcum[x + 1]) >> 20;
-    if (a.xstamp && blockIdx.x == 0 && threadIdx.x == 0) a.stats[7] = __builtin_amdgcn_s_memrealtime() & EPA_XSTAMP_MASK;
+    if (a.xstamp == 1 && blockIdx.x == 0 && threadIdx.x == 0) a.stats[7] = __builtin_amdgcn_s_memrealtime() & EPA_XSTAMP_MASK;
   }
   const unsigned long long clk0 = __builtin_amdgcn_s_memtime(), rt0 = __builtin_amdgcn_s_memrealtime();
   uint32_t wstat[3] = {0, 0, 0};
@@ -931,7 +948,7 @@
       const uint32_t cur = nxt;
       uint32_t f = 0;
       if (lane == 0) f = atomicAdd(ctr, 1u);
-      process_pair<NCH, ZERO0, INV, NW, LOCAL, TAILH, NG, TDPP>(a, lo + cur, lane, tab + cb.wv * 64, qts, qa + cb.wv * (16 * QA_STRIDE), lc, cb, wstat);
+      process_pair<NCH, ZERO0, INV, NW, LOCAL, TAILH, NG, TDPP, TIPD>(a, lo + cur, lane, tab + cb.wv * 64, qts, qa + cb.wv * (16 * QA_STRIDE), lc, cb, wstat, dts);
       nxt = (uint32_t)__builtin_amdgcn_readfirstlane((int)f);
 #ifdef TH_TIMING
       ++npr;
@@ -954,7 +971,7 @@
       if (a.xstamp) atomicMax(&a.stats[8 + x], ((unsigned long long)(__builtin_amdgcn_s_memrealtime() & EPA_XSTAMP_MASK) << 21) |
                                                    (unsigned long long)(a.xcum[x + 1] - a.xcum[x]));
     }
-    if (a.xstamp && blockIdx.x == 0) {
+    if (a.xstamp == 1 && blockIdx.x == 0) {
       a.stats[5] = __builtin_amdgcn_s_memtime() - clk0;
       a.stats[6] = __builtin_amdgcn_s_memrealtime() - rt0;
     }
@@ -965,6 +982,31 @@
 template __global__ void k_thorough_dna<3, true, false, 1, false, true, 1>(const ThArgs a);
 template __global__ void k_thorough_dna<3, true, false, 1, false, true, 1, true>(const ThArgs a);
 }
+#elif defined(TH_TIPD_UNIT)
+}
+#if TH_TIPD_UNIT == 2
+void launch_dna_tipd2h(hipStream_t stream, uint32_t nwg, const void* args) {
+  const ThArgs& a = *static_cast<const ThArgs*>(args);
+  hipLaunchKernelGGL((k_thorough_dna<2, true, false, 1, false, true, 1, true, true>), dim3(nwg), dim3(64), 0, stream, a);
+}
+#else
+void launch_dna_tipd2h(hipStream_t stream, uint32_t nwg, const void* args);
+void launch_dna_tipd(hipStream_t stream, int nch, bool tailh, bool newton_lds, uint32_t nwg, const void* args) {
+  const ThArgs& a = *static_cast<const ThArgs*>(args);
+  if (nch == 2 && tailh && !newton_lds) { launch_dna_tipd2h(stream, nwg, args); return; }
+#define TIPD_L(N, TH)                                                                                                        \
+  do {                                                                                                                      \
+    if (newton_lds) hipLaunchKernelGGL((k_thorough_dna<N, true, false, 1, false, TH, 1, false, true>), dim3(nwg), dim3(64), 0, stream, a); \
+    else hipLaunchKernelGGL((k_thorough_dna<N, true, false, 1, false, TH, 1, true, true>), dim3(nwg), dim3(64), 0, stream, a);           \
+  } while (0)
+  if (nch == 1) TIPD_L(1, false);
+  else if (nch == 2 && tailh) hipLaunchKernelGGL((k_thorough_dna<2, true, false, 1, false, true, 1, false, true>), dim3(nwg), dim3(64), 0, stream, a);
+  else if (nch == 2) TIPD_L(2, false);
+  else if (tailh) TIPD_L(3, true);
+  else TIPD_L(3, false);
+#undef TIPD_L
+}
+#endif
 #else
 template <class Deriv>
 __device__ __forceinline__ double newton_fn(Deriv&& deriv, double x1, double xguess, double x2, double tol,
@@ -1183,19 +1225,25 @@
 
 }
 
+void launch_dna_tipd(hipStream_t stream, int nch, bool tailh, bool newton_lds, uint32_t nwg, const void* args);
+
 namespace {
 
 __global__ void __launch_bounds__(256) k_pair_class(const epa_pair* __restrict__ pairs, uint64_t n,
                                                    const uint32_t* __restrict__ win_span, int states,
+                                                   const uint32_t* __restrict__ tip_row,
                                                    uint32_t* __restrict__ keys, uint32_t* __restrict__ idx,
                                                    uint32_t* __restrict__ hist) {
   const uint64_t i = (uint64_t)blockIdx.x * 256 + threadIdx.x;
-  const int cls = i < n ? epa_span_class(states, win_span[pairs[i].seq_id]) : -1;
+  int cls = -1;
   if (i < n) {
+    const epa_pair pr = pairs[i];
+    cls = epa_span_class(states, win_span[pr.seq_id]);
+    if (tip_row && epa_tip_class_ok(cls) && tip_row[pr.branch_id] != 0xffffffffu) cls = epa_tip_class(cls);
     if (keys) { keys[i] = (uint32_t)cls; idx[i] = (uint32_t)i; }
   }
   if (hist) {
-    for (int c = 0; c < EPA_N_CLS; ++c) {
+    for (int c = 0; c < EPA_N_CLSX; ++c) {
       const unsigned long long bal = __ballot(cls == c);
       if (bal && (threadIdx.x & 63) == 0) atomicAdd(&hist[c], (uint32_t)__popcll(bal));
     }
@@ -1203,7 +1251,13 @@
 }
 
 template <int NCH, bool ZERO0, bool INV, int NW, bool LOCAL = false, bool TAILH = false>
-void launch_dna(const epa_ctx* ctx, uint32_t nwg, const ThArgs& a) {
+void launch_dna(const epa_ctx* ctx, uint32_t nwg, const ThArgs& a, bool tipd = false) {
+  if constexpr (ZERO0 && !INV && NW == 1 && !LOCAL && NCH <= 3 && TH_WAVES < 3) {
+    if (tipd) {
+      launch_dna_tipd(ctx->stream, NCH, TAILH, ctx->opt.newton_lds != 0, nwg, &a);
+      return;
+    }
+  }
   if constexpr (ZERO0 && NW == 1 && !LOCAL && TH_WAVES < 3) {
     if (!ctx->opt.newton_lds) {
       hipLaunchKernelGGL((k_thorough_dna<NCH, ZERO0, INV, NW, LOCAL, TAILH, 1, true>), dim3(nwg), dim3(64), 0, ctx->stream, a);
@@ -1215,8 +1269,11 @@
 
 }
 
-static int launch_thorough_dna_class(epa_ctx* ctx, ThArgs a, int cls, uint32_t max_span) {
+static int launch_thorough_dna_class(epa_ctx* ctx, ThArgs a, int cls, uint32_t max_span, bool tipd = false,
+                                     bool dual = false, bool side_ctr_clean = false) {
   const uint64_t n_pairs = a.n_pairs;
+  if (tipd && !(epa_tip_class_ok(cls) && ctx->dna.ng == 1 && ctx->dna_zero0 && ctx->blo.sliding && !a.cinv))
+    return epa_fail(ctx, EPA_ERR_INVALID_ARG, "thorough: tip-distal launch outside the classes the TIPD kernels serve");
   uint32_t per_slot = (uint32_t)std::min<uint64_t>(32, std::max<uint64_t>(8, n_pairs / (2048 * 4)));
   constexpr uint64_t th_grid_waves = 0;
 #ifdef TH_TIMING
@@ -1232,8 +1289,13 @@
     a.qctr = nullptr;                                                                              \
     if ((NW_) == 1) {                                                                              \
       TH_TIMING_ALLOC                                                                              \
-      { const int zr_ = epa_th_ctr_reset(ctx); if (zr_) return zr_; }                                  \
-      a.qctr = epa_th_ctr(ctx);                                                                        \
+      if (tipd) {                                                                                  \
+        if (!side_ctr_clean) { const int zr_ = epa_zero_async(ctx, epa_th_ctr(ctx) + 8, 32); if (zr_) return zr_; }  \
+        a.qctr = epa_th_ctr(ctx) + 8;                                                              \
+      } else {                                                                                     \
+        { const int zr_ = epa_th_ctr_reset(ctx, dual ? 32 : 64); if (zr_) return zr_; }            \
+        a.qctr = epa_th_ctr(ctx);                                                                  \
+      }                                                                                            \
       want = th_grid_waves ? th_grid_waves : 1024 * TH_WAVES;                                                   \
     }                                                                                              \
     if (want > n_pairs) want = n_pairs;                                                            \
@@ -1246,11 +1308,11 @@
     else if (tailh && TH_ && ctx->dna_zero0 && ctx->blo.sliding && a.cinv)                                        \
       launch_dna<N, true, true, 1, false, TH_>(ctx, nwg, a);                                                       \
     else if (tailh && TH_ && ctx->dna_zero0 && ctx->blo.sliding)                                                   \
-      launch_dna<N, true, false, 1, false, TH_>(ctx, nwg, a);                                                      \
+      launch_dna<N, true, false, 1, false, TH_>(ctx, nwg, a, tipd);                                                \
     else if (!ctx->blo.sliding && a.cinv) launch_dna<N, true, true, NW_, true>(ctx, nwg, a);                       \
     else if (!ctx->blo.sliding) launch_dna<N, true, false, NW_, true>(ctx, nwg, a);                                \
     else if (a.cinv) launch_dna<N, true, true, NW_>(ctx, nwg, a);                                                  \
-    else if (ctx->dna_zero0) launch_dna<N, true, false, NW_>(ctx, nwg, a);                                         \
+    else if (ctx->dna_zero0) launch_dna<N, true, false, NW_>(ctx, nwg, a, tipd);                                   \
     else launch_dna<N, false, false, NW_>(ctx, nwg, a);                                                            \
   } while (0)
   if (ctx->dna.ng > 1) {
@@ -1365,6 +1427,9 @@
   a.spec_max = 0;
   for (int i = 0; i < 9; ++i) a.xcum[i] = ctx->xcd_cum[i];
   a.xstamp = 0;
+  a.tip_row = ctx->tip_row;
+  a.tipmask = ctx->tipmask;
+  a.tipd = ctx->tipd;
   return a;
 }
 
@@ -1397,19 +1462,22 @@
   if (ctx->generic_thorough || (!ctx->blo.sliding && ctx->s == 4 && max_span > 1536u)) {
     return launch_thorough_generic(ctx, d_pairs, n_pairs, d_codes, d_begin, d_span, max_span, d_out, d_stats);
   }
-  uint32_t hist[EPA_N_CLS] = {};
+  uint32_t hist[EPA_N_CLSX] = {};
   const int cmax = epa_span_class(ctx->s, max_span);
+  const bool tipd = epa_tipd_active(ctx) && TH_WAVES < 3;
+  const uint32_t* tip_row = tipd ? ctx->tip_row : nullptr;
   uint64_t given = 0;
-  if (cls_hist) for (int c = 0; c < EPA_N_CLS; ++c) given += cls_hist[c];
+  if (cls_hist) for (int c = 0; c < EPA_N_CLSX; ++c) given += cls_hist[c];
   const bool cached = cls_hist && given == n_pairs && n_pairs != 0;
   if (cached) {
-    for (int c = 0; c < EPA_N_CLS; ++c) hist[c] = cls_hist[c];
-  } else if (cmax == 0) {
+    for (int c = 0; c < EPA_N_CLSX; ++c) hist[c] = cls_hist[c];
+  } else if (cmax == 0 && !tipd) {
     hist[0] = (uint32_t)n_pairs;
   }
   size_t temp_bytes = 0;
   (void)rocprim::radix_sort_pairs<epa_radix_cfg>(nullptr, temp_bytes, (uint32_t*)nullptr, (uint32_t*)nullptr,
-                                  (uint32_t*)nullptr, (uint32_t*)nullptr, (size_t)n_pairs, 0, 4, ctx->stream);
+                                  (uint32_t*)nullptr, (uint32_t*)nullptr, (size_t)n_pairs, 0, 5, ctx->stream);
+  auto sp_tips = [](const uint32_t* h) { for (int c = EPA_N_CLS; c < EPA_N_CLSX; ++c) if (h[c]) return true; return false; };
   const size_t nb = (sizeof(uint32_t) * n_pairs + 255) & ~(size_t)255;
   uint32_t* d_hist = nullptr;
   uint32_t *d_keys = nullptr, *d_idx = nullptr, *d_keys2 = nullptr, *d_order = nullptr;
@@ -1423,58 +1491,85 @@
   };
   const dim3 cgrid((uint32_t)((n_pairs + 255) / 256));
   bool have_keys = false;
-  if (!cached && cmax != 0) {
+  if (!cached && (cmax != 0 || tipd)) {
     int rc = carve();
     if (rc) return rc;
-    EPA_HIP(ctx, hipMemsetAsync(d_hist, 0, 64, ctx->stream));
-    hipLaunchKernelGGL(k_pair_class, cgrid, dim3(256), 0, ctx->stream, d_pairs, n_pairs, d_span, ctx->s, d_keys,
+    EPA_HIP(ctx, hipMemsetAsync(d_hist, 0, 128, ctx->stream));
+    hipLaunchKernelGGL(k_pair_class, cgrid, dim3(256), 0, ctx->stream, d_pairs, n_pairs, d_span, ctx->s, tip_row, d_keys,
                        d_idx, d_hist);
     EPA_HIP(ctx, hipMemcpyAsync(hist, d_hist, sizeof(hist), hipMemcpyDeviceToHost, ctx->stream));
     EPA_HIP(ctx, hipStreamSynchronize(ctx->stream));
     have_keys = true;
   }
-  int present = 0;
-  for (int c = 0; c < EPA_N_CLS; ++c) present += hist[c] != 0;
+  int present = 0, spans = 0;
+  for (int c = 0; c < EPA_N_CLSX; ++c) present += hist[c] != 0;
+  for (int c = 0; c < EPA_N_CLS; ++c) spans += (hist[c] != 0 || (epa_tip_class_ok(c) && hist[epa_tip_class(c)] != 0));
   const uint32_t* order = nullptr;
   if (present > 1) {
     if (!have_keys) {
       int rc = carve();
       if (rc) return rc;
       hipLaunchKernelGGL(k_pair_class, cgrid, dim3(256), 0, ctx->stream, d_pairs, n_pairs, d_span, ctx->s,
-                         d_keys, d_idx, (uint32_t*)nullptr);
+                         sp_tips(hist) ? ctx->tip_row : tip_row, d_keys, d_idx, (uint32_t*)nullptr);
     }
     void* temp = (char*)d_order + nb;
-    EPA_HIP(ctx, rocprim::radix_sort_pairs<epa_radix_cfg>(temp, temp_bytes, d_keys, d_keys2, d_idx, d_order, (size_t)n_pairs, 0, 4,
+    EPA_HIP(ctx, rocprim::radix_sort_pairs<epa_radix_cfg>(temp, temp_bytes, d_keys, d_keys2, d_idx, d_order, (size_t)n_pairs, 0, 5,
                                            ctx->stream));
     order = d_order;
   }
   epa_timer_start(ctx, epa_t(ctx, epa_ctx::T_THOROUGH));
   int rc = EPA_OK;
   uint64_t off = 0;
-  ctx->xstamp_ok = present == 1;
+  ctx->xstamp_ok = spans == 1;
+  const bool dual = sp_tips(hist) && ctx->s == 4;
+  hipStream_t const main_stream = ctx->stream;
+  hipStream_t side = nullptr;
+  bool side_clean = false;
+  if (dual) {
+    const int bk = ctx->bank;
+    if (!ctx->side_stream[bk]) {
+      EPA_HIP(ctx, hipStreamCreateWithFlags(&ctx->side_stream[bk], hipStreamNonBlocking));
+      EPA_HIP(ctx, hipEventCreateWithFlags(&ctx->ev_fork[bk], hipEventDisableTiming));
+      EPA_HIP(ctx, hipEventCreateWithFlags(&ctx->ev_join[bk], hipEventDisableTiming));
+    }
+    side = ctx->side_stream[bk];
+    side_clean = ctx->clean_ctr[bk];
+    EPA_HIP(ctx, hipEventRecord(ctx->ev_fork[bk], main_stream));
+    EPA_HIP(ctx, hipStreamWaitEvent(side, ctx->ev_fork[bk], 0));
+  }
   static const uint32_t dna_bound[EPA_N_CLS] = {64, 128, 192, 256, 384, 512, 768, 1024, 1536, 0xffffffffu, 96, 160};
-  for (int c = 0; c < EPA_N_CLS && rc == EPA_OK; ++c) {
-    if (!hist[c]) continue;
+  for (int key = 0; key < EPA_N_CLSX && rc == EPA_OK; ++key) {
+    if (!hist[key]) continue;
+    const int c = epa_base_class(key);
+    const bool tip = key >= EPA_N_CLS;
     const uint32_t* ord = order ? order + off : nullptr;
-    off += hist[c];
+    off += hist[key];
     if (ctx->s == 20) {
       static const uint32_t aa_bound[4] = {64, 128, 192, 0xffffffffu};
       const bool aa_valu = ctx->opt.aa_valu != 0;
       const uint32_t bound = std::min(max_span, aa_bound[c < 4 ? c : 3]);
       const uint32_t mfma_max = ctx->c == 4 ? 384u : 256u;
       if (bound <= mfma_max && (!aa_valu || !ctx->blo.sliding || ctx->c != 4))
-        rc = launch_thorough_aa_mfma(ctx, d_pairs, ord, hist[c], d_codes, d_begin, d_span, bound, d_out, d_stats);
+        rc = launch_thorough_aa_mfma(ctx, d_pairs, ord, hist[key], d_codes, d_begin, d_span, bound, d_out, d_stats);
       else if (ctx->c == 4 && ctx->blo.sliding)
-        rc = launch_thorough_aa(ctx, d_pairs, ord, hist[c], d_codes, d_begin, d_span, bound,
+        rc = launch_thorough_aa(ctx, d_pairs, ord, hist[key], d_codes, d_begin, d_span, bound,
                                 bound <= EPA_AA_LDS_MAX_SPAN, d_out, d_stats);
       else
-        rc = launch_thorough_generic(ctx, d_pairs, hist[c], d_codes, d_begin, d_span, bound, d_out, d_stats, ord, true);
+        rc = launch_thorough_generic(ctx, d_pairs, hist[key], d_codes, d_begin, d_span, bound, d_out, d_stats, ord, true);
       continue;
     }
     ThArgs a = dna_args(ctx, d_pairs, ord, d_codes, d_begin, d_span, d_out, d_stats);
-    a.n_pairs = hist[c];
-    a.xstamp = (present == 1 && ctx->dna.ng == 1 && (c <= 2 || c == 10 || c == 11)) ? 1u : 0u;
-    rc = launch_thorough_dna_class(ctx, a, c, std::min(max_span, dna_bound[c]));
+    a.n_pairs = hist[key];
+    a.xstamp = (spans == 1 && ctx->dna.ng == 1 && (c <= 2 || c == 10 || c == 11)) ? ((tip && hist[c]) ? 2u : 1u) : 0u;
+    if (tip) ctx->stream = side;
+    rc = launch_thorough_dna_class(ctx, a, c, std::min(max_span, dna_bound[c]), tip, dual, side_clean);
+    if (tip) { ctx->stream = main_stream; side_clean = false; }
+  }
+  if (dual) {
+    const int bk = ctx->bank;
+    EPA_HIP(ctx, hipEventRecord(ctx->ev_join[bk], side));
+    EPA_HIP(ctx, hipStreamWaitEvent(main_stream, ctx->ev_join[bk], 0));
+    ctx->clean_ctr[bk] = false;
   }
   epa_timer_stop(ctx, epa_t(ctx, epa_ctx::T_THOROUGH));
   if (rc) return rc;
diff --git a/epa_ng_amd/csrc/thorough_dna_tipd.hip b/epa_ng_amd/csrc/thorough_dna_tipd.hip
--- /dev/null
+++ b/epa_ng_amd/csrc/thorough_dna_tipd.hip
@@ -0,0 +1,2 @@
+#define TH_TIPD_UNIT 1
+#include "thorough_dna.hip"
diff --git a/epa_ng_amd/csrc/thorough_dna_tipd2h.hip b/epa_ng_amd/csrc/thorough_dna_tipd2h.hip
--- /dev/null
+++ b/epa_ng_amd/csrc/thorough_dna_tipd2h.hip
@@ -0,0 +1,2 @@
+#define TH_TIPD_UNIT 2
+#include "thorough_dna.hip"
diff --git a/profiles/dpp_hazard_check.py b/profiles/dpp_hazard_check.py
--- a/profiles/dpp_hazard_check.py
+++ b/profiles/dpp_hazard_check.py
@@ -7,14 +7,15 @@
 
 ROOT = os.path.dirname(os.path.dirname(os.path.abspath(__file__)))
 LLVM = "/opt/rocm/lib/llvm/bin/"
-obj = os.path.join(ROOT, "epa_ng_amd", "build", "thorough_dna.o")
-with tempfile.TemporaryDirectory() as d:
-    fat, co = os.path.join(d, "fat.bin"), os.path.join(d, "k.co")
-    subprocess.check_call([LLVM + "llvm-objcopy", "--dump-section", ".hip_fatbin=" + fat, obj])
-    subprocess.check_call([LLVM + "clang-offload-bundler", "--unbundle", "--type=o", "--input=" + fat,
-                           "--targets=hipv4-amdgcn-amd-amdhsa--gfx950", "--output=" + co])
-    asm = subprocess.check_output([LLVM + "llvm-objdump", "-d", co], text=True)
-
+asm = ""
+for name in ("thorough_dna.o", "thorough_dna_tipd.o", "thorough_dna_tipd2h.o"):
+    obj = os.path.join(ROOT, "epa_ng_amd", "build", name)
+    with tempfile.TemporaryDirectory() as d:
+        fat, co = os.path.join(d, "fat.bin"), os.path.join(d, "k.co")
+        subprocess.check_call([LLVM + "llvm-objcopy", "--dump-section", ".hip_fatbin=" + fat, obj])
+        subprocess.check_call([LLVM + "clang-offload-bundler", "--unbundle", "--type=o", "--input=" + fat,
+                               "--targets=hipv4-amdgcn-amd-amdhsa--gfx950", "--output=" + co])
+        asm += subprocess.check_output([LLVM + "llvm-objdump", "-d", co], text=True) + "\n"
 
 def vregs(op):
     m = re.match(r"v\[(\d+):(\d+)\]", op.strip())
```
